# CompVis/ipoke

Hardware: AMD Instinct MI355X
Metric: video-frames/sec (second-stage train step) (higher is better)
Workload: dtype bf16; 1 GPU; plants_128 second_stage train, 16x3x128x128 clips, z=64, flow 2048 hidden (1.237 B params), per-GPU batch 20; global_batch=20, clip_frames=16, parallelism=dp1, weights=random init of the named architecture (no checkpoints offline)

## Files before the change

include/ipoke_hip.h:

```cpp
#ifndef IPOKE_HIP_H
#define IPOKE_HIP_H

#include <stdint.h>

#ifdef __cplusplus
extern "C" {
#endif

typedef enum {
  IPOKE_OK = 0,
  IPOKE_ERR_INVALID = -1,
  IPOKE_ERR_HIP = -2,
  IPOKE_ERR_STATE = -3
} ipoke_status;

enum { IPOKE_F32 = 0, IPOKE_BF16 = 1 };
enum { IPOKE_ACT_NONE = 0, IPOKE_ACT_ELU = 1, IPOKE_ACT_RELU = 2, IPOKE_ACT_LRELU02 = 3, IPOKE_ACT_TANH = 4,
       IPOKE_ACT_SIGMOID = 5 };

const char* ipoke_last_error(void);
int ipoke_version(void);
int ipoke_dtype_size(int dtype);

typedef struct {
// ... 26 lines not shown
  int32_t w_kmajor;
  int64_t c_sd;
  void* acc_scratch;
  int64_t acc_scratch_bytes;
} ipoke_conv_desc;

int ipoke_conv_forward(const ipoke_conv_desc* d, int dtype, void* stream);
int64_t ipoke_conv_acc_scratch_bytes(int M, int Nout, int splitk);
int ipoke_conv_acc_scratch_init(void* scratch, void* stream);

int ipoke_conv3x3_skinny_splitk(int M, int Kc, int dtype);

typedef struct {
  float* params; float* m; float* v; float* vmax; void* operand;
  float lr, beta1, beta2, eps, weight_decay, grad_scale;
  int32_t step;
  int32_t keep_grad;
} ipoke_wgrad_adam;

typedef struct {
  int32_t NB, Di, Hi, Wi, Do, Ho, Wo, kd, kh, kw, sd, sh, sw, pd, ph, pw, transposed;
  const void* A; int32_t a_f32; int64_t a_sn, a_sd, a_sh, a_sw, a_sc; int32_t a_coff, Kc_real, Kc;
  const void* dY; int32_t ldy; int32_t y_coff; int32_t Nout;
  float* dW; int64_t w_sn, w_sc, w_st;
  int32_t accumulate;
  int32_t splitm;
  int32_t Kc_store;
  int64_t split_stride;
  int32_t max_workgroups;
  const ipoke_wgrad_adam* adam;
} ipoke_wgrad_desc;

int ipoke_conv_wgrad(const ipoke_wgrad_desc* d, int dtype, void* stream);
int ipoke_conv_wgrad_splitm(const ipoke_wgrad_desc* d, int dtype, int target_workgroups);
int ipoke_wgrad_batch_entry_size(void);
int ipoke_conv_wgrad_batched(const ipoke_wgrad_desc* d, const void* entries_dev, int nbatch, const void* a_base,
                             const void* y_base, float* w_base, int dtype, void* stream);


int ipoke_nchw_to_state(const float* x_nchw, float* state, int B, int C, int P, int ld, void* stream);
int ipoke_state_to_nchw(const float* state, float* x_nchw, int B, int C, int P, int ld, void* stream);
int ipoke_extract_cols(const float* state, int ld, int off, int stride, int C, void* out, int ldo, int64_t M, int dtype,
                       void* stream);
int ipoke_cond_prepare(const float* cond_nchw, void* out, int B, int Cc, int P, int act, int dtype, void* stream);
int ipoke_copy_cols(const void* src, int lds, void* dst, int ldd, int C, int64_t M, int dtype, void* stream);

int ipoke_actnorm_fwd(const float* in, float* out, int M, int ld, int c0, int C, const float* log_scale,
                      const float* bias, const int32_t* idx, void* stream);
int ipoke_actnorm_inv(const float* in, float* out, int M, int ld, int c0, int C, const float* log_scale,
                      const float* bias, const int32_t* inv_idx, void* stream);
int ipoke_actnorm_inv_ext(const float* in, float* out, int M, int ld, int c0, int C, const float* log_scale,
                          const float* bias, const int32_t* inv_idx, void* ext, int ext_ld, int e_off, int e_stride, int e_C,
                          int dtype, void* stream);
int ipoke_actnorm_bwd(const float* dy, const float* x, float* dx, int M, int ld, int c0, int C,
                      const float* log_scale, const int32_t* idx, const float* dld, int B, int P,
                      float* part, void* stream);
int ipoke_actnorm_init(const float* x, int M, int ld, int c0, int C, float* log_scale, float* bias, void* stream);

typedef struct {
  const float* raw; int32_t nsplit; int64_t split_stride; int32_t ldraw;
  const float* bias;
  int32_t Cp, t_off, t_stride;
  int32_t P, ld;
} ipoke_affine_desc;
int ipoke_affine_fwd(const ipoke_affine_desc* d, const float* in, float* out, float* scale_out ,
                     float* logdet_slot , int slot_stride, int B, void* stream);
int ipoke_affine_inv(const ipoke_affine_desc* d, const float* in, float* out, int B, void* stream);
int ipoke_affine_fwd_ext(const ipoke_affine_desc* d, const float* in, float* out, float* scale_out, float* logdet_slot, int slot_stride,
                         int B, void* ext, int ext_ld, int dtype, void* stream);
int ipoke_affine_inv_ext(const ipoke_affine_desc* d, const float* in, float* out, int B, void* ext, int ext_ld, int dtype, void* stream);
int ipoke_affine_bwd(int Cp, int t_off, int t_stride, int P, int ld, const float* dy, const float* x,
                     const float* scale, const float* dld, float* dx, void* dparams , int ldp,
                     float* dbias_part , int B, int dtype, void* stream);
int ipoke_affine_actnorm_fwd(const ipoke_affine_desc* d, const float* in, float* out, float* out2, float* scale_out, float* logdet_slot,
                             int slot_stride, int B, int c0, int C, const float* log_scale, const float* bias, const int32_t* idx, void* stream);
int ipoke_actnorm_affine_bwd(int c0, int C, const float* log_scale, const int32_t* idx, const float* dy2, const float* x1, float* part,
                             int Cp, int t_off, int t_stride, int P, int ld, const float* x0, const float* scale, const float* dld, float* dx,
                             void* dparams, int ldp, float* dbias_part, int B, int dtype, void* stream);
typedef struct {
  int32_t mode;
  const float* in; float* out; float* out2; float* scale_out; float* logdet_slot; int32_t slot_stride;
  int32_t an_c0, an_C; const float* an_log_scale; const float* an_bias; const int32_t* an_idx;
  void* ext; int32_t ext_ld;
  void* xchg;
} ipoke_coupling_epi;
int ipoke_conv3x3_coupling_splitk(int M, int Kc, int dtype);
int64_t ipoke_conv3x3_coupling_xchg_bytes(void);
int ipoke_conv3x3_coupling_xchg_init(void* xchg, void* stream);
int ipoke_conv3x3_coupling(const ipoke_conv_desc* conv, const ipoke_affine_desc* aff, const ipoke_coupling_epi* epi, int B, int dtype,
                           void* stream);
int ipoke_reduce_rows(const float* src, float* dst, int R, int ncols, void* stream);
int ipoke_reduce_entry_size(void);
int ipoke_reduce_rows_multi(const float* src, float* dst, const void* entries_dev, int nentries, int R, void* stream);

int ipoke_logdet_finalize(const float* slots, int nslots, int B, int slot_w, float const_term, const float* const_dev,
                          float* logdet, void* stream);
int ipoke_actnorm_logdet(const float* params, const void* refs_dev, int n, int P, float* out_scalar, void* stream);
int ipoke_flow_nll(const float* z_state, const float* logdet, int B, int P, int C, int ld, float logdet_weight,
                   float* scalars3, float* d_out_state, float* dld, void* stream);
int ipoke_adam_amsgrad_step(float* p, const float* g, float* m, float* v, float* vmax, int64_t n, float lr, float beta1,
                            float beta2, float eps, float weight_decay, int step, float grad_scale, void* stream);
int ipoke_adam_amsgrad_step_grid(float* p, const float* g, float* m, float* v, float* vmax, int64_t n, float lr, float beta1,
                                 float beta2, float eps, float weight_decay, int step, float grad_scale, int max_blocks,
                                 void* stream);

typedef struct {
  const float* x; float* y;
  int32_t ld, C, B;
  const void* cond; int32_t Cc;
  const void* W1; const void* W2; const float* bias2;
  int32_t order;
  int32_t rows_per_block;
  void* a2_save; float* scale_save; float* logdet_slot;
  const void* W2T; const void* W1T;
  const float* dy; const float* dld; float* dx;
  void* dparams_save; void* dc_save; float* dbias_part;
  const float* post_log_scale; const float* post_bias;
  const float* y_post; float* post_part;
  void* x_op_save;
  void* zc_out; int32_t zc_off, zc_stride, zc_cin, zc_ld;
  int32_t split; void* xchg;
  const struct ipoke_unit_pair_desc* pair;
} ipoke_mcf_desc;
typedef struct ipoke_unit_pair_desc {
  const float* an_log_scale; const int32_t* an_idx; const float* an_x; float* an_part;
  int32_t Cp, t_off, t_stride; const float* x0; const float* scale; void* dparams; int32_t ldp; float* dbias_part;
  float* dx;
} ipoke_unit_pair_desc;
int ipoke_mcf_shadow_dims(int C, int Cc, int dtype, int32_t* dims8);
int ipoke_mcf_fwd(const ipoke_mcf_desc* d, int dtype, void* stream);
int ipoke_mcf_inv(const ipoke_mcf_desc* d, int dtype, void* stream);
int ipoke_mcf_bwd(const ipoke_mcf_desc* d, int dtype, void* stream);

int ipoke_macow_unit_supported(int C, int Cc, int dtype);
int64_t ipoke_macow_unit_xchg_bytes(int B, int split);
int ipoke_macow_unit_fwd(const ipoke_mcf_desc* d4, int dtype, void* stream);
int ipoke_macow_unit_bwd(const ipoke_mcf_desc* d4, int dtype, void* stream);
int ipoke_macow_unit_inv(const ipoke_mcf_desc* d4, int dtype, void* stream);

int ipoke_relayout_job_size(void);
int ipoke_wn_job_size(void);
int ipoke_relayout_multi(const float* params, void* shadow, const float* wn_scale, const void* jobs_dev, int njobs,
                         int total_blocks, const int32_t* block_job_dev, int dtype, void* stream);
int ipoke_relayout_multi_range(const float* params, void* shadow, const float* wn_scale, const void* jobs_dev, int njobs,
                               int block_begin, int nblocks, const int32_t* block_job_dev, int dtype, void* stream);
int ipoke_wn_scale_multi_range(const float* params, float* scale, float* inv_norm, const void* jobs_dev, int job_begin, int njobs,
                               int row_begin, int nrows, void* stream);
int ipoke_wn_scale_multi(const float* params, float* scale, float* inv_norm, const void* jobs_dev, int njobs,
                         int total_rows, void* stream);
int ipoke_wn_bwd_multi(const float* params, float* grads, const float* inv_norm, const void* jobs_dev, int njobs,
                       int total_rows, void* stream);
int ipoke_wn_bwd_multi_range(const float* params, float* grads, const float* inv_norm, const void* jobs_dev, int job_begin, int njobs,
                             int row_begin, int nrows, void* stream);



int ipoke_lu_job_size(void);
int ipoke_lu_prepare(const float* params, const float* fbuf, float* workspace, const void* jobs_dev, int njobs, void* stream);
int ipoke_lu_apply(const float* in, float* out, int64_t M, int ld, int C, const float* mat, int transposed, void* stream);
int ipoke_lu_wgrad(const float* dy, const float* x, int B, int P8, int ld, const float* params, const float* fbuf,
                   const float* workspace, const void* job_dev, const float* dld, float* grads, void* stream);

typedef struct ipoke_flow ipoke_flow;
typedef struct {
  int32_t z_channels;
  int32_t hidden;
  int32_t cond_channels;
  int32_t factor;
  int32_t n_levels;
  int32_t num_steps[32];
  int32_t kernel_h, kernel_w;
  int32_t dtype;
  int32_t max_batch;
  int32_t use1x1;
  int32_t condition_nice;
} ipoke_flow_config;

int ipoke_flow_create(const ipoke_flow_config* cfg, ipoke_flow** out);
void ipoke_flow_destroy(ipoke_flow* f);
int64_t ipoke_flow_param_count(const ipoke_flow* f);
int64_t ipoke_flow_index_count(const ipoke_flow* f);
int32_t ipoke_flow_tensor_count(const ipoke_flow* f);
int32_t ipoke_flow_op_count(const ipoke_flow* f);
int ipoke_flow_tensor_info(const ipoke_flow* f, int i, char* name, int name_cap, int64_t* offset, int32_t* ndim,
                           int64_t* shape4, int32_t* kind);
int ipoke_flow_set_graph(ipoke_flow* f, int enable);
int64_t ipoke_flow_float_buffer_count(const ipoke_flow* f);
int ipoke_flow_set_float_buffers(ipoke_flow* f, const float* fbuf_dev);
int64_t ipoke_flow_shadow_bytes(const ipoke_flow* f);
int ipoke_flow_op_info(const ipoke_flow* f, int i, int64_t* out32);
int64_t ipoke_flow_shadow_base(const ipoke_flow* f);
int64_t ipoke_flow_workspace_bytes(ipoke_flow* f, int B, int training);
int ipoke_flow_prepare_weights(ipoke_flow* f, const float* params, void* shadow, void* stream);
int ipoke_flow_forward(ipoke_flow* f, const float* params, const int32_t* perm, const void* shadow, const float* x_nchw,
                       const float* cond_nchw, int B, float* out_nchw, float* logdet, void* workspace,
                       int save_for_backward, void* stream);
int ipoke_flow_init_forward(ipoke_flow* f, float* params, const int32_t* perm, const float* x_nchw, int B,
                            float* out_nchw, float* logdet, void* workspace, void* stream);
int ipoke_flow_reverse(ipoke_flow* f, const float* params, const int32_t* perm, const void* shadow, const float* z_nchw,
                       const float* cond_nchw, int B, float* x_nchw, void* workspace, void* stream);
int ipoke_flow_prepare_weights_range(ipoke_flow* f, const float* params, void* shadow, int64_t begin, int64_t end, void* stream);
int ipoke_flow_adam_range(ipoke_flow* f, float* params, const float* grads, float* m, float* v, float* vmax, void* shadow, int64_t begin,
                          int64_t end, float lr, float beta1, float beta2, float eps, float weight_decay, int step, float grad_scale,
                          int max_blocks, void* stream);
int ipoke_adam_tile_job_size(void);
int ipoke_adam_seg_size(void);
int ipoke_adam_amsgrad_shadow_tiles(float* p, const float* g, float* m, float* v, float* vmax, void* shadow, const void* jobs_dev, int njobs,
                                    int tile_begin, int ntiles, float lr, float beta1, float beta2, float eps, float weight_decay, int step,
                                    float grad_scale, int max_blocks, int dtype, void* stream);
int ipoke_adam_amsgrad_cast_tiles(float* p, const float* g, float* m, float* v, float* vmax, void* shadow, const void* jobs_dev, int njobs,
                                  int tile_begin, int ntiles, float lr, float beta1, float beta2, float eps, float weight_decay, int step,
                                  float grad_scale, int max_blocks, int dtype, void* stream);
int ipoke_adam_amsgrad_segments(float* p, const float* g, float* m, float* v, float* vmax, const void* segs_dev, int seg_begin, int nsegs,
                                int64_t begin, int64_t end, float lr, float beta1, float beta2, float eps, float weight_decay, int step,
                                float grad_scale, int blocks_per_segment, void* stream);
int ipoke_flow_backward(ipoke_flow* f, const float* params, const int32_t* perm, const void* shadow,
                        const float* d_out_nchw, const float* d_logdet, int B, float* grads, float* dx_nchw,
                        void* workspace, void* stream);
typedef void (*ipoke_grad_ready_fn)(void* user, int piece, int64_t begin, int64_t end);
int ipoke_flow_piece_ranges(const ipoke_flow* f, int npieces, int64_t* ranges, int max_ranges);
int ipoke_flow_set_native_adam(ipoke_flow* f, float* m, float* v, float* vmax, float lr, float beta1, float beta2, float eps,
                               float weight_decay, int step, float grad_scale, int max_blocks);
int ipoke_flow_backward_pieces(ipoke_flow* f, const float* params, const int32_t* perm, const void* shadow,
                               const float* d_out_nchw, const float* d_logdet, int B, float* grads, float* dx_nchw,
                               void* workspace, int npieces, void* ready_stream, ipoke_grad_ready_fn ready, void* user,
                               void* stream);
int ipoke_flow_handoff_timeouts(ipoke_flow* f, uint32_t* out);
void* ipoke_flow_side_stream(ipoke_flow* f);


typedef struct {
  const void* x; int32_t ldx; void* y; int32_t ldy; int32_t y_f32;
  int32_t N, S, C, G; float eps;
  const float* gamma; const float* beta;
  const void* mod_gamma; const void* mod_beta; int32_t ld_mod;
  const void* res; int32_t ld_res;
  int32_t act;
  float* workspace;
  int32_t mod_samples;
  int32_t res_post;
  float* next_part; int32_t next_G;
  int32_t part_chunks;
} ipoke_norm_desc;
int64_t ipoke_groupnorm_workspace_floats(int N, int S, int G);
int ipoke_groupnorm(const ipoke_norm_desc* d, int dtype, void* stream);
int ipoke_add_act(const void* a, int lda, const void* b, int ldb, void* y, int ldy, int64_t M, int C, int act, int dtype,
                  void* stream);
int ipoke_gru_gates(const void* ur_pre, const void* h, int ldh, void* hr_out, int ld_hr, void* u_out, int64_t M, int Ch,
                    int dtype, void* stream);
int ipoke_gru_update(const void* o_pre, const void* u, const void* h, int ldh, void* h_new, int ld_new, int64_t M, int Ch,
                     int dtype, void* stream);
int ipoke_reparameterize(const void* mulv, int ld, const float* eps, float* z, float* mu, float* logvar, int64_t M, int Z,
                         int dtype, void* stream);
int ipoke_bilinear_cl(const float* x_nchw, float* y_cl, int N, int C, int Hi, int Wi, int Ho, int Wo, void* stream);
int ipoke_cl_to_nchw(const void* x_cl, int ld, float* y, int N, int C, int S, int dtype, void* stream);
int ipoke_nchw_to_cl(const float* x, void* y_cl, int ld, int N, int C, int S, int dtype, void* stream);

int ipoke_groupnorm_stats(const void* x, int ldx, int N, int S, int C, int G, float eps, float* workspace, int dtype, void* stream);
typedef struct {
  const void* x; int32_t ldx;
  const void* y; int32_t ldy;
  const void* dy; int32_t lddy;
  void* dx; int32_t lddx;
  void* dres; int32_t lddres;
  void* dmod_gamma; void* dmod_beta; int32_t ld_dmod;
  int32_t N, S, C, G; float eps;
  const float* gamma; const float* beta;
  const void* mod_gamma; int32_t ld_mod;
  float* dgamma; float* dbeta;
  int32_t act;
  float* workspace;
  const float* stats;
  int32_t mod_samples;
  const float* rs_scale; int32_t rs_scale_stride;
  int64_t rs_rows_per_group;
  const float* rs_bias;
  float* rs_dots;
  float* rs_dbias;
  float* rs_workspace;
  int32_t dmod_summed;
  int32_t act_from_pre;
} ipoke_norm_bwd_desc;
int64_t ipoke_groupnorm_stats_offset(int N, int S, int G);
int64_t ipoke_groupnorm_bwd_workspace_floats(int N, int S, int C, int G);
int64_t ipoke_groupnorm_bwd_rs_workspace_floats(int N, int S, int C);
int ipoke_groupnorm_bwd(const ipoke_norm_bwd_desc* d, int dtype, void* stream);
int ipoke_act_bwd(const void* dy, int lddy, const void* y, int ldy, void* out, int ldo, int64_t M, int C, int Cpad, int act,
                  int dtype, void* stream);
int64_t ipoke_colsum_workspace_floats(int64_t M, int C);
int ipoke_colsum(const void* src, int ld, int64_t M, int C, int src_f32, float* out, int accumulate, float* workspace, int dtype,
                 void* stream);
int ipoke_gru_update_bwd(const void* o_pre, const void* u, const void* h, int ldh, const void* d_hnew, int ld_dhnew, void* d_o_pre,
                         void* d_u, void* d_h, int ld_dh, int64_t M, int Ch, int dtype, void* stream);
int ipoke_gru_gates_bwd(const void* ur_pre, const void* h, int ldh, const void* d_hr, int ld_dhr, const void* d_u, void* d_ur_pre,
                        void* d_h, int ld_dh, int64_t M, int Ch, int dtype, void* stream);
int ipoke_conv_weight_operand(const float* w, int cout, int cin, int taps, int transposed, const float* inv_scale, void* out, int kc,
                              int dtype, void* stream);
int ipoke_conv_weight_operand_multi(const float* const* w, void* const* out, const int32_t* dims5, int count, int dtype, void* stream);
typedef struct { int32_t B, T, L, Cx, Ch, H, W; } ipoke_gru_desc;
int64_t ipoke_gru_workspace_bytes(const ipoke_gru_desc* d, int dtype);
int ipoke_gru_unroll_forward(const ipoke_gru_desc* d, const void* x0, int ldx, const void* h0, int ldh, const float* const* weights,
                             void* workspace, void* out, int ldo, int dtype, void* stream);
int ipoke_gru_unroll_backward(const ipoke_gru_desc* d, const void* d_out, int ldo, void* workspace, float* const* dweights, float* d_x0,
                              float* d_h0, int dtype, void* stream);
typedef struct {
  const void* dy; int32_t lddy;
// ... 80 lines not shown
```

include/ipoke_hip_dev.h:

```cpp
#ifndef IPOKE_HIP_DEV_H
#define IPOKE_HIP_DEV_H

#include "ipoke_hip.h"

#ifdef __cplusplus
extern "C" {
#endif

int ipoke_conv_forward_repeat(const ipoke_conv_desc* d, int dtype, int n, void* stream);
int ipoke_set_dispatch_override(const char* name, int value);
enum { IPOKE_KERNEL_NONE = 0, IPOKE_KERNEL_IGEMM = 1, IPOKE_KERNEL_S8 = 2, IPOKE_KERNEL_HALO = 3, IPOKE_KERNEL_HALO16 = 4, IPOKE_KERNEL_C64 = 5, IPOKE_KERNEL_K8 = 6 };
int ipoke_last_conv_kernel(void);
enum { IPOKE_WGRAD_KERNEL_NONE = 0, IPOKE_WGRAD_KERNEL_TN = 1, IPOKE_WGRAD_KERNEL_TN_GLDS = 2, IPOKE_WGRAD_KERNEL_TN_NARROW = 3,
       IPOKE_WGRAD_KERNEL_LAT8 = 4, IPOKE_WGRAD_KERNEL_HALO = 5 };
int ipoke_last_wgrad_kernel(void);

int ipoke_spin_delay(int us, void* stream);

#define IPOKE_TAG_NT_SQUARE 1
#define IPOKE_TAG_TN_SQUARE 2
#define IPOKE_TAG_UNIT_FWD 3
#define IPOKE_TAG_UNIT_BWD 4
#define IPOKE_TAG_UNIT_INV 5
#define IPOKE_TAG_NN_SQUARE 6
#define IPOKE_TAG_CONV_BASE 16
#define IPOKE_TAG_WGRAD 32
int ipoke_timing_start(void);
int ipoke_timing_start_all(void);
int ipoke_timing_stop(const int* tags, int ntags, int* counts, double* mean_us);
int ipoke_timing_stop_ex(const int* tags, int ntags, int* counts, double* total_us, double* flops, double* bytes);

int ipoke_desc_sizes(int32_t* out, int n);

int ipoke_flow_test_inject_timeout(ipoke_flow* f, int which, void* stream);

int ipoke_gru_set_fused(int mode);

#ifdef __cplusplus
}
#endif
#endif
```

ipoke_amd/_lib.py:

```python
import ctypes
import os
from ctypes import CFUNCTYPE, POINTER, Structure, c_char_p, c_float, c_int, c_int32, c_int64, c_uint32, c_void_p

_HERE = os.path.dirname(os.path.abspath(__file__))
LIB_PATH = os.environ.get("IPOKE_LIB_PATH") or os.path.join(_HERE, "libipoke_hip.so")

F32, BF16 = 0, 1
ACT_NONE, ACT_ELU, ACT_RELU, ACT_LRELU02, ACT_TANH, ACT_SIGMOID = range(6)

DTYPES = {"f32": F32, "fp32": F32, "float32": F32, "bf16": BF16, "bfloat16": BF16}


class ConvDesc(Structure):
    _fields_ = [(n, c_int32) for n in ("NB", "Di", "Hi", "Wi", "Do", "Ho", "Wo", "kd", "kh", "kw", "sd", "sh", "sw",
                                       "pd", "ph", "pw", "transposed")] + [
        ("A", c_void_p), ("a_f32", c_int32),
        ("a_sn", c_int64), ("a_sd", c_int64), ("a_sh", c_int64), ("a_sw", c_int64), ("a_sc", c_int64),
        ("a_coff", c_int32), ("Kc_real", c_int32), ("Kc", c_int32),
        ("W", c_void_p), ("ldw", c_int32), ("Nout", c_int32),
        ("bias", c_void_p), ("act", c_int32), ("dact", c_void_p), ("ld_dact", c_int32), ("dact_act", c_int32),
        ("C", c_void_p), ("c_f32", c_int32), ("c_accumulate", c_int32), ("ldc", c_int64),
        ("c_coff", c_int32), ("c_cstride", c_int32), ("splitk", c_int32),
        ("c_scatter", c_int32), ("c_sn", c_int64), ("c_sh", c_int64), ("c_sw", c_int64), ("c_row0", c_int64),
        ("row_scale", c_void_p), ("rs_images", c_int32), ("rs_stride", c_int32), ("w_kmajor", c_int32), ("c_sd", c_int64),
# ... 79 lines not shown
                ("N", c_int32), ("S", c_int32), ("C", c_int32), ("G", c_int32), ("eps", c_float),
                ("gamma", c_void_p), ("beta", c_void_p),
                ("mod_gamma", c_void_p), ("mod_beta", c_void_p), ("ld_mod", c_int32),
                ("res", c_void_p), ("ld_res", c_int32), ("act", c_int32), ("workspace", c_void_p), ("mod_samples", c_int32),
                ("res_post", c_int32), ("next_part", c_void_p), ("next_G", c_int32), ("part_chunks", c_int32)]


class SnJob(Structure):
    _fields_ = [("w", c_void_p), ("cout", c_int32), ("cin", c_int32), ("taps", c_int32), ("transposed", c_int32),
                ("u", c_void_p), ("v", c_void_p), ("out", c_void_p), ("out_stride", c_int64), ("snap", c_void_p), ("snap_stride", c_int64),
                ("workspace", c_void_p)]


class FlowConfig(Structure):
    _fields_ = [("z_channels", c_int32), ("hidden", c_int32), ("cond_channels", c_int32), ("factor", c_int32),
                ("n_levels", c_int32), ("num_steps", c_int32 * 32), ("kernel_h", c_int32), ("kernel_w", c_int32),
                ("dtype", c_int32), ("max_batch", c_int32), ("use1x1", c_int32), ("condition_nice", c_int32)]


_P = c_void_p
GRAD_READY_FN = CFUNCTYPE(None, c_void_p, c_int, c_int64, c_int64)
SIGNATURES = {
    "ipoke_last_error": (c_char_p, []),
    "ipoke_version": (c_int, []),
    "ipoke_dtype_size": (c_int, [c_int]),
    "ipoke_conv_forward": (c_int, [POINTER(ConvDesc), c_int, _P]),
    "ipoke_conv_forward_repeat": (c_int, [POINTER(ConvDesc), c_int, c_int, _P]),
    "ipoke_set_dispatch_override": (c_int, [c_char_p, c_int]),
    "ipoke_last_conv_kernel": (c_int, []),
    "ipoke_last_wgrad_kernel": (c_int, []),
    "ipoke_gru_set_fused": (c_int, [c_int]),
    "ipoke_gru_workspace_bytes": (c_int64, [POINTER(GruDesc), c_int]),
    "ipoke_gru_unroll_forward": (c_int, [POINTER(GruDesc), _P, c_int, _P, c_int, POINTER(c_void_p), _P, _P, c_int, c_int, _P]),
    "ipoke_gru_unroll_backward": (c_int, [POINTER(GruDesc), _P, c_int, _P, POINTER(c_void_p), _P, _P, c_int, _P]),
    "ipoke_rowscale_bwd_workspace_floats": (c_int64, [c_int64, c_int, c_int64]),
    "ipoke_rowscale_bwd": (c_int, [POINTER(RowScaleBwdDesc), c_int, _P]),
    "ipoke_spectral_bwd_frames": (c_int, [_P, c_int, c_int, c_int, c_int, _P, _P, c_int64, _P, c_int64, _P, c_int, _P]),
    "ipoke_sum_frames": (c_int, [_P, _P, c_int, c_int64, c_int, _P]),
    "ipoke_desc_sizes": (c_int, [POINTER(c_int32), c_int]),
    "ipoke_conv3x3_skinny_splitk": (c_int, [c_int, c_int, c_int]),
    "ipoke_conv3x3_coupling_splitk": (c_int, [c_int, c_int, c_int]),
    "ipoke_conv3x3_coupling_xchg_bytes": (c_int64, []),
    "ipoke_conv3x3_coupling_xchg_init": (c_int, [_P, _P]),
    "ipoke_conv3x3_coupling": (c_int, [POINTER(ConvDesc), POINTER(AffineDesc), POINTER(CouplingEpi), c_int, c_int, _P]),
    "ipoke_conv_wgrad": (c_int, [POINTER(WgradDesc), c_int, _P]),
    "ipoke_wgrad_batch_entry_size": (c_int, []),
    "ipoke_conv_wgrad_batched": (c_int, [POINTER(WgradDesc), _P, c_int, _P, _P, _P, c_int, _P]),
    "ipoke_reduce_entry_size": (c_int, []),
    "ipoke_reduce_rows_multi": (c_int, [_P, _P, _P, c_int, c_int, _P]),
    "ipoke_nchw_to_state": (c_int, [_P, _P, c_int, c_int, c_int, c_int, _P]),
    "ipoke_state_to_nchw": (c_int, [_P, _P, c_int, c_int, c_int, c_int, _P]),
    "ipoke_extract_cols": (c_int, [_P, c_int, c_int, c_int, c_int, _P, c_int, c_int64, c_int, _P]),
    "ipoke_copy_cols": (c_int, [_P, c_int, _P, c_int, c_int, c_int64, c_int, _P]),
    "ipoke_cond_prepare": (c_int, [_P, _P, c_int, c_int, c_int, c_int, c_int, _P]),
    "ipoke_actnorm_fwd": (c_int, [_P, _P, c_int, c_int, c_int, c_int, _P, _P, _P, _P]),
    "ipoke_actnorm_inv": (c_int, [_P, _P, c_int, c_int, c_int, c_int, _P, _P, _P, _P]),
    "ipoke_actnorm_inv_ext": (c_int, [_P, _P, c_int, c_int, c_int, c_int, _P, _P, _P, _P, c_int, c_int, c_int, c_int, c_int, _P]),
    "ipoke_actnorm_bwd": (c_int, [_P, _P, _P, c_int, c_int, c_int, c_int, _P, _P, _P, c_int, c_int, _P, _P]),
    "ipoke_actnorm_init": (c_int, [_P, c_int, c_int, c_int, c_int, _P, _P, _P]),
    "ipoke_affine_fwd": (c_int, [POINTER(AffineDesc), _P, _P, _P, _P, c_int, c_int, _P]),
    "ipoke_affine_inv": (c_int, [POINTER(AffineDesc), _P, _P, c_int, _P]),
    "ipoke_affine_fwd_ext": (c_int, [POINTER(AffineDesc), _P, _P, _P, _P, c_int, c_int, _P, c_int, c_int, _P]),
    "ipoke_affine_inv_ext": (c_int, [POINTER(AffineDesc), _P, _P, c_int, _P, c_int, c_int, _P]),
    "ipoke_affine_bwd": (c_int, [c_int, c_int, c_int, c_int, c_int, _P, _P, _P, _P, _P, _P, c_int, _P, c_int, c_int, _P]),
    "ipoke_affine_actnorm_fwd": (c_int, [POINTER(AffineDesc), _P, _P, _P, _P, _P, c_int, c_int, c_int, c_int, _P, _P, _P, _P]),
    "ipoke_actnorm_affine_bwd": (c_int, [c_int, c_int, _P, _P, _P, _P, _P, c_int, c_int, c_int, c_int, c_int, _P, _P, _P, _P, _P, c_int, _P,
                                         c_int, c_int, _P]),
    "ipoke_reduce_rows": (c_int, [_P, _P, c_int, c_int, _P]),
    "ipoke_spin_delay": (c_int, [c_int, _P]),
    "ipoke_logdet_finalize": (c_int, [_P, c_int, c_int, c_int, c_float, _P, _P, _P]),
    "ipoke_actnorm_logdet": (c_int, [_P, _P, c_int, c_int, _P, _P]),
    "ipoke_flow_nll": (c_int, [_P, _P, c_int, c_int, c_int, c_int, c_float, _P, _P, _P, _P]),
    "ipoke_adam_amsgrad_step": (c_int, [_P, _P, _P, _P, _P, c_int64, c_float, c_float, c_float, c_float, c_float, c_int,
                                        c_float, _P]),
    "ipoke_adam_amsgrad_step_grid": (c_int, [_P, _P, _P, _P, _P, c_int64, c_float, c_float, c_float, c_float, c_float, c_int,
                                             c_float, c_int, _P]),
    "ipoke_mcf_shadow_dims": (c_int, [c_int, c_int, c_int, POINTER(c_int32)]),
    "ipoke_mcf_fwd": (c_int, [POINTER(McfDesc), c_int, _P]),
    "ipoke_mcf_inv": (c_int, [POINTER(McfDesc), c_int, _P]),
    "ipoke_mcf_bwd": (c_int, [POINTER(McfDesc), c_int, _P]),
    "ipoke_macow_unit_supported": (c_int, [c_int, c_int, c_int]),
    "ipoke_macow_unit_xchg_bytes": (c_int64, [c_int, c_int]),
    "ipoke_macow_unit_fwd": (c_int, [POINTER(McfDesc), c_int, _P]),
    "ipoke_macow_unit_bwd": (c_int, [POINTER(McfDesc), c_int, _P]),
    "ipoke_macow_unit_inv": (c_int, [POINTER(McfDesc), c_int, _P]),
    "ipoke_relayout_job_size": (c_int, []),
    "ipoke_wn_job_size": (c_int, []),
    "ipoke_relayout_multi": (c_int, [_P, _P, _P, _P, c_int, c_int, _P, c_int, _P]),
    "ipoke_wn_scale_multi": (c_int, [_P, _P, _P, _P, c_int, c_int, _P]),
    "ipoke_wn_bwd_multi": (c_int, [_P, _P, _P, _P, c_int, c_int, _P]),
    "ipoke_groupnorm_workspace_floats": (c_int64, [c_int, c_int, c_int]),
    "ipoke_groupnorm": (c_int, [POINTER(NormDesc), c_int, _P]),
    "ipoke_add_act": (c_int, [_P, c_int, _P, c_int, _P, c_int, c_int64, c_int, c_int, c_int, _P]),
    "ipoke_gru_gates": (c_int, [_P, _P, c_int, _P, c_int, _P, c_int64, c_int, c_int, _P]),
    "ipoke_gru_update": (c_int, [_P, _P, _P, c_int, _P, c_int, c_int64, c_int, c_int, _P]),
    "ipoke_reparameterize": (c_int, [_P, c_int, _P, _P, _P, _P, c_int64, c_int, c_int, _P]),
    "ipoke_bilinear_cl": (c_int, [_P, _P, c_int, c_int, c_int, c_int, c_int, c_int, _P]),
    "ipoke_cl_to_nchw": (c_int, [_P, c_int, _P, c_int, c_int, c_int, c_int, _P]),
    "ipoke_nchw_to_cl": (c_int, [_P, _P, c_int, c_int, c_int, c_int, c_int, _P]),
    "ipoke_image_metrics_workspace_bytes": (c_int64, [c_int64, c_int, c_int]),
    "ipoke_psnr_ssim": (c_int, [_P, _P, c_int64, c_int, c_int, _P, _P, _P]),
    "ipoke_clip_to_cl4": (c_int, [_P, c_int64, c_int64, c_int64, c_int64, c_int64, c_int, c_int, c_int, c_int, c_int, c_int, _P, c_int, _P]),
    "ipoke_groupnorm_stats": (c_int, [_P, c_int, c_int, c_int, c_int, c_int, c_float, _P, c_int, _P]),
    "ipoke_groupnorm_stats_offset": (c_int64, [c_int, c_int, c_int]),
    "ipoke_groupnorm_bwd_workspace_floats": (c_int64, [c_int, c_int, c_int, c_int]),
    "ipoke_groupnorm_bwd": (c_int, [POINTER(NormBwdDesc), c_int, _P]),
    "ipoke_groupnorm_bwd_rs_workspace_floats": (c_int64, [c_int, c_int, c_int]),
    "ipoke_act_bwd": (c_int, [_P, c_int, _P, c_int, _P, c_int, c_int64, c_int, c_int, c_int, c_int, _P]),
    "ipoke_colsum_workspace_floats": (c_int64, [c_int64, c_int]),
    "ipoke_colsum": (c_int, [_P, c_int, c_int64, c_int, c_int, _P, c_int, _P, c_int, _P]),
    "ipoke_gru_update_bwd": (c_int, [_P, _P, _P, c_int, _P, c_int, _P, _P, _P, c_int, c_int64, c_int, c_int, _P]),
    "ipoke_gru_gates_bwd": (c_int, [_P, _P, c_int, _P, c_int, _P, _P, _P, c_int, c_int64, c_int, c_int, _P]),
    "ipoke_conv_weight_operand": (c_int, [_P, c_int, c_int, c_int, c_int, _P, _P, c_int, c_int, _P]),
    "ipoke_conv_weight_operand_multi": (c_int, [POINTER(c_void_p), POINTER(c_void_p), POINTER(c_int32), c_int, c_int, _P]),
    "ipoke_spectral_workspace_floats": (ctypes.c_long, [c_int, c_int, c_int]),
    "ipoke_spectral_sigma": (c_int, [_P, c_int, c_int, c_int, c_int, _P, _P, c_int, ctypes.c_float, _P, _P, _P, _P]),
    "ipoke_spectral_bwd": (c_int, [_P, c_int, c_int, c_int, c_int, _P, _P, _P, _P, _P]),
    "ipoke_spectral_bwd_workspace_floats": (ctypes.c_long, []),
    "ipoke_sn_job_size": (c_int, []),
    "ipoke_sn_jobs_upload": (c_int, [_P, c_int, _P, _P]),
    "ipoke_spectral_sigma_multi": (c_int, [_P, c_int, c_int, c_int, c_int, c_float, _P]),
    "ipoke_adam_multi": (c_int, [_P, _P, _P, _P, _P, c_int, ctypes.c_float, ctypes.c_float, ctypes.c_float, ctypes.c_float,
                                 ctypes.c_float, c_int, ctypes.c_float, _P]),
    "ipoke_maxpool3d_fwd": (c_int, [_P, _P, c_int, _P, c_int, _P, c_int, _P]),
    "ipoke_maxpool3d_bwd": (c_int, [_P, _P, c_int, _P, _P, c_int, c_int, _P]),
    "ipoke_avgpool_rows": (c_int, [_P, c_int, _P, c_int, c_int64, c_int, c_int, c_int, _P]),
    "ipoke_avgpool_rows_bwd": (c_int, [_P, c_int, _P, c_int, c_int64, c_int, c_int, c_int, _P]),
    "ipoke_groupnorm_jvp": (c_int, [_P, c_int, _P, c_int, _P, c_int, _P, c_int, _P, c_int, _P, c_int, c_int, c_int, c_int, c_int, c_float,
                                    _P, c_int, _P]),
    "ipoke_groupnorm_jvp_bwd": (c_int, [_P, c_int, _P, c_int, _P, c_int, _P, c_int, _P, c_int, _P, c_int, _P, c_int, _P, _P,
                                        c_int, c_int, c_int, c_int, c_int, c_float, _P, c_int, _P]),
    "ipoke_groupnorm_jvp_workspace_floats": (ctypes.c_long, [c_int, c_int]),
    "ipoke_gather_rows": (c_int, [_P, c_int, _P, _P, c_int, c_int64, c_int, c_int, _P]),
    "ipoke_l1_pair": (c_int, [_P, c_int, _P, c_int, c_int64, c_int, c_float, _P, _P, c_int, c_int, _P]),
    "ipoke_kl_loss": (c_int, [_P, _P, c_int64, c_int, _P, _P, _P, _P]),
    "ipoke_reparam_bwd": (c_int, [_P, c_int, _P, _P, _P, _P, _P, c_int, c_int64, c_int, c_int, _P]),
    "ipoke_l1_loss": (c_int, [_P, c_int, _P, c_int, c_int, c_int, c_int64, c_float, _P, _P, c_int, _P, _P]),
    "ipoke_l1_loss_partials": (ctypes.c_long, []),
    "ipoke_relayout_multi_range": (c_int, [_P, _P, _P, _P, c_int, c_int, c_int, _P, c_int, _P]),
    "ipoke_wn_scale_multi_range": (c_int, [_P, _P, _P, _P, c_int, c_int, c_int, c_int, _P]),
    "ipoke_flow_prepare_weights_range": (c_int, [_P, _P, _P, c_int64, c_int64, _P]),
    "ipoke_flow_set_native_adam": (c_int, [_P, _P, _P, _P, c_float, c_float, c_float, c_float, c_float, c_int, c_float, c_int]),
    "ipoke_flow_adam_range": (c_int, [_P, _P, _P, _P, _P, _P, _P, c_int64, c_int64, c_float, c_float, c_float, c_float, c_float, c_int,
                                      c_float, c_int, _P]),
    "ipoke_adam_tile_job_size": (c_int, []),
    "ipoke_adam_seg_size": (c_int, []),
    "ipoke_adam_amsgrad_shadow_tiles": (c_int, [_P, _P, _P, _P, _P, _P, _P, c_int, c_int, c_int, c_float, c_float, c_float, c_float, c_float,
                                                c_int, c_float, c_int, c_int, _P]),
    "ipoke_adam_amsgrad_cast_tiles": (c_int, [_P, _P, _P, _P, _P, _P, _P, c_int, c_int, c_int, c_float, c_float, c_float, c_float, c_float,
                                              c_int, c_float, c_int, c_int, _P]),
    "ipoke_adam_amsgrad_segments": (c_int, [_P, _P, _P, _P, _P, _P, c_int, c_int, c_int64, c_int64, c_float, c_float, c_float, c_float,
                                            c_float, c_int, c_float, c_int, _P]),
    "ipoke_wn_bwd_multi_range": (c_int, [_P, _P, _P, _P, c_int, c_int, c_int, c_int, _P]),
    "ipoke_flow_backward_pieces": (c_int, [_P, _P, _P, _P, _P, _P, c_int, _P, _P, _P, c_int, _P, GRAD_READY_FN, _P, _P]),
    "ipoke_video_to_cl": (c_int, [_P, c_int64, c_int64, c_int64, c_int64, c_int64, c_int, c_int, c_int, c_int, c_int, _P, c_int, c_int, c_int,
                                  c_int, _P, _P]),
    "ipoke_min_reset": (c_int, [_P, _P]),
    "ipoke_denorm_if_negative": (c_int, [_P, c_int64, c_int, c_int, c_int, c_int, _P, _P]),
    "ipoke_pool3d_same": (c_int, [_P, _P, c_int, _P, c_int, c_int, _P]),
    "ipoke_pool_rows_weighted": (c_int, [_P, c_int, _P, c_int, c_int64, c_int, c_int, _P, c_int, _P]),
    "ipoke_activation_moments": (c_int, [_P, c_int, c_int, _P, _P, _P, _P]),
    "ipoke_flow_resize": (c_int, [_P, _P, c_int, c_int, c_int, c_int, c_int, c_int, c_float, _P]),
    "ipoke_poke_workspace_bytes": (c_int64, [c_int, c_int, c_int, c_int, c_int]),
    "ipoke_poke_simulate": (c_int, [_P, c_int, c_int, c_int, c_int, c_int, c_int, c_int, _P, _P, _P, _P, _P, _P, _P, _P]),
    "ipoke_timing_start": (c_int, []),
    "ipoke_timing_start_all": (c_int, []),
    "ipoke_timing_stop": (c_int, [POINTER(c_int), c_int, POINTER(c_int), POINTER(ctypes.c_double)]),
    "ipoke_timing_stop_ex": (c_int, [POINTER(c_int), c_int, POINTER(c_int), POINTER(ctypes.c_double), POINTER(ctypes.c_double),
                                     POINTER(ctypes.c_double)]),
    "ipoke_flow_create": (c_int, [POINTER(FlowConfig), POINTER(c_void_p)]),
    "ipoke_flow_destroy": (None, [_P]),
    "ipoke_flow_piece_ranges": (c_int, [_P, c_int, POINTER(c_int64), c_int]),
    "ipoke_flow_handoff_timeouts": (c_int, [_P, POINTER(c_uint32)]),
    "ipoke_flow_side_stream": (c_void_p, [_P]),
    "ipoke_flow_test_inject_timeout": (c_int, [_P, c_int, _P]),
    "ipoke_conv_wgrad_splitm": (c_int, [_P, c_int, c_int]),
    "ipoke_conv_acc_scratch_bytes": (c_int64, [c_int, c_int, c_int]),
    "ipoke_conv_acc_scratch_init": (c_int, [_P, _P]),
    "ipoke_flow_param_count": (c_int64, [_P]),
    "ipoke_flow_index_count": (c_int64, [_P]),
    "ipoke_flow_tensor_count": (c_int32, [_P]),
    "ipoke_flow_op_count": (c_int32, [_P]),
    "ipoke_flow_tensor_info": (c_int, [_P, c_int, c_char_p, c_int, POINTER(c_int64), POINTER(c_int32), POINTER(c_int64),
                                       POINTER(c_int32)]),
    "ipoke_flow_shadow_bytes": (c_int64, [_P]),
    "ipoke_flow_set_graph": (c_int, [_P, c_int]),
    "ipoke_flow_float_buffer_count": (c_int64, [_P]),
    "ipoke_flow_set_float_buffers": (c_int, [_P, _P]),
    "ipoke_lu_job_size": (c_int, []),
    "ipoke_lu_prepare": (c_int, [_P, _P, _P, _P, c_int, _P]),
    "ipoke_lu_apply": (c_int, [_P, _P, c_int64, c_int, c_int, _P, c_int, _P]),
    "ipoke_lu_wgrad": (c_int, [_P, _P, c_int, c_int, c_int, _P, _P, _P, _P, _P, _P, _P]),
    "ipoke_flow_op_info": (c_int, [_P, c_int, POINTER(c_int64)]),
    "ipoke_flow_shadow_base": (c_int64, [_P]),
    "ipoke_flow_workspace_bytes": (c_int64, [_P, c_int, c_int]),
    "ipoke_flow_prepare_weights": (c_int, [_P, _P, _P, _P]),
    "ipoke_flow_forward": (c_int, [_P, _P, _P, _P, _P, _P, c_int, _P, _P, _P, c_int, _P]),
    "ipoke_flow_init_forward": (c_int, [_P, _P, _P, _P, c_int, _P, _P, _P, _P]),
    "ipoke_flow_reverse": (c_int, [_P, _P, _P, _P, _P, _P, c_int, _P, _P, _P]),
    "ipoke_flow_backward": (c_int, [_P, _P, _P, _P, _P, _P, c_int, _P, _P, _P, _P]),
}

_lib = None


def lib():
    global _lib
    if _lib is None:
        if not os.path.exists(LIB_PATH):
            raise RuntimeError(
                f"{LIB_PATH} not found: the HIP extension is not built. ipoke_amd has no CPU fallback; "
                "run `make -C ipoke_amd/csrc` (or __graft_entry__.build()) first.")
        import torch
        handle = ctypes.CDLL(LIB_PATH)
        for name, (res, args) in SIGNATURES.items():
            fn = getattr(handle, name)
            fn.restype = res
            fn.argtypes = args
        _lib = handle
    return _lib


def check(rc):
    if rc != 0:
        msg = lib().ipoke_last_error()
        raise RuntimeError(f"libipoke_hip call failed ({rc}): {msg.decode() if msg else '?'}")


def ptr(t):
    if t is None:
        return None
    return c_void_p(t.data_ptr())


def current_stream():
    import torch
    return c_void_p(torch.cuda.current_stream().cuda_stream)


def require_gpu():
    import torch
    if not torch.cuda.is_available():
        raise RuntimeError("ipoke_amd needs an MI355X (gfx950) GPU: no HIP device is visible and there is no CPU path")


import contextlib


KERNEL_NONE, KERNEL_IGEMM, KERNEL_S8, KERNEL_HALO, KERNEL_HALO16, KERNEL_C64, KERNEL_K8 = range(7)
WGRAD_NONE, WGRAD_TN, WGRAD_TN_GLDS, WGRAD_TN_NARROW, WGRAD_LAT8, WGRAD_HALO = range(6)


@contextlib.contextmanager
def dispatch_override(name, value):
    check(lib().ipoke_set_dispatch_override(name.encode(), int(value)))
    try:
        yield
    finally:
        check(lib().ipoke_set_dispatch_override(name.encode(), -1))
```

ipoke_amd/csrc/flow_engine.hip:

```cpp
#include <functional>
#include <memory>
#include <vector>
#include <string>
#include <cstring>

#include "common.h"

namespace ipoke {

enum OpType { OP_ACTNORM = 0, OP_MCF = 1, OP_NICE = 2, OP_LU = 3 };
enum TensorKind { TK_PARAM = 0, TK_IDX_FWD = 1, TK_IDX_BWD = 2, TK_FLAG = 3, TK_FBUF = 4 };

struct TensorInfo {
  std::string name;
  int64_t offset;
  std::vector<int64_t> shape;
  int kind;
};

struct Op {
  int type = 0;
  int C = 0;
  int c0 = 0, Cn = 0;
  int64_t p_ls = -1, p_bias = -1, idx_fwd = -1, idx_bwd = -1;
  int order = 0;
  int64_t p_w1 = -1, p_b = -1, p_g = -1, p_v = -1;
  int Cp = 0, K1p = 0, K2p = 0, K3p = 0, Hq = 0, H = 0;
  int64_t sh_w1 = -1, sh_w1t = -1, sh_w2 = -1, sh_w2t = -1;
  int64_t wn_off = -1;
  int cin = 0, cout = 0, z_off = 0, z_stride = 1, t_off = 0, t_stride = 1;
  int64_t p_c1 = -1, p_c2 = -1;
  int Kc1 = 0, Kc3 = 0;
  int64_t sh_c1 = -1, sh_c1t = -1, sh_c2 = -1, sh_c2t = -1, sh_c3 = -1, sh_c3t = -1;
  int64_t ws_a = -1, ws_b = -1, ws_c = -1, ws_d = -1, ws_e = -1, ws_f = -1, ws_g = -1;
  int slot = -1;
  int mcf_idx = -1;
  int nice_idx = -1;
  int hidK = 0;
  int level = 0;
  int fuse_act = -1;
  bool fused = false;
  bool unit_head = false;
  int unit_of = -1;
  int lu_idx = -1;
  int an_next = -1;
  int an_prev = -1;
  int pair_unit = -1;
};

struct RelayoutJobH {
  long src_off, s_n, s_k, dstA, dstB, scale_off;
  int taps, n_real, k_real, A_rows_pad, A_inner_pad, B_rows_pad, B_inner_pad, B_rows_real, tile, tiles_k, block_start, frag_tiled;
};
struct WnJobH { long v_off, g_off, out_off; int rows, K, row_start; };
struct AdamTileJobH { long src_off, dstA, dstB; int N, K, tile_start, pad; };
struct AdamSegH { long off, len; };
struct LsRefH { long off; int C; };
struct LuJobH { long p_l, p_u, p_logs, b_perm, b_sign, b_lmask, b_umask, b_eye, w_off; int C, pad; };

}

using namespace ipoke;

struct ipoke_flow {
  ipoke_flow_config cfg;
  int esz = 2, e16 = 8, ks = 32;
  std::vector<TensorInfo> tensors;
  std::vector<Op> ops;
  int64_t n_params = 0, n_perm = 0, n_fbuf = 0;
  std::vector<LuJobH> lujobs; void* d_lujobs = nullptr; const float* fbuf = nullptr;
  int64_t shadow_elems = 0;
  int64_t wn_rows = 0;
  int nslots = 0;
  int n_mcf = 0;
  int tab_B = 0; void* d_w1tab = nullptr; void* d_w2tab = nullptr; void* d_redtab = nullptr; int n_red = 0;
  void* d_ntab[3] = {nullptr, nullptr, nullptr};
  int n_nice = 0;
  std::vector<RelayoutJobH> rjobs; int rblocks = 0;
  std::vector<AdamTileJobH> ajobs; int atiles = 0;
  std::vector<RelayoutJobH> rjobs2; int rblocks2 = 0;
  std::vector<AdamSegH> asegs;
  void* d_ajobs = nullptr; void* d_rjobs2 = nullptr; void* d_rblockjob2 = nullptr; void* d_asegs = nullptr;
  std::vector<WnJobH> wjobs;
  std::vector<LsRefH> lsrefs;
  void* d_rjobs = nullptr; void* d_wjobs = nullptr; void* d_lsrefs = nullptr; void* d_rblockjob = nullptr;
  hipStream_t side = nullptr;
  std::vector<hipStream_t> lanes;
  int n_lanes = 1;
  std::vector<hipEvent_t> events; size_t ev_next = 0;
  bool use_side = true;
  struct GraphEntry { std::vector<uintptr_t> key; hipGraph_t graph = nullptr; hipGraphExec_t exec = nullptr; int state = 0; uint64_t used = 0; };
  std::vector<GraphEntry> graphs; hipStream_t cap = nullptr; bool use_graph = false; uint64_t tick = 0;
  struct Unit { int64_t p_lo, p_hi; int wj_lo, wj_hi, row_lo, row_hi; int kind; int op_lo, op_hi; int64_t p2_lo = -1, p2_hi = -1; };
  std::vector<Unit> units;
  std::vector<int> red_first;
  int last_fwd_B = 0; bool have_saved = false;
  int P = 64;
  int unit_split = 1; void* d_xchg = nullptr;
  bool coupling_fuse = false; void* d_cxchg = nullptr;
  void* d_acc = nullptr; int64_t acc_bytes = 0;
  unsigned* h_tmo = nullptr; hipEvent_t pass_ev = nullptr; hipStream_t pass_stream = nullptr; bool pass_recorded = false, pass_unchecked = false;
  int64_t xchg_bytes = 0;
  bool mcf_xop = false;
  bool c2_straight = false;
  struct NativeAdam { bool on = false; float* m = nullptr; float* v = nullptr; float* vmax = nullptr; float lr = 0, beta1 = 0, beta2 = 0, eps = 0, wd = 0,
                      grad_scale = 1; int step = 0, max_blocks = 0; } nadam;
};

namespace {

int64_t align_up(int64_t v, int64_t a) { return (v + a - 1) / a * a; }

struct Builder {
  ipoke_flow& f;
  explicit Builder(ipoke_flow& fl) : f(fl) {}
  int64_t add_param(const std::string& name, std::vector<int64_t> shape) {
    int64_t n = 1; for (auto s : shape) n *= s;
    const int64_t off = f.n_params;
    f.tensors.push_back({name, off, shape, TK_PARAM});
    f.n_params = align_up(off + n, 4);
    return off;
  }
  int64_t add_idx(const std::string& name, int C, int kind) {
    const int64_t off = f.n_perm;
    f.tensors.push_back({name, off, {C}, kind});
    f.n_perm += C;
    return off;
  }
  void add_flag(const std::string& name) { f.tensors.push_back({name, -1, {}, TK_FLAG}); }
  int64_t add_fbuf(const std::string& name, std::vector<int64_t> shape) {
    int64_t n = 1; for (auto s : shape) n *= s;
    const int64_t off = f.n_fbuf;
    f.tensors.push_back({name, off, shape, TK_FBUF});
    f.n_fbuf = align_up(off + n, 4);
    return off;
  }
  void lu(const std::string& pfx, int C) {
    Op op; op.type = OP_LU; op.C = C; op.lu_idx = (int)f.lujobs.size();
    LuJobH j{};
    j.C = C;
    j.p_l = add_param(pfx + ".l", {C, C}); j.p_u = add_param(pfx + ".u", {C, C}); j.p_logs = add_param(pfx + ".log_s", {C});
    j.b_perm = add_fbuf(pfx + ".permutated", {C, C}); j.b_sign = add_fbuf(pfx + ".sign_s", {C});
    j.b_lmask = add_fbuf(pfx + ".lmask", {C, C}); j.b_umask = add_fbuf(pfx + ".umask", {C, C}); j.b_eye = add_fbuf(pfx + ".eye", {C, C});
    j.w_off = (long)op.lu_idx * 4 * 64 * 64;
    f.lujobs.push_back(j);
    f.lsrefs.push_back({j.p_logs, C});
    f.ops.push_back(op);
  }
  int64_t add_shadow(int64_t elems) {
    const int64_t off = f.shadow_elems;
    f.shadow_elems = align_up(off + elems, 64);
    return off;
  }
  void relayout_pair(long src, long s_n, long s_k, int taps, int n_real, int k_real, long scale, long dstA, int A_rows_pad,
                     int A_inner_pad, long dstB, int B_rows_pad, int B_inner_pad, int B_rows_real, int frag_tiled = 0) {
    const int tile = taps == 1 ? 64 : 32;
    const int n_ext = std::max(A_rows_pad, B_inner_pad), k_ext = std::max(A_inner_pad, B_rows_pad);
    const int tiles_n = (n_ext + tile - 1) / tile, tiles_k = (k_ext + tile - 1) / tile;
    RelayoutJobH j{src, s_n, s_k, dstA, dstB, scale, taps, n_real, k_real, A_rows_pad, A_inner_pad, B_rows_pad, B_inner_pad,
                   B_rows_real, tile, tiles_k, f.rblocks, frag_tiled};
    f.rjobs.push_back(j);
    f.rblocks += tiles_n * tiles_k;
    const bool fusable = taps == 1 && scale < 0 && !frag_tiled && s_k == 1 && s_n == k_real && n_real % 64 == 0 && k_real % 64 == 0 &&
                         A_rows_pad == n_real && A_inner_pad == k_real && B_rows_pad == k_real && B_inner_pad == n_real &&
                         B_rows_real == k_real;
    if (fusable) {
      f.ajobs.push_back({src, dstA, dstB, n_real, k_real, f.atiles, 0});
      f.atiles += (n_real / 64) * (k_real / 64);
    } else {
      j.block_start = f.rblocks2;
      f.rjobs2.push_back(j);
      f.rblocks2 += tiles_n * tiles_k;
    }
  }

  void actnorm(const std::string& pfx, int C_active, int c0, int Cn, const std::string* shuffle_pfx) {
    Op op; op.type = OP_ACTNORM; op.C = C_active; op.c0 = c0; op.Cn = Cn;
    if (!pfx.empty()) {
      op.p_ls = add_param(pfx + ".log_scale", {Cn, 1, 1});
      op.p_bias = add_param(pfx + ".bias", {Cn, 1, 1});
      add_flag(pfx + ".initialized");
      f.lsrefs.push_back({(long)op.p_ls, Cn});
    }
    if (shuffle_pfx) {
      op.idx_fwd = add_idx(*shuffle_pfx + ".forward_shuffle_idx", Cn, TK_IDX_FWD);
      op.idx_bwd = add_idx(*shuffle_pfx + ".backward_shuffle_idx", Cn, TK_IDX_BWD);
    }
    f.ops.push_back(op);
  }

  void mcf(const std::string& pfx, int C, int order) {
    const int Cc = f.cfg.cond_channels;
    Op op; op.type = OP_MCF; op.C = C; op.order = order;
    const int kh = order < 2 ? f.cfg.kernel_h : f.cfg.kernel_w, kw = order < 2 ? f.cfg.kernel_w : f.cfg.kernel_h;
    op.H = 4 * C;
    op.Cp = round_up(C, f.ks);
    op.K1p = 6 * op.Cp;
    op.K2p = round_up(op.H + Cc, f.ks);
    op.K3p = round_up(2 * C, f.ks);
    op.Hq = round_up(op.H, f.ks);
    const int K2 = op.H + Cc;
    op.p_w1 = add_param(pfx + ".net.shift_conv.weight", {op.H, C, kh, kw});
    add_flag(pfx + ".net.conv1x1.initialized");
    op.p_b = add_param(pfx + ".net.conv1x1.conv.bias", {2 * C});
    op.p_g = add_param(pfx + ".net.conv1x1.conv.weight_g", {2 * C, 1, 1, 1});
    op.p_v = add_param(pfx + ".net.conv1x1.conv.weight_v", {2 * C, K2, 1, 1});
    op.wn_off = f.wn_rows;
    f.wjobs.push_back({(long)op.p_v, (long)op.p_g, (long)op.wn_off, 2 * C, K2, (int)f.wn_rows});
    f.wn_rows += 2 * C;
    const int Hr = round_up(op.H, 16), N2r = round_up(2 * C, 16), Cr = round_up(C, 16);
    op.sh_w1 = add_shadow((int64_t)Hr * op.K1p);
    op.sh_w1t = add_shadow((int64_t)Cr * 6 * op.Hq);
    op.sh_w2 = add_shadow((int64_t)N2r * op.K2p);
    op.sh_w2t = add_shadow((int64_t)Hr * op.K3p);
    relayout_pair(op.p_w1, (long)C * 6, 6, 6, op.H, C, -1, op.sh_w1, Hr, op.Cp, op.sh_w1t, Cr, op.Hq, C, 1);
    relayout_pair(op.p_v, K2, 1, 1, 2 * C, K2, op.wn_off, op.sh_w2, N2r, op.K2p, op.sh_w2t, Hr, op.K3p, op.H, 1);
    op.slot = f.nslots++;
    op.mcf_idx = f.n_mcf++;
    f.ops.push_back(op);
  }

  void nice(const std::string& pfx, int C, bool skip, bool up, int factor) {
    const int hid = f.cfg.hidden;
    Op op; op.type = OP_NICE; op.C = C;
    op.cout = C / factor; op.cin = C - op.cout;
    if (skip && (C % 2 == 1)) skip = false;
    if (!skip) {
      const int z1 = up ? op.cin : op.cout;
      if (up) { op.z_off = 0; op.t_off = z1; } else { op.z_off = z1; op.t_off = 0; }
      op.z_stride = op.t_stride = 1;
    } else {
      op.z_stride = op.t_stride = 2;
      if (up) { op.z_off = 0; op.t_off = 1; } else { op.z_off = 1; op.t_off = 0; }
    }
    op.Kc1 = round_up(op.cin, f.e16);
    op.Kc3 = round_up(2 * op.cout, f.e16);
// ... 304 lines not shown
  d.W1 = c.sh(op.sh_w1); d.W2 = c.sh(op.sh_w2); d.bias2 = c.params + op.p_b; d.order = op.order;
  d.W1T = c.sh(op.sh_w1t); d.W2T = c.sh(op.sh_w2t);
}

int lu_prepare_all(const Ctx& c) {
  ipoke_flow* f = c.f;
  if (f->lujobs.empty()) return IPOKE_OK;
  IPK_REQUIRE(f->fbuf != nullptr, "use1x1: ipoke_flow_set_float_buffers has not been called");
  IPK_REQUIRE(f->n_lanes == 1, "use1x1 does not support sub-batch lanes");
  return ipoke_lu_prepare(c.params, f->fbuf, c.at<float>(c.plan.lu), f->d_lujobs, (int)f->lujobs.size(), c.stream());
}
const float* lu_mat(const Ctx& c, const Op& op, int which) {
  return c.at<float>(c.plan.lu) + (int64_t)op.lu_idx * 4 * 64 * 64 + (int64_t)which * op.C * op.C;
}

int common_checks(ipoke_flow* f, int B) {
  IPK_REQUIRE(f != nullptr, "null flow handle");
  IPK_REQUIRE(B >= 1 && B <= f->cfg.max_batch, "batch exceeds max_batch of the flow handle");
  return IPOKE_OK;
}

struct WgEntryH { long a_off, y_off, w_off; int kh, kw, ph, pw; long sh_off = 0; };
struct RedEntryH { long src, dst; int ld, ncols, rmul, pad; };

void drop_graphs(ipoke_flow* f) {
  for (auto& g : f->graphs) {
    if (g.exec) (void)hipGraphExecDestroy(g.exec);
    if (g.graph) (void)hipGraphDestroy(g.graph);
  }
  f->graphs.clear();
}

int ensure_tables(ipoke_flow* f, int B, const Plan& plan) {
  if (f->tab_B == B && f->d_w1tab) return IPOKE_OK;
  IPK_REQUIRE((int)sizeof(WgEntryH) == ipoke_wgrad_batch_entry_size() && (int)sizeof(RedEntryH) == ipoke_reduce_entry_size(),
              "batch table layout mismatch");
  std::vector<WgEntryH> w1(f->n_mcf), w2(f->n_mcf);
  std::vector<WgEntryH> nt[3] = {std::vector<WgEntryH>(f->n_nice), std::vector<WgEntryH>(f->n_nice), std::vector<WgEntryH>(f->n_nice)};
  std::vector<RedEntryH> red;
  f->red_first.assign(f->ops.size() + 1, 0);
  for (size_t i = 0; i < f->ops.size(); ++i) {
    const Op& op = f->ops[i];
    f->red_first[i] = (int)red.size();
    const long dbp = (long)(plan.dbias_part / 4) + (long)i * (kMaxUnitSplit * B + 1) * 128;
    const int rmul = op.unit_of >= 0 || op.pair_unit >= 0 ? f->unit_split : 1;
    if (op.type == OP_MCF) {
      const McfGeom g = mcf_geom(op.order);
      w1[op.mcf_idx] = {f->mcf_xop ? (long)op.ws_e : (long)(plan.state0 + (int64_t)i * plan.state_stride), (long)op.ws_d, (long)op.p_w1, g.kh,
                        g.kw, -g.oy, -g.ox};
      w2[op.mcf_idx] = {(long)op.ws_a, (long)op.ws_c, (long)op.p_v, 1, 1, 0, 0};
      red.push_back({dbp, (long)op.p_b, 2 * op.C, 2 * op.C, rmul, 0});
    } else if (op.type == OP_NICE) {
      nt[0][op.nice_idx] = {(long)op.ws_g, (long)op.ws_f, (long)op.p_c1, 3, 3, 1, 1};
      nt[1][op.nice_idx] = {(long)op.ws_a, (long)op.ws_e, (long)op.p_c2, 1, 1, 0, 0, (long)op.sh_c2};
      nt[2][op.nice_idx] = {(long)op.ws_b, (long)op.ws_d, (long)op.p_v, 3, 3, 1, 1};
      red.push_back({dbp, (long)op.p_b, 2 * op.cout, 2 * op.cout, rmul, 0});
    } else if (op.p_ls >= 0) {
      red.push_back({dbp, (long)op.p_ls, 2 * op.Cn, op.Cn, rmul, 0});
      red.push_back({dbp + op.Cn, (long)op.p_bias, 2 * op.Cn, op.Cn, rmul, 0});
    }
  }
  drop_graphs(f);
  f->red_first[f->ops.size()] = (int)red.size();
  if (f->d_w1tab) { (void)hipFree(f->d_w1tab); (void)hipFree(f->d_w2tab); (void)hipFree(f->d_redtab); }
  for (int k = 0; k < 3; ++k) {
    if (f->d_ntab[k]) (void)hipFree(f->d_ntab[k]);
    IPK_HIP(hipMalloc(&f->d_ntab[k], nt[k].size() * sizeof(WgEntryH)));
    IPK_HIP(hipMemcpy(f->d_ntab[k], nt[k].data(), nt[k].size() * sizeof(WgEntryH), hipMemcpyHostToDevice));
  }
  IPK_HIP(hipMalloc(&f->d_w1tab, w1.size() * sizeof(WgEntryH)));
  IPK_HIP(hipMalloc(&f->d_w2tab, w2.size() * sizeof(WgEntryH)));
  IPK_HIP(hipMalloc(&f->d_redtab, red.size() * sizeof(RedEntryH)));
  IPK_HIP(hipMemcpy(f->d_w1tab, w1.data(), w1.size() * sizeof(WgEntryH), hipMemcpyHostToDevice));
  IPK_HIP(hipMemcpy(f->d_w2tab, w2.data(), w2.size() * sizeof(WgEntryH), hipMemcpyHostToDevice));
  IPK_HIP(hipMemcpy(f->d_redtab, red.data(), red.size() * sizeof(RedEntryH), hipMemcpyHostToDevice));
  f->n_red = (int)red.size();
  f->tab_B = B;
  return IPOKE_OK;
}

std::vector<std::pair<int, int>> backward_pieces(const ipoke_flow* f, int npieces) {
  std::vector<std::pair<int, int>> pieces;
  const int U = (int)f->units.size();
  int64_t total = 0;
  for (const auto& u : f->units) total += u.p_hi - u.p_lo;
  const int np = npieces < 1 ? 1 : (npieces > U ? U : npieces);
  static double ta = -1, tb = -1;
  if (ta < 0) {
    ta = 0.5; tb = 0.25;
    if (const char* e = getenv("IPOKE_PIECE_TAPER")) { double a = 0, b = 0; if (sscanf(e, "%lf,%lf", &a, &b) == 2 && a > 0 && b > 0) { ta = a; tb = b; } }
  }
  std::vector<double> w((size_t)np, 1.0);
  if (np >= 4) { w[(size_t)np - 2] = ta; w[(size_t)np - 1] = tb; }
  double wsum = 0; for (double x : w) wsum += x;
  int hi = U - 1;
  int64_t acc = 0; double target_acc = 0;
  int64_t done = 0;
  for (int u = U - 1; u >= 0; --u) {
    acc += f->units[u].p_hi - f->units[u].p_lo;
    const int idx = (int)pieces.size();
    const int left = np - idx;
    const double want = (double)total * (target_acc + w[(size_t)(idx < np ? idx : np - 1)]) / wsum;
    if (u == 0 || (left > 1 && ((double)(done + acc) >= want || u == left - 1))) {
      pieces.push_back({u, hi}); hi = u - 1; done += acc; acc = 0; target_acc += w[(size_t)(idx < np ? idx : np - 1)];
    }
  }
  return pieces;
}
void piece_param_ranges(const ipoke_flow* f, int lvl_lo, int lvl_hi, int64_t p0[3], int64_t p1[3]) {
  for (int k = 0; k < 3; ++k) { p0[k] = -1; p1[k] = -1; }
  for (int u = lvl_lo; u <= lvl_hi; ++u) {
    const auto& un = f->units[u];
    const int k = un.kind;
    if (p0[k] < 0) p0[k] = un.p_lo;
    p1[k] = un.p_hi;
    if (un.p2_lo >= 0) { if (p0[2] < 0) p0[2] = un.p2_lo; p1[2] = un.p2_hi; }
  }
}

hipEvent_t next_event(ipoke_flow* f) {
  hipEvent_t e = f->events[f->ev_next];
  f->ev_next = (f->ev_next + 1) % f->events.size();
  return e;
}

}

extern "C" int ipoke_flow_create(const ipoke_flow_config* cfg, ipoke_flow** out) {
  IPK_REQUIRE(cfg && out, "null argument");
  IPK_REQUIRE(cfg->dtype == IPOKE_F32 || cfg->dtype == IPOKE_BF16, "bad dtype");
  IPK_REQUIRE(cfg->n_levels >= 1 && cfg->n_levels <= 32 && cfg->n_levels < cfg->factor, "num_steps must be shorter than factor");
  IPK_REQUIRE(cfg->z_channels % cfg->factor == 0 && cfg->z_channels <= 64, "flow_in_channels must be a multiple of factor, <= 64");
  IPK_REQUIRE((cfg->z_channels / cfg->factor) % 2 == 0, "channel step must be even (skip split)");
  IPK_REQUIRE(cfg->kernel_h == 2 && cfg->kernel_w == 3, "kernel_size must be [2,3] (shipped configs)");
  IPK_REQUIRE(cfg->hidden % 32 == 0 && cfg->cond_channels % 32 == 0, "hidden / cond widths must be multiples of 32");
  std::unique_ptr<ipoke_flow> f(new ipoke_flow());
  f->cfg = *cfg;
  f->esz = cfg->dtype == IPOKE_BF16 ? 2 : 4; f->e16 = 16 / f->esz; f->ks = 64 / f->esz;
  {
    const char* cs = getenv("IPOKE_C2_STRAIGHT");
    f->c2_straight = cfg->dtype == IPOKE_BF16 && cfg->hidden % 64 == 0 && !(cs && cs[0] == '0');
  }
  int rc = build(*f); if (rc) return rc;
  {
    int64_t pos = 0;
    for (size_t k = 0; k < f->ajobs.size(); ++k) {
      IPK_REQUIRE(f->ajobs[k].src_off >= pos, "fused tensors must be in parameter order");
      if (f->ajobs[k].src_off > pos) f->asegs.push_back({(long)pos, (long)(f->ajobs[k].src_off - pos)});
      pos = f->ajobs[k].src_off + (int64_t)f->ajobs[k].N * f->ajobs[k].K;
    }
    if (pos < f->n_params) f->asegs.push_back({(long)pos, (long)(f->n_params - pos)});
    for (size_t k = 1; k < f->rjobs.size(); ++k) IPK_REQUIRE(f->rjobs[k].src_off > f->rjobs[k - 1].src_off, "relayout jobs must be in parameter order");
  }
  const char* env = getenv("IPOKE_NO_SIDE_STREAM");
  f->use_side = !(env && env[0] == '1');
  const char* gr = getenv("IPOKE_GRAPH");
  f->use_graph = gr && gr[0] == '1';
  const char* ln = getenv("IPOKE_LANES");
  f->n_lanes = ln ? atoi(ln) : 1;
  if (f->n_lanes < 1) f->n_lanes = 1;
  if (f->n_lanes > kMaxLanes) f->n_lanes = kMaxLanes;
  {
    const char* us = getenv("IPOKE_UNIT_SPLIT");
    f->unit_split = us ? atoi(us) : kDefaultUnitSplit;
    if (f->unit_split != 2 && f->unit_split != 4) f->unit_split = 1;
    if (f->n_lanes > 1 || cfg->dtype != IPOKE_BF16) f->unit_split = 1;
  }
  f->coupling_fuse = f->n_lanes == 1 && cfg->dtype == IPOKE_BF16 && ipoke_conv3x3_coupling_splitk(64, cfg->hidden, cfg->dtype) > 0;
  {
    const char* up = getenv("IPOKE_UNIT_PAIR");
    const bool on = f->unit_split > 1 && f->n_lanes == 1 && (up ? atoi(up) != 0 : true);
    for (size_t h = 2; on && h < f->ops.size(); ++h) {
      const Op& u = f->ops[h]; Op& an = f->ops[h - 1]; Op& cp = f->ops[h - 2];
      if (u.unit_head && an.type == OP_ACTNORM && an.an_prev == (int)h - 2 && cp.type == OP_NICE && an.c0 == 0 && an.Cn == u.C &&
          cp.cout <= 32 && cp.t_off + (cp.cout - 1) * cp.t_stride < u.C) {
        an.pair_unit = (int)h; cp.pair_unit = (int)h;
      }
    }
  }
  *out = f.release();
  return IPOKE_OK;
}

static int ensure_device(ipoke_flow* f) {
  if (f->d_rjobs) return IPOKE_OK;
  if (f->unit_split > 1 && !f->d_xchg) {
    const int64_t nb = ipoke_macow_unit_xchg_bytes(f->cfg.max_batch, f->unit_split);
    IPK_HIP(hipMalloc(&f->d_xchg, nb));
    IPK_HIP(hipMemset(f->d_xchg, 0, nb));
    f->xchg_bytes = nb;
  }
  if (!f->d_acc) {
    static const bool atomics = getenv("IPOKE_DGRAD_ATOMICS") != nullptr;
    if (!atomics) {
      f->acc_bytes = ipoke_conv_acc_scratch_bytes(f->cfg.max_batch * f->P, 64, 32);
      IPK_HIP(hipMalloc(&f->d_acc, (size_t)f->acc_bytes));
      int rc = ipoke_conv_acc_scratch_init(f->d_acc, nullptr); if (rc) return rc;
      IPK_HIP(hipDeviceSynchronize());
    }
  }
  if (!f->h_tmo) {
    IPK_HIP(hipHostMalloc(reinterpret_cast<void**>(&f->h_tmo), 64, hipHostMallocMapped));
    std::memset(f->h_tmo, 0, 64);
    IPK_HIP(hipEventCreateWithFlags(&f->pass_ev, hipEventDisableTiming));
  }
  if (f->coupling_fuse && !f->d_cxchg) {
    IPK_HIP(hipMalloc(&f->d_cxchg, (size_t)ipoke_conv3x3_coupling_xchg_bytes()));
    int rc = ipoke_conv3x3_coupling_xchg_init(f->d_cxchg, nullptr); if (rc) return rc;
    IPK_HIP(hipDeviceSynchronize());
  }
  IPK_REQUIRE((int)sizeof(RelayoutJobH) == ipoke_relayout_job_size() && (int)sizeof(WnJobH) == ipoke_wn_job_size(),
              "job table layout mismatch");
  IPK_HIP(hipMalloc(&f->d_rjobs, f->rjobs.size() * sizeof(RelayoutJobH)));
  IPK_HIP(hipMemcpy(f->d_rjobs, f->rjobs.data(), f->rjobs.size() * sizeof(RelayoutJobH), hipMemcpyHostToDevice));
  {
    std::vector<int32_t> bj((size_t)f->rblocks);
    for (size_t k = 0; k < f->rjobs.size(); ++k) {
      const int b0 = f->rjobs[k].block_start, b1 = k + 1 < f->rjobs.size() ? f->rjobs[k + 1].block_start : f->rblocks;
      for (int b = b0; b < b1; ++b) bj[b] = (int32_t)k;
    }
    IPK_HIP(hipMalloc(&f->d_rblockjob, bj.size() * sizeof(int32_t)));
    IPK_HIP(hipMemcpy(f->d_rblockjob, bj.data(), bj.size() * sizeof(int32_t), hipMemcpyHostToDevice));
  }
  IPK_REQUIRE((int)sizeof(AdamTileJobH) == ipoke_adam_tile_job_size() && (int)sizeof(AdamSegH) == ipoke_adam_seg_size(), "Adam table layout mismatch");
  if (!f->ajobs.empty()) {
    IPK_HIP(hipMalloc(&f->d_ajobs, f->ajobs.size() * sizeof(AdamTileJobH)));
    IPK_HIP(hipMemcpy(f->d_ajobs, f->ajobs.data(), f->ajobs.size() * sizeof(AdamTileJobH), hipMemcpyHostToDevice));
  }
  if (!f->asegs.empty()) {
    IPK_HIP(hipMalloc(&f->d_asegs, f->asegs.size() * sizeof(AdamSegH)));
    IPK_HIP(hipMemcpy(f->d_asegs, f->asegs.data(), f->asegs.size() * sizeof(AdamSegH), hipMemcpyHostToDevice));
  }
  if (!f->rjobs2.empty()) {
    IPK_HIP(hipMalloc(&f->d_rjobs2, f->rjobs2.size() * sizeof(RelayoutJobH)));
    IPK_HIP(hipMemcpy(f->d_rjobs2, f->rjobs2.data(), f->rjobs2.size() * sizeof(RelayoutJobH), hipMemcpyHostToDevice));
    std::vector<int32_t> bj((size_t)f->rblocks2);
    for (size_t k = 0; k < f->rjobs2.size(); ++k) {
      const int b0 = f->rjobs2[k].block_start, b1 = k + 1 < f->rjobs2.size() ? f->rjobs2[k + 1].block_start : f->rblocks2;
      for (int b = b0; b < b1; ++b) bj[b] = (int32_t)k;
    }
    IPK_HIP(hipMalloc(&f->d_rblockjob2, bj.size() * sizeof(int32_t)));
    IPK_HIP(hipMemcpy(f->d_rblockjob2, bj.data(), bj.size() * sizeof(int32_t), hipMemcpyHostToDevice));
  }
  IPK_HIP(hipMalloc(&f->d_wjobs, f->wjobs.size() * sizeof(WnJobH)));
  IPK_HIP(hipMemcpy(f->d_wjobs, f->wjobs.data(), f->wjobs.size() * sizeof(WnJobH), hipMemcpyHostToDevice));
  if (!f->lujobs.empty()) {
    IPK_REQUIRE((int)sizeof(LuJobH) == ipoke_lu_job_size(), "LU job table layout mismatch");
    IPK_HIP(hipMalloc(&f->d_lujobs, f->lujobs.size() * sizeof(LuJobH)));
    IPK_HIP(hipMemcpy(f->d_lujobs, f->lujobs.data(), f->lujobs.size() * sizeof(LuJobH), hipMemcpyHostToDevice));
  }
  IPK_HIP(hipMalloc(&f->d_lsrefs, f->lsrefs.size() * sizeof(LsRefH)));
  IPK_HIP(hipMemcpy(f->d_lsrefs, f->lsrefs.data(), f->lsrefs.size() * sizeof(LsRefH), hipMemcpyHostToDevice));
  {
    int least = 0, greatest = 0;
    IPK_HIP(hipDeviceGetStreamPriorityRange(&least, &greatest));
    static const bool flat = getenv("IPOKE_SIDE_FLAT_PRIORITY") != nullptr;
    IPK_HIP(hipStreamCreateWithPriority(&f->side, hipStreamNonBlocking, flat ? 0 : least));
  }
  IPK_HIP(hipStreamCreateWithFlags(&f->cap, hipStreamNonBlocking));
  f->lanes.resize(kMaxLanes - 1);
  for (auto& l : f->lanes) IPK_HIP(hipStreamCreateWithFlags(&l, hipStreamNonBlocking));
  f->events.resize(256);
  for (auto& e : f->events) IPK_HIP(hipEventCreateWithFlags(&e, hipEventDisableTiming));
  return IPOKE_OK;
}

extern "C" void ipoke_flow_destroy(ipoke_flow* f) {
  if (!f) return;
  if (f->d_rjobs) (void)hipFree(f->d_rjobs);
  if (f->d_wjobs) (void)hipFree(f->d_wjobs);
  if (f->d_lsrefs) (void)hipFree(f->d_lsrefs);
  if (f->d_lujobs) (void)hipFree(f->d_lujobs);
  if (f->d_rblockjob) (void)hipFree(f->d_rblockjob);
  if (f->d_ajobs) (void)hipFree(f->d_ajobs);
  if (f->d_asegs) (void)hipFree(f->d_asegs);
  if (f->d_rjobs2) (void)hipFree(f->d_rjobs2);
  if (f->d_rblockjob2) (void)hipFree(f->d_rblockjob2);
  if (f->d_w1tab) (void)hipFree(f->d_w1tab);
  for (int k = 0; k < 3; ++k) if (f->d_ntab[k]) (void)hipFree(f->d_ntab[k]);
  if (f->d_w2tab) (void)hipFree(f->d_w2tab);
  if (f->d_redtab) (void)hipFree(f->d_redtab);
  if (f->d_xchg) (void)hipFree(f->d_xchg);
  if (f->d_cxchg) (void)hipFree(f->d_cxchg);
  if (f->d_acc) (void)hipFree(f->d_acc);
  if (f->pass_ev) (void)hipEventDestroy(f->pass_ev);
  if (f->h_tmo) (void)hipHostFree(f->h_tmo);
  for (auto e : f->events) (void)hipEventDestroy(e);
  drop_graphs(f);
  if (f->side) (void)hipStreamDestroy(f->side);
  if (f->cap) (void)hipStreamDestroy(f->cap);
  for (auto l : f->lanes) if (l) (void)hipStreamDestroy(l);
  delete f;
}

extern "C" int ipoke_flow_piece_ranges(const ipoke_flow* f, int npieces, int64_t* ranges, int max_ranges) {
  IPK_REQUIRE(f != nullptr && (ranges != nullptr || max_ranges == 0), "bad arguments");
  const std::vector<std::pair<int, int>> pieces = backward_pieces(f, npieces);
  int n = 0;
  for (size_t i = 0; i < pieces.size(); ++i) {
    int64_t p0[3], p1[3];
    piece_param_ranges(f, pieces[i].first, pieces[i].second, p0, p1);
    for (int kind = 0; kind < 3; ++kind) {
      if (p0[kind] < 0 || p1[kind] <= p0[kind]) continue;
      if (n < max_ranges) { ranges[3 * n] = (int64_t)i; ranges[3 * n + 1] = p0[kind]; ranges[3 * n + 2] = p1[kind]; }
      ++n;
    }
  }
  return n;
}

extern "C" void* ipoke_flow_side_stream(ipoke_flow* f) {
  if (!f || ensure_device(f) != IPOKE_OK) return nullptr;
  return reinterpret_cast<void*>(f->side);
}
extern "C" int64_t ipoke_flow_param_count(const ipoke_flow* f) { return f ? f->n_params : -1; }
extern "C" int64_t ipoke_flow_index_count(const ipoke_flow* f) { return f ? f->n_perm : -1; }
extern "C" int ipoke_flow_set_graph(ipoke_flow* f, int enable) {
  IPK_REQUIRE(f != nullptr, "null flow handle");
  f->use_graph = enable != 0;
  return IPOKE_OK;
}
extern "C" int64_t ipoke_flow_float_buffer_count(const ipoke_flow* f) { return f ? f->n_fbuf : -1; }
extern "C" int ipoke_flow_set_float_buffers(ipoke_flow* f, const float* fbuf_dev) {
  IPK_REQUIRE(f != nullptr, "null flow handle");
  f->fbuf = fbuf_dev;
  return IPOKE_OK;
}
extern "C" int32_t ipoke_flow_tensor_count(const ipoke_flow* f) { return f ? (int32_t)f->tensors.size() : -1; }
extern "C" int32_t ipoke_flow_op_count(const ipoke_flow* f) { return f ? (int32_t)f->ops.size() : -1; }
extern "C" int ipoke_flow_tensor_info(const ipoke_flow* f, int i, char* name, int name_cap, int64_t* offset, int32_t* ndim,
                                      int64_t* shape4, int32_t* kind) {
  IPK_REQUIRE(f && i >= 0 && i < (int)f->tensors.size() && name && offset && ndim && shape4 && kind, "bad arguments");
  const TensorInfo& t = f->tensors[i];
  IPK_REQUIRE((int)t.name.size() + 1 <= name_cap, "name buffer too small");
  std::memcpy(name, t.name.c_str(), t.name.size() + 1);
  *offset = t.offset; *ndim = (int32_t)t.shape.size(); *kind = t.kind;
  for (int k = 0; k < 4; ++k) shape4[k] = k < (int)t.shape.size() ? t.shape[k] : 1;
  return IPOKE_OK;
}
extern "C" int ipoke_flow_op_info(const ipoke_flow* f, int i, int64_t* out32) {
  IPK_REQUIRE(f && out32 && i >= 0 && i < (int)f->ops.size(), "bad arguments");
  const Op& o = f->ops[i];
  const int64_t v[32] = {o.type, o.C, o.c0, o.Cn, o.p_ls, o.p_bias, o.idx_fwd, o.idx_bwd, o.order, o.p_w1, o.p_b, o.p_g, o.p_v,
                         o.sh_w1, o.sh_w1t, o.sh_w2, o.sh_w2t, o.wn_off, o.cin, o.cout, o.z_off, o.z_stride, o.t_off, o.t_stride,
                         o.p_c1, o.p_c2, o.sh_c1, o.sh_c1t, o.sh_c2, o.sh_c2t, o.sh_c3, o.sh_c3t};
  for (int k = 0; k < 32; ++k) out32[k] = v[k];
  return IPOKE_OK;
}
extern "C" int64_t ipoke_flow_shadow_base(const ipoke_flow* f) { return f ? 2 * align_up(f->wn_rows, 64) * 4 : -1; }

extern "C" int64_t ipoke_flow_shadow_bytes(const ipoke_flow* f) {
  if (!f) return -1;
  return 2 * align_up(f->wn_rows, 64) * 4 + f->shadow_elems * f->esz;
}
extern "C" int64_t ipoke_flow_workspace_bytes(ipoke_flow* f, int B, int training) {
  if (!f || B < 1) return -1;
  return make_plan(*f, B, training ? 1 : 0).bytes;
}

extern "C" int ipoke_flow_prepare_weights(ipoke_flow* f, const float* params, void* shadow, void* stream) {
  IPK_REQUIRE(f && params && shadow, "null argument");
  { int rc0 = ensure_device(f); if (rc0) return rc0; }
  float* wn_scale = reinterpret_cast<float*>(shadow);
  float* wn_inv = wn_scale + align_up(f->wn_rows, 64);
  int rc = ipoke_wn_scale_multi(params, wn_scale, wn_inv, f->d_wjobs, (int)f->wjobs.size(), (int)f->wn_rows, stream);
  if (rc) return rc;
  void* sh = reinterpret_cast<unsigned char*>(shadow) + 2 * align_up(f->wn_rows, 64) * 4;
  return ipoke_relayout_multi(params, sh, wn_scale, f->d_rjobs, (int)f->rjobs.size(), f->rblocks,
                              reinterpret_cast<const int32_t*>(f->d_rblockjob), f->cfg.dtype, stream);
}

static int prepare_range(ipoke_flow* f, const float* params, void* shadow, int64_t begin, int64_t end, bool skip_fused, void* stream) {
  float* wn_scale = reinterpret_cast<float*>(shadow);
  float* wn_inv = wn_scale + align_up(f->wn_rows, 64);
  int w0 = 0, w1 = 0;
  while (w0 < (int)f->wjobs.size() && f->wjobs[w0].v_off < begin) ++w0;
  w1 = w0;
  while (w1 < (int)f->wjobs.size() && f->wjobs[w1].v_off < end) ++w1;
  if (w1 > w0) {
    const int row0 = f->wjobs[w0].row_start;
    const int row1 = w1 < (int)f->wjobs.size() ? f->wjobs[w1].row_start : (int)f->wn_rows;
    int rc = ipoke_wn_scale_multi_range(params, wn_scale, wn_inv, f->d_wjobs, w0, w1 - w0, row0, row1 - row0, stream);
    if (rc) return rc;
  }
  const std::vector<RelayoutJobH>& jobs = skip_fused ? f->rjobs2 : f->rjobs;
  const int nblocks = skip_fused ? f->rblocks2 : f->rblocks;
  int j0 = 0, j1 = 0;
  while (j0 < (int)jobs.size() && jobs[j0].src_off < begin) ++j0;
  j1 = j0;
  while (j1 < (int)jobs.size() && jobs[j1].src_off < end) ++j1;
  if (j1 > j0) {
    const int b0 = jobs[j0].block_start;
    const int b1 = j1 < (int)jobs.size() ? jobs[j1].block_start : nblocks;
    void* sh = reinterpret_cast<unsigned char*>(shadow) + 2 * align_up(f->wn_rows, 64) * 4;
    return ipoke_relayout_multi_range(params, sh, wn_scale, skip_fused ? f->d_rjobs2 : f->d_rjobs, (int)jobs.size(), b0, b1 - b0,
                                      reinterpret_cast<const int32_t*>(skip_fused ? f->d_rblockjob2 : f->d_rblockjob), f->cfg.dtype, stream);
  }
  return IPOKE_OK;
}

extern "C" int ipoke_flow_set_native_adam(ipoke_flow* f, float* m, float* v, float* vmax, float lr, float beta1, float beta2, float eps,
                                          float weight_decay, int step, float grad_scale, int max_blocks) {
  IPK_REQUIRE(f != nullptr, "null flow handle");
  ipoke_flow::NativeAdam& A = f->nadam;
  A.on = m != nullptr;
  if (!A.on) return IPOKE_OK;
  IPK_REQUIRE(v && vmax && step >= 1, "bad optimizer state");
  A.m = m; A.v = v; A.vmax = vmax; A.lr = lr; A.beta1 = beta1; A.beta2 = beta2; A.eps = eps; A.wd = weight_decay; A.step = step;
  A.grad_scale = grad_scale; A.max_blocks = max_blocks;
  return IPOKE_OK;
}

extern "C" int ipoke_flow_prepare_weights_range(ipoke_flow* f, const float* params, void* shadow, int64_t begin, int64_t end,
                                                void* stream) {
  IPK_REQUIRE(f && params && shadow && begin >= 0 && end >= begin, "bad arguments");
  { int rc0 = ensure_device(f); if (rc0) return rc0; }
  return prepare_range(f, params, shadow, begin, end, false, stream);
}

static int adam_range(ipoke_flow* f, float* params, const float* grads, float* m, float* v, float* vmax, void* shadow, int64_t begin, int64_t end,
                      float lr, float beta1, float beta2, float eps, float weight_decay, int step, float grad_scale, int max_blocks, void* stream,
                      bool skip_tiles = false);

extern "C" int ipoke_flow_adam_range(ipoke_flow* f, float* params, const float* grads, float* m, float* v, float* vmax, void* shadow,
                                     int64_t begin, int64_t end, float lr, float beta1, float beta2, float eps, float weight_decay,
                                     int step, float grad_scale, int max_blocks, void* stream) {
  IPK_REQUIRE(f && params && grads && m && v && vmax && shadow && begin >= 0 && end >= begin && end <= f->n_params, "bad arguments");
  { int rc0 = ensure_device(f); if (rc0) return rc0; }
  return adam_range(f, params, grads, m, v, vmax, shadow, begin, end, lr, beta1, beta2, eps, weight_decay, step, grad_scale, max_blocks, stream);
}

static int adam_range(ipoke_flow* f, float* params, const float* grads, float* m, float* v, float* vmax, void* shadow, int64_t begin, int64_t end,
                      float lr, float beta1, float beta2, float eps, float weight_decay, int step, float grad_scale, int max_blocks, void* stream,
                      bool skip_tiles) {
  if (end == begin) return IPOKE_OK;
  int a0 = 0, a1 = 0;
  while (a0 < (int)f->ajobs.size() && f->ajobs[a0].src_off < begin) ++a0;
  a1 = a0;
  while (a1 < (int)f->ajobs.size() && f->ajobs[a1].src_off < end) ++a1;
  if (a1 > a0 && !skip_tiles) {
    IPK_REQUIRE(f->ajobs[a1 - 1].src_off + (int64_t)f->ajobs[a1 - 1].N * f->ajobs[a1 - 1].K <= end, "range must cover whole tensors");
    const int t0 = f->ajobs[a0].tile_start, t1 = a1 < (int)f->ajobs.size() ? f->ajobs[a1].tile_start : f->atiles;
    void* sh = reinterpret_cast<unsigned char*>(shadow) + 2 * align_up(f->wn_rows, 64) * 4;
    int rc = f->c2_straight
        ? ipoke_adam_amsgrad_cast_tiles(params, grads, m, v, vmax, sh, f->d_ajobs, (int)f->ajobs.size(), t0, t1 - t0, lr, beta1, beta2,
                                        eps, weight_decay, step, grad_scale, max_blocks, f->cfg.dtype, stream)
        : ipoke_adam_amsgrad_shadow_tiles(params, grads, m, v, vmax, sh, f->d_ajobs, (int)f->ajobs.size(), t0, t1 - t0, lr, beta1, beta2,
                                          eps, weight_decay, step, grad_scale, max_blocks, f->cfg.dtype, stream);
    if (rc) return rc;
  }
  int s0 = 0, s1 = 0;
  while (s0 < (int)f->asegs.size() && f->asegs[s0].off + f->asegs[s0].len <= begin) ++s0;
  s1 = s0;
  while (s1 < (int)f->asegs.size() && f->asegs[s1].off < end) ++s1;
  if (s1 > s0) {
    int per = max_blocks > 0 ? max_blocks / (s1 - s0) : 16;
    if (per < 2) per = 2; if (per > 32) per = 32;
    int rc = ipoke_adam_amsgrad_segments(params, grads, m, v, vmax, f->d_asegs, s0, s1 - s0, begin, end, lr, beta1, beta2, eps, weight_decay,
                                         step, grad_scale, per, stream);
    if (rc) return rc;
  }
  return prepare_range(f, params, shadow, begin, end, true, stream);
}

static int make_lanes(const Ctx& full, int want, std::vector<Ctx>& lanes) {
  ipoke_flow* f = full.f;
  int n = want < 1 ? 1 : want;
  if (n > kMaxLanes) n = kMaxLanes;
  if (n > full.B) n = full.B;
  lanes.clear();
  int b0 = 0;
  for (int k = 0; k < n; ++k) {
    const int nb = (full.B - b0 + (n - k) - 1) / (n - k);
    Ctx c = full;
    c.b0 = b0; c.B = nb; c.M = (int64_t)nb * f->P; c.Bfull = full.B; c.lane = k;
    c.s = k == 0 ? full.s : f->lanes[k - 1];
    lanes.push_back(c);
    b0 += nb;
  }
  return IPOKE_OK;
}
static int fork_lanes(ipoke_flow* f, hipStream_t from, const std::vector<Ctx>& lanes) {
  if (lanes.size() < 2) return IPOKE_OK;
  hipEvent_t e = next_event(f);
  IPK_HIP(hipEventRecord(e, from));
  for (size_t k = 1; k < lanes.size(); ++k) IPK_HIP(hipStreamWaitEvent(lanes[k].s, e, 0));
  return IPOKE_OK;
}
static int join_lanes(ipoke_flow* f, const std::vector<Ctx>& lanes, hipStream_t to) {
  for (size_t k = 0; k < lanes.size(); ++k) {
    if (lanes[k].s == to) continue;
    hipEvent_t e = next_event(f);
    IPK_HIP(hipEventRecord(e, lanes[k].s));
    IPK_HIP(hipStreamWaitEvent(to, e, 0));
  }
  return IPOKE_OK;
}

template <typename Fn>
static int with_graph(ipoke_flow* f, std::vector<uintptr_t> key, hipStream_t caller, Fn enqueue) {
  if (!f->use_graph) return enqueue(caller);
  int rc0 = ensure_device(f); if (rc0) return rc0;
  ipoke_flow::GraphEntry* e = nullptr;
  for (auto& g : f->graphs) if (g.key == key) { e = &g; break; }
  if (!e) {
    if (f->graphs.size() >= 12) {
      size_t old = 0;
      for (size_t i = 1; i < f->graphs.size(); ++i) if (f->graphs[i].used < f->graphs[old].used) old = i;
      if (f->graphs[old].exec) (void)hipGraphExecDestroy(f->graphs[old].exec);
      if (f->graphs[old].graph) (void)hipGraphDestroy(f->graphs[old].graph);
      f->graphs.erase(f->graphs.begin() + old);
    }
    ipoke_flow::GraphEntry ne; ne.key = std::move(key); ne.used = ++f->tick;
    f->graphs.push_back(std::move(ne));
    return enqueue(caller);
  }
  e->used = ++f->tick;
  if (e->state < 0) return enqueue(caller);
  if (!e->exec) {
    const std::vector<uintptr_t> k = e->key;
    IPK_HIP(hipStreamBeginCapture(f->cap, hipStreamCaptureModeThreadLocal));
    const int rc = enqueue(f->cap);
    hipGraph_t g = nullptr;
    const hipError_t er = hipStreamEndCapture(f->cap, &g);
    e = nullptr;
    for (auto& ge : f->graphs) if (ge.key == k) { e = &ge; break; }
    if (rc != IPOKE_OK) { if (g) (void)hipGraphDestroy(g); if (e) e->state = -1; return rc; }
    if (er != hipSuccess || !g || !e) { (void)hipGetLastError(); if (g) (void)hipGraphDestroy(g); if (e) e->state = -1; return enqueue(caller); }
    hipGraphExec_t ex = nullptr;
    if (hipGraphInstantiate(&ex, g, nullptr, nullptr, 0) != hipSuccess) {
      (void)hipGetLastError(); (void)hipGraphDestroy(g); e->state = -1; return enqueue(caller);
    }
    e->graph = g; e->exec = ex; e->state = 1;
  }
  hipEvent_t a = next_event(f);
  IPK_HIP(hipEventRecord(a, caller)); IPK_HIP(hipStreamWaitEvent(f->cap, a, 0));
  IPK_HIP(hipGraphLaunch(e->exec, f->cap));
  hipEvent_t b = next_event(f);
  IPK_HIP(hipEventRecord(b, f->cap)); IPK_HIP(hipStreamWaitEvent(caller, b, 0));
  return IPOKE_OK;
}

__global__ void handoff_poll_kernel(const unsigned* unit_xchg, const unsigned* coupling_xchg, unsigned* host_words) {
  if (threadIdx.x == 0) {
    host_words[0] = unit_xchg ? unit_xchg[0] : 0u;
    host_words[1] = coupling_xchg ? coupling_xchg[0] : 0u;
  }
}
static int reinit_scratch(ipoke_flow* f, hipStream_t s) {
  if (f->d_xchg) IPK_HIP(hipMemsetAsync(f->d_xchg, 0, (size_t)f->xchg_bytes, s));
  if (f->d_cxchg) { int rc = ipoke_conv3x3_coupling_xchg_init(f->d_cxchg, reinterpret_cast<void*>(s)); if (rc) return rc; }
  return IPOKE_OK;
}
static bool stream_is_capturing(hipStream_t s) {
  hipStreamCaptureStatus st = hipStreamCaptureStatusNone;
  if (hipStreamIsCapturing(s, &st) != hipSuccess) { (void)hipGetLastError(); return false; }
  return st != hipStreamCaptureStatusNone;
}
static int pass_begin(ipoke_flow* f, hipStream_t s) {
  int rc = ensure_device(f); if (rc) return rc;
  if (!f->pass_recorded || stream_is_capturing(s)) return IPOKE_OK;
  if (s != f->pass_stream) IPK_HIP(hipStreamWaitEvent(s, f->pass_ev, 0));
  if (f->pass_unchecked) {
    const hipError_t q = hipEventQuery(f->pass_ev);
    if (q == hipSuccess) {
      f->pass_unchecked = false;
      const unsigned tu = f->h_tmo[0], tc = f->h_tmo[1];
      if (tu | tc) {
        rc = reinit_scratch(f, s); if (rc) return rc;
        f->h_tmo[0] = f->h_tmo[1] = 0;
        return fail(IPOKE_ERR_STATE, "hand-off time-out in an earlier pass of this flow (row-split unit launches: " + std::to_string(tu) +
                                     ", fused conv3 + coupling launches: " + std::to_string(tc) +
                                     "): the states / gradients of that pass are invalid; the exchange scratches have been re-initialised");
      }
    } else {
      (void)hipGetLastError();
    }
  }
  return IPOKE_OK;
}
static int pass_end(ipoke_flow* f, hipStream_t s) {
  if (!f->h_tmo || (!f->d_xchg && !f->d_cxchg) || stream_is_capturing(s)) return IPOKE_OK;
  hipLaunchKernelGGL(handoff_poll_kernel, dim3(1), dim3(64), 0, s, reinterpret_cast<const unsigned*>(f->d_xchg),
                     reinterpret_cast<const unsigned*>(f->d_cxchg), f->h_tmo);
  IPK_LAUNCH_CHECK();
  IPK_HIP(hipEventRecord(f->pass_ev, s));
  f->pass_stream = s; f->pass_recorded = true; f->pass_unchecked = true;
  return IPOKE_OK;
}
__global__ void handoff_inject_kernel(unsigned* word) { if (threadIdx.x == 0) atomicAdd(word, 1u); }
extern "C" int ipoke_flow_test_inject_timeout(ipoke_flow* f, int which, void* stream) {
  IPK_REQUIRE(f && (which == 0 || which == 1), "bad arguments");
  int rc = ensure_device(f); if (rc) return rc;
  unsigned* w = reinterpret_cast<unsigned*>(which == 0 ? f->d_xchg : f->d_cxchg);
  IPK_REQUIRE(w != nullptr, "this flow has no such scratch (unit_split = 1 / coupling fusion off)");
  hipLaunchKernelGGL(handoff_inject_kernel, dim3(1), dim3(64), 0, reinterpret_cast<hipStream_t>(stream), w);
  IPK_LAUNCH_CHECK();
  return IPOKE_OK;
}
extern "C" int ipoke_flow_handoff_timeouts(ipoke_flow* f, uint32_t* out) {
  IPK_REQUIRE(f && out, "null argument");
  out[0] = out[1] = 0;
  IPK_HIP(hipDeviceSynchronize());
  if (f->d_xchg) IPK_HIP(hipMemcpy(&out[0], f->d_xchg, sizeof(uint32_t), hipMemcpyDeviceToHost));
  if (f->d_cxchg) IPK_HIP(hipMemcpy(&out[1], f->d_cxchg, sizeof(uint32_t), hipMemcpyDeviceToHost));
  return IPOKE_OK;
}

static int run_forward(ipoke_flow* f, const float* params, const int32_t* perm, const void* shadow, const float* x_nchw,
                       const float* cond_nchw, int B, float* out_nchw, float* logdet, void* workspace, int save, int init,
                       float* params_mut, hipStream_t stream_h) {
  void* stream = reinterpret_cast<void*>(stream_h);
  int rc = common_checks(f, B); if (rc) return rc;
  rc = ensure_device(f); if (rc) return rc;
  IPK_REQUIRE(params && perm && x_nchw && out_nchw && workspace, "null argument");
// ... 172 lines not shown
  std::vector<Ctx> lanes;
  rc = make_lanes(c, f->n_lanes, lanes); if (rc) return rc;
  rc = fork_lanes(f, c.s, lanes); if (rc) return rc;
  const int64_t hb = (int64_t)f->cfg.hidden * f->esz;
  static const bool no_an_ext = getenv("IPOKE_NO_AN_EXT") != nullptr;
  auto actnorm_feeds = [&](int k) {
    if (no_an_ext || k < 1 || k >= (int)f->ops.size()) return false;
    const Op& an = f->ops[k]; const Op& nx = f->ops[k - 1];
    return an.type == OP_ACTNORM && an.unit_of < 0 && nx.type == OP_NICE && nx.Kc1 - nx.cin <= c.ld && nx.Kc1 <= 64;
  };
  int cur = 0;
  for (int i = (int)f->ops.size() - 1; i >= 0; --i) {
    const Op& op = f->ops[i];
    if (op.unit_of >= 0 && i == op.unit_of + 5) {
      const int h = op.unit_of;
      static const int lidx[4] = {0, 1, 3, 4};
      for (const Ctx& l : lanes) {
        ipoke_mcf_desc d4[4];
        for (int k = 0; k < 4; ++k) {
          const Op& mk = f->ops[h + lidx[k]];
          mcf_desc(l, mk, d4[k]);
          if (mk.fuse_act >= 0) { d4[k].post_log_scale = params + f->ops[mk.fuse_act].p_ls; d4[k].post_bias = params + f->ops[mk.fuse_act].p_bias; }
        }
        d4[3].x = l.state(cur); d4[0].y = l.state(cur ^ 1);
        d4[0].x = d4[3].x; d4[3].y = d4[0].y;
        rc = ipoke_macow_unit_inv(d4, l.dtype, l.stream()); if (rc) return rc;
      }
      cur ^= 1;
      i = h;
      continue;
    }
    for (const Ctx& l : lanes) {
      const float* in = l.state(cur); float* out = l.state(cur ^ 1);
      if (op.type == OP_LU) {
        rc = ipoke_lu_apply(in, out, (int64_t)l.B * l.f->P, l.ld, op.C, lu_mat(l, op, 1), 0, l.stream());
      } else if (op.type == OP_ACTNORM) {
        const Op* nx = actnorm_feeds(i) ? &f->ops[i - 1] : nullptr;
        rc = ipoke_actnorm_inv_ext(in, out, (int)l.M, l.ld, op.c0, op.Cn, op.p_ls >= 0 ? params + op.p_ls : nullptr,
                                   op.p_bias >= 0 ? params + op.p_bias : nullptr, op.idx_bwd >= 0 ? perm + op.idx_bwd : nullptr,
                                   nx ? l.rows(l.plan.tmp_zc, 64L * f->esz) : nullptr, nx ? nx->Kc1 : 0, nx ? nx->z_off : 0,
                                   nx ? nx->z_stride : 1, nx ? nx->cin : 0, l.dtype, l.stream());
      } else if (op.type == OP_MCF) {
        ipoke_mcf_desc d; mcf_desc(l, op, d);
        d.x = in; d.y = out;
        rc = ipoke_mcf_inv(&d, l.dtype, l.stream());
      } else {
        const bool have_zc = i + 1 < (int)f->ops.size() && (nice_feeds(f->ops[i + 1], op) || actnorm_feeds(i + 1));
        const bool one_launch = nice_fused(l, op);
        void* h2 = l.rows(l.plan.tmp_h2, (int64_t)op.hidK * f->esz);
        rc = nice_net(l, op, in, l.rows(l.plan.tmp_h1, hb), h2, l.rows(l.plan.tmp_zc, 64L * f->esz), have_zc, !one_launch);
        if (rc) return rc;
        ipoke_affine_desc a; nice_affine_desc(l, op, a);
        const bool feed = i > 0 && nice_feeds(op, f->ops[i - 1]);
        void* ext = feed ? l.rows(l.plan.tmp_zc, 64L * f->esz) : nullptr;
        const int ext_ld = feed ? f->ops[i - 1].Kc1 : 0;
        if (one_launch) {
          ipoke_conv_desc d3; nice_conv3_desc(l, op, h2, d3);
          ipoke_coupling_epi e; std::memset(&e, 0, sizeof(e));
          e.mode = 2; e.in = in; e.out = out; e.ext = ext; e.ext_ld = ext_ld; e.xchg = f->d_cxchg;
          rc = ipoke_conv3x3_coupling(&d3, &a, &e, l.B, l.dtype, l.stream());
        } else {
          rc = ipoke_affine_inv_ext(&a, in, out, l.B, ext, ext_ld, l.dtype, l.stream());
        }
      }
      if (rc) return rc;
    }
    cur ^= 1;
  }
  rc = join_lanes(f, lanes, c.s); if (rc) return rc;
  return ipoke_state_to_nchw(c.state(cur), x_nchw, B, z, f->P, c.ld, stream);
}

extern "C" int ipoke_flow_reverse(ipoke_flow* f, const float* params, const int32_t* perm, const void* shadow,
                                  const float* z_nchw, const float* cond_nchw, int B, float* x_nchw, void* workspace,
                                  void* stream) {
  IPK_REQUIRE(f != nullptr, "null flow handle");
  std::vector<uintptr_t> key = {2, (uintptr_t)params, (uintptr_t)perm, (uintptr_t)shadow, (uintptr_t)z_nchw, (uintptr_t)cond_nchw,
                                (uintptr_t)B, (uintptr_t)x_nchw, (uintptr_t)workspace};
  int rc = pass_begin(f, reinterpret_cast<hipStream_t>(stream)); if (rc) return rc;
  rc = with_graph(f, std::move(key), reinterpret_cast<hipStream_t>(stream), [&](hipStream_t s) {
    return run_reverse(f, params, perm, shadow, z_nchw, cond_nchw, B, x_nchw, workspace, s);
  });
  return rc ? rc : pass_end(f, reinterpret_cast<hipStream_t>(stream));
}

static int run_backward(ipoke_flow* f, const float* params, const int32_t* perm, const void* shadow,
                        const float* d_out_nchw, const float* d_logdet, int B, float* grads, float* dx_nchw,
                        void* workspace, hipStream_t stream_h, int npieces = 1, hipStream_t ready_stream = nullptr,
                        ipoke_grad_ready_fn ready = nullptr, void* user = nullptr) {
  void* stream = reinterpret_cast<void*>(stream_h);
  int rc = common_checks(f, B); if (rc) return rc;
  rc = ensure_device(f); if (rc) return rc;
  IPK_REQUIRE(params && perm && shadow && d_out_nchw && d_logdet && grads && workspace, "null argument");
  hipStream_t s = reinterpret_cast<hipStream_t>(stream);
  Ctx c{f, B, (int64_t)B * f->P, f->cfg.z_channels, f->cfg.dtype, s, params, perm,
        reinterpret_cast<const unsigned char*>(shadow), reinterpret_cast<unsigned char*>(workspace), make_plan(*f, B, 1)};
  c.Bfull = B;
  const int z = f->cfg.z_channels, hid = f->cfg.hidden;
  const int64_t hb = (int64_t)hid * f->esz;
  rc = ipoke_nchw_to_state(d_out_nchw, c.at<float>(c.plan.g0), B, z, f->P, c.ld, stream); if (rc) return rc;
  IPK_HIP(hipMemcpyAsync(c.dld(), d_logdet, B * sizeof(float), hipMemcpyDeviceToDevice, s));
  std::vector<Ctx> lanes;
  rc = make_lanes(c, f->n_lanes, lanes); if (rc) return rc;
  rc = fork_lanes(f, s, lanes); if (rc) return rc;
  hipStream_t ws_stream = f->use_side ? f->side : s;
  void* wstream = reinterpret_cast<void*>(ws_stream);
  static const int side_delay = getenv("IPOKE_SIDE_DELAY_US") ? atoi(getenv("IPOKE_SIDE_DELAY_US")) : 0;
  auto wgrads_wait_lanes = [&]() -> int {
    int r0 = join_lanes(f, lanes, ws_stream); if (r0) return r0;
    if (side_delay > 0 && f->use_side) return ipoke_spin_delay(side_delay, wstream);
    return IPOKE_OK;
  };
  rc = ensure_tables(f, B, c.plan); if (rc) return rc;
  int pend_lo = -1, pend_hi = -1, pend_op = -1;
  auto flush_mcf = [&]() -> int {
    if (pend_lo < 0) return IPOKE_OK;
    const Op& op = f->ops[pend_op];
    const int nb = pend_hi - pend_lo + 1;
    int r = wgrads_wait_lanes(); if (r) return r;
    static const int mcf_cap = getenv("IPOKE_TN_MAX_WGS") ? atoi(getenv("IPOKE_TN_MAX_WGS")) : 0;
    ipoke_wgrad_desc w; std::memset(&w, 0, sizeof(w));
    w.NB = B; w.Di = 1; w.Hi = 8; w.Wi = 8; w.Do = 1; w.Ho = 8; w.Wo = 8; w.kd = w.kh = w.kw = 1; w.sd = w.sh = w.sw = 1;
    w.max_workgroups = f->use_side ? mcf_cap : 0;
    const int K2 = op.H + f->cfg.cond_channels;
    w.a_f32 = 0; w.a_sn = 64L * op.K2p; w.a_sh = 8L * op.K2p; w.a_sw = op.K2p; w.a_sc = 1; w.Kc_real = K2; w.Kc = op.K2p;
    w.ldy = op.K3p; w.Nout = 2 * op.C; w.w_sn = K2; w.w_sc = 1; w.w_st = 0;
    r = ipoke_conv_wgrad_batched(&w, reinterpret_cast<const unsigned char*>(f->d_w2tab) + (size_t)pend_lo * ipoke_wgrad_batch_entry_size(),
                                 nb, c.ws, c.ws, grads, c.dtype, wstream);
    if (r) return r;
    std::memset(&w, 0, sizeof(w));
    w.NB = B; w.Di = 1; w.Hi = 8; w.Wi = 8; w.Do = 1; w.Ho = 8; w.Wo = 8; w.kd = 1; w.kh = 2; w.kw = 3; w.sd = w.sh = w.sw = 1;
    w.max_workgroups = f->use_side ? mcf_cap : 0;
    if (f->mcf_xop) {
      w.a_f32 = 0; w.a_sn = 64L * op.Cp; w.a_sh = 8L * op.Cp; w.a_sw = op.Cp; w.a_sc = 1; w.Kc_real = op.Cp; w.Kc = op.Cp; w.Kc_store = op.C;
    } else {
      w.a_f32 = 1; w.a_sn = 64L * c.ld; w.a_sh = 8L * c.ld; w.a_sw = c.ld; w.a_sc = 1; w.Kc_real = op.C; w.Kc = op.Cp;
    }
    w.ldy = op.Hq; w.Nout = op.H; w.w_sn = (int64_t)op.C * 6; w.w_sc = 6; w.w_st = 1;
    r = ipoke_conv_wgrad_batched(&w, reinterpret_cast<const unsigned char*>(f->d_w1tab) + (size_t)pend_lo * ipoke_wgrad_batch_entry_size(),
                                 nb, c.ws, c.ws, grads, c.dtype, wstream);
    pend_lo = pend_hi = pend_op = -1;
    return r;
  };
  if (f->use_side) {
    hipEvent_t e = next_event(f);
    IPK_HIP(hipEventRecord(e, s)); IPK_HIP(hipStreamWaitEvent(f->side, e, 0));
  }
  hipStream_t rs = ready_stream ? ready_stream : s;
  const std::vector<std::pair<int, int>> pieces = backward_pieces(f, npieces);
  const int wgrad_adam_mode = getenv("IPOKE_WGRAD_ADAM") ? atoi(getenv("IPOKE_WGRAD_ADAM")) : 0;
  const bool wgrad_adam = wgrad_adam_mode != 0 && f->nadam.on && !getenv("IPOKE_PROBE_SKIP_ADAM") && f->c2_straight &&
                          c.dtype == IPOKE_BF16 && f->use_side && lanes.size() == 1 && hid % 128 == 0 && (int)f->ajobs.size() == f->n_nice && !f->cfg.condition_nice;
  std::function<int()> flush_nice_fn = []() { return (int)IPOKE_OK; };
  auto native_adam_range = [&](int64_t b0, int64_t b1, int max_blocks) -> int {
    const ipoke_flow::NativeAdam& A = f->nadam;
    float* pm = const_cast<float*>(params);
    void* rstream = reinterpret_cast<void*>(rs);
    if (f->c2_straight)
      return adam_range(f, pm, grads, A.m, A.v, A.vmax, const_cast<void*>(shadow), b0, b1, A.lr, A.beta1, A.beta2, A.eps, A.wd, A.step,
                        A.grad_scale, max_blocks, rstream, wgrad_adam);
    int r = ipoke_adam_amsgrad_step_grid(pm + b0, grads + b0, A.m + b0, A.v + b0, A.vmax + b0, b1 - b0, A.lr, A.beta1, A.beta2, A.eps, A.wd, A.step,
                                         A.grad_scale, max_blocks, rstream);
    if (r) return r;
    return prepare_range(f, params, const_cast<void*>(shadow), b0, b1, false, rstream);
  };
  auto finish_piece = [&](int lvl_lo, int lvl_hi, int piece) -> int {
    int r = flush_nice_fn(); if (r) return r;
    r = flush_mcf(); if (r) return r;
    r = join_lanes(f, lanes, rs); if (r) return r;
    if (f->use_side && f->side != rs) {
      hipEvent_t e = next_event(f);
      IPK_HIP(hipEventRecord(e, f->side)); IPK_HIP(hipStreamWaitEvent(rs, e, 0));
    }
    void* rstream = reinterpret_cast<void*>(rs);
    const int r0 = f->red_first[f->units[lvl_lo].op_lo], r1 = f->red_first[f->units[lvl_hi].op_hi];
    if (r1 > r0) {
      r = ipoke_reduce_rows_multi(reinterpret_cast<const float*>(c.ws), grads,
                                  reinterpret_cast<const unsigned char*>(f->d_redtab) + (size_t)r0 * ipoke_reduce_entry_size(), r1 - r0, B,
                                  rstream);
      if (r) return r;
    }
    int64_t p0[3] = {-1, -1, -1}, p1[3] = {-1, -1, -1};
    int wj0[3] = {0, 0, 0}, wj1[3] = {0, 0, 0}, rw0[3] = {0, 0, 0}, rw1[3] = {0, 0, 0};
    for (int u = lvl_lo; u <= lvl_hi; ++u) {
      const auto& un = f->units[u];
      const int k = un.kind;
      if (p0[k] < 0) { p0[k] = un.p_lo; wj0[k] = un.wj_lo; rw0[k] = un.row_lo; }
      p1[k] = un.p_hi; wj1[k] = un.wj_hi; rw1[k] = un.row_hi;
      if (un.p2_lo >= 0) { if (p0[2] < 0) p0[2] = un.p2_lo; p1[2] = un.p2_hi; }
    }
    for (int kind = 0; kind < 2; ++kind) {
      if (p0[kind] < 0) continue;
      r = ipoke_wn_bwd_multi_range(params, grads, c.wn_inv(), f->d_wjobs, wj0[kind], wj1[kind] - wj0[kind], rw0[kind],
                                   rw1[kind] - rw0[kind], rstream);
      if (r) return r;
    }
    static const bool probe_skip_adam = getenv("IPOKE_PROBE_SKIP_ADAM") != nullptr;
    if (f->nadam.on && !probe_skip_adam) {
      ipoke_flow::NativeAdam A = f->nadam;
      {
        static const int early = getenv("IPOKE_ADAM_EARLY_BLOCKS") ? atoi(getenv("IPOKE_ADAM_EARLY_BLOCKS")) : 0;
        static const int late = getenv("IPOKE_ADAM_LATE_PIECES") ? atoi(getenv("IPOKE_ADAM_LATE_PIECES")) : 3;
        if (early > 0 && piece < (int)pieces.size() - late) A.max_blocks = early;
      }
      for (int kind = 0; kind < 3; ++kind) {
        if (p0[kind] < 0 || p1[kind] <= p0[kind]) continue;
        r = native_adam_range(p0[kind], p1[kind], A.max_blocks); if (r) return r;
      }
    }
    if (ready)
      for (int kind = 0; kind < 3; ++kind)
        if (p0[kind] >= 0 && p1[kind] > p0[kind]) ready(user, piece, p0[kind], p1[kind]);
    return IPOKE_OK;
  };
  std::vector<int> pend_nice;
  auto flush_nice = [&]() -> int {
    if (pend_nice.empty()) return IPOKE_OK;
    int rc = wgrads_wait_lanes(); if (rc) return rc;
    static const int tn_cap = getenv("IPOKE_TN_MAX_WGS") ? atoi(getenv("IPOKE_TN_MAX_WGS")) : 0;
    size_t i0 = 0;
    while (i0 < pend_nice.size()) {
      const Op& op = f->ops[pend_nice[i0]];
      size_t i1 = i0 + 1;
      while (i1 < pend_nice.size()) {
        const Op& o2 = f->ops[pend_nice[i1]];
        if (o2.nice_idx != f->ops[pend_nice[i1 - 1]].nice_idx - 1 || o2.Kc1 != op.Kc1 || o2.cin != op.cin || o2.cout != op.cout ||
            o2.Kc3 != op.Kc3) break;
        ++i1;
      }
      const int nb = (int)(i1 - i0), lo = f->ops[pend_nice[i1 - 1]].nice_idx;
      ipoke_wgrad_desc w;
      auto base8 = [&](int k, int pad) {
        std::memset(&w, 0, sizeof(w));
        w.NB = B; w.Di = 1; w.Hi = 8; w.Wi = 8; w.Do = 1; w.Ho = 8; w.Wo = 8; w.kd = 1; w.kh = w.kw = k;
        w.sd = w.sh = w.sw = 1; w.ph = w.pw = pad;
        w.max_workgroups = f->use_side ? tn_cap : 0;
      };
      auto entries = [&](int k) {
        return reinterpret_cast<const unsigned char*>(f->d_ntab[k]) + (size_t)lo * ipoke_wgrad_batch_entry_size();
      };
      base8(3, 1);
      w.a_sn = 64L * op.hidK; w.a_sh = 8L * op.hidK; w.a_sw = op.hidK; w.a_sc = 1; w.Kc_real = op.hidK; w.Kc = op.hidK;
      w.ldy = op.Kc3; w.Nout = 2 * op.cout;
      w.w_sn = (int64_t)op.hidK * 9; w.w_sc = 9; w.w_st = 1;
      rc = ipoke_conv_wgrad_batched(&w, entries(2), nb, c.ws, c.ws, grads, c.dtype, wstream); if (rc) return rc;
      base8(1, 0);
      w.a_sn = 64L * hid; w.a_sh = 8L * hid; w.a_sw = hid; w.a_sc = 1; w.Kc_real = hid; w.Kc = hid;
      w.ldy = hid; w.Nout = hid;
      w.w_sn = hid; w.w_sc = 1; w.w_st = 0;
      ipoke_wgrad_adam wa;
      if (wgrad_adam) {
        const ipoke_flow::NativeAdam& A = f->nadam;
        wa.params = const_cast<float*>(params); wa.m = A.m; wa.v = A.v; wa.vmax = A.vmax;
        wa.operand = const_cast<unsigned char*>(c.shadow + c.shadow_base());
        wa.lr = A.lr; wa.beta1 = A.beta1; wa.beta2 = A.beta2; wa.eps = A.eps; wa.weight_decay = A.wd; wa.grad_scale = A.grad_scale; wa.step = A.step;
        wa.keep_grad = wgrad_adam_mode == 2;
        w.adam = &wa;
      }
      rc = ipoke_conv_wgrad_batched(&w, entries(1), nb, c.ws, c.ws, grads, c.dtype, wstream); if (rc) return rc;
      base8(3, 1);
      w.a_f32 = 0; w.a_sn = 64L * op.Kc1; w.a_sh = 8L * op.Kc1; w.a_sw = op.Kc1; w.a_sc = 1;
      w.Kc_real = op.Kc1; w.Kc = op.Kc1;
      w.ldy = hid; w.Nout = hid;
      w.w_sn = (int64_t)op.cin * 9; w.w_sc = 9; w.w_st = 1; w.Kc_store = op.cin;
      rc = ipoke_conv_wgrad_batched(&w, entries(0), nb, c.ws, c.ws, grads, c.dtype, wstream); if (rc) return rc;
      i0 = i1;
    }
    pend_nice.clear();
    return IPOKE_OK;
  };
  flush_nice_fn = flush_nice;
  static const int flush_min = getenv("IPOKE_NICE_FLUSH_MIN") ? atoi(getenv("IPOKE_NICE_FLUSH_MIN")) : 4;
  auto maybe_flush_nice = [&]() -> int { return (int)pend_nice.size() >= flush_min ? flush_nice() : (int)IPOKE_OK; };
  size_t pk = 0;
  int cur = 0;
  int pending_an = -1;
  const int64_t goff[2] = {c.plan.g0, c.plan.g1};
  for (int i = (int)f->ops.size() - 1; i >= 0; --i) {
    const Op& op = f->ops[i];
    if (op.unit_of >= 0 && i == op.unit_of + 5) {
      const int h = op.unit_of;
      rc = maybe_flush_nice(); if (rc) return rc;
      static const int lidx[4] = {0, 1, 3, 4};
      for (const Ctx& l : lanes) {
        ipoke_mcf_desc d4[4];
        for (int k = 0; k < 4; ++k) {
          const int j = h + lidx[k];
          const Op& mk = f->ops[j];
          mcf_desc(l, mk, d4[k]);
          d4[k].x = l.state(j);
          d4[k].a2_save = l.rows(mk.ws_a, (int64_t)mk.K2p * f->esz); d4[k].scale_save = l.rowsf(mk.ws_b, mk.C);
          d4[k].dparams_save = l.rows(mk.ws_c, (int64_t)mk.K3p * f->esz); d4[k].dc_save = l.rows(mk.ws_d, (int64_t)mk.Hq * f->esz);
          if (f->mcf_xop) d4[k].x_op_save = l.rows(mk.ws_e, (int64_t)mk.Cp * f->esz);
          d4[k].dbias_part = l.dbp(j, 2 * mk.C, f->unit_split);
          if (mk.fuse_act >= 0) {
            const Op& an = f->ops[mk.fuse_act];
            d4[k].post_log_scale = params + an.p_ls; d4[k].post_bias = params + an.p_bias;
            d4[k].y_post = l.state(j + 2);
            d4[k].post_part = l.dbp(mk.fuse_act, 2 * an.Cn, f->unit_split);
          }
        }
        d4[3].dy = l.rowsf(goff[cur], l.ld); d4[0].dx = l.rowsf(goff[cur ^ 1], l.ld); d4[0].dld = l.dld();
        IPK_REQUIRE(f->unit_split == 1 || f->d_xchg, "row-split unit launches without exchange scratch (ensure_tables)");
        if (f->unit_split > 1) { d4[0].split = f->unit_split; d4[0].xchg = f->d_xchg; }
        ipoke_unit_pair_desc pq;
        if (h >= 2 && f->ops[h - 1].pair_unit == h) {
          const Op& an = f->ops[h - 1]; const Op& cp = f->ops[h - 2];
          std::memset(&pq, 0, sizeof(pq));
          pq.an_log_scale = an.p_ls >= 0 ? params + an.p_ls : nullptr; pq.an_idx = an.idx_fwd >= 0 ? perm + an.idx_fwd : nullptr;
          pq.an_x = l.state(h - 1); pq.an_part = an.p_ls >= 0 ? l.dbp(h - 1, 2 * an.Cn, f->unit_split) : nullptr;
          pq.Cp = cp.cout; pq.t_off = cp.t_off; pq.t_stride = cp.t_stride; pq.x0 = l.state(h - 2); pq.scale = l.rowsf(cp.ws_c, cp.cout);
          pq.dparams = l.rows(cp.ws_d, (int64_t)cp.Kc3 * f->esz); pq.ldp = cp.Kc3; pq.dbias_part = l.dbp(h - 2, 2 * cp.cout, f->unit_split);
          pq.dx = d4[0].dx;
          d4[0].pair = &pq;
        }
        rc = ipoke_macow_unit_bwd(d4, l.dtype, l.stream()); if (rc) return rc;
      }
      for (int k = 3; k >= 0; --k) {
        const int j = h + lidx[k];
        const Op& mk = f->ops[j];
        if (pend_lo >= 0 && (f->ops[pend_op].C != mk.C || pend_hi - pend_lo + 1 >= 256)) { rc = flush_mcf(); if (rc) return rc; }
        if (pend_lo < 0) { pend_hi = mk.mcf_idx; pend_op = j; }
        pend_lo = mk.mcf_idx;
      }
      cur ^= 1;
      i = h;
      continue;
    }
    if (op.fused) {
      if (i == f->units[pieces[pk].first].op_lo) { rc = finish_piece(pieces[pk].first, pieces[pk].second, pk); if (rc) return rc; ++pk; }
      continue;
    }
    if (op.type == OP_ACTNORM && op.pair_unit >= 0) {
      if (i == f->units[pieces[pk].first].op_lo) { rc = finish_piece(pieces[pk].first, pieces[pk].second, pk); if (rc) return rc; ++pk; }
      continue;
    }
    if (op.type == OP_ACTNORM && op.an_prev >= 0 && i != f->units[pieces[pk].first].op_lo) { pending_an = i; continue; }
    if (op.type != OP_NICE) { rc = maybe_flush_nice(); if (rc) return rc; }
    for (const Ctx& l : lanes) {
      const bool by_unit = op.type == OP_NICE && op.pair_unit >= 0;
      const float* gin = l.rowsf(goff[cur], l.ld); float* gout = l.rowsf(goff[by_unit ? cur : cur ^ 1], l.ld);
      const float* xin = l.state(i);
      if (op.type == OP_LU) {
        rc = ipoke_lu_apply(gin, gout, (int64_t)l.B * l.f->P, l.ld, op.C, lu_mat(l, op, 0), 1, l.stream()); if (rc) return rc;
        rc = ipoke_lu_wgrad(gin, xin, l.B, f->P, l.ld, params, f->fbuf, l.at<float>(l.plan.lu),
                            reinterpret_cast<const unsigned char*>(f->d_lujobs) + (size_t)op.lu_idx * sizeof(LuJobH), l.dld(), grads,
                            l.stream());
        if (rc) return rc;
      } else if (op.type == OP_ACTNORM) {
        rc = ipoke_actnorm_bwd(gin, xin, gout, (int)l.M, l.ld, op.c0, op.Cn, op.p_ls >= 0 ? params + op.p_ls : nullptr,
// ... 104 lines not shown
```

ipoke_amd/csrc/prep.hip:

```cpp
#include "common.h"

namespace ipoke {

struct RelayoutJob {
  long src_off;
  long s_n, s_k;
  long dstA, dstB;
  long scale_off;
  int taps, n_real, k_real;
  int A_rows_pad, A_inner_pad, B_rows_pad, B_inner_pad, B_rows_real;
  int tile, tiles_k;
  int block_start;
  int frag_tiled;
};

template <typename T>
__device__ __forceinline__ long tiled_offset(int row, int col, int ld) {
  constexpr int KS = 64 / (int)sizeof(T), E16 = 16 / (int)sizeof(T);
  const int rb = row >> 4, r = row & 15, ks = col / KS, cq = col - ks * KS;
  return ((long)rb * (ld / KS) + ks) * (16 * KS) + (cq / E16) * (16 * E16) + r * E16 + (cq % E16);
}

template <typename T> struct RPack4;
template <> struct RPack4<bf16_t> { typedef __attribute__((ext_vector_type(4))) __bf16 type; };
template <> struct RPack4<float> { typedef f32x4 type; };

template <typename T, int TAPS, int TE>
__device__ __forceinline__ void relayout_tile(const RelayoutJob& j, const float* __restrict__ params, T* __restrict__ shadow,
                                              const float* __restrict__ wn_scale, int n0, int k0, float* tile) {
  constexpr int TP = TE + 1;
  constexpr int total = TE * TE * TAPS;
  typedef typename RPack4<T>::type pack_t;
  const bool k_mid = j.s_k < j.s_n;
  if (TAPS == 1 && j.s_k == 1 && ((j.s_n | j.src_off) & 3) == 0) {
    for (int e = threadIdx.x; e < total / 4; e += 256) {
      const int kl = (e % (TE / 4)) * 4, nl = e / (TE / 4);
      const int n = n0 + nl, k = k0 + kl;
      f32x4 v = {0.f, 0.f, 0.f, 0.f};
      if (n < j.n_real && k < j.k_real) {
        const float sc = j.scale_off >= 0 ? wn_scale[j.scale_off + n] : 1.f;
        const float* src = params + j.src_off + (long)n * j.s_n + k;
        if (k + 3 < j.k_real) {
          v = *reinterpret_cast<const f32x4*>(src);
          v[0] *= sc; v[1] *= sc; v[2] *= sc; v[3] *= sc;
        } else {
          for (int q = 0; q < 4; ++q) if (k + q < j.k_real) v[q] = src[q] * sc;
        }
      }
#pragma unroll
      for (int q = 0; q < 4; ++q) tile[nl * TP + kl + q] = v[q];
    }
  } else {
    for (int e = threadIdx.x; e < total; e += 256) {
      const int t = e % TAPS, rest = e / TAPS;
      const int m = rest % TE, sl = rest / TE;
      const int nl = k_mid ? sl : m, kl = k_mid ? m : sl;
      const int n = n0 + nl, k = k0 + kl;
      float v = 0.f;
      if (n < j.n_real && k < j.k_real) {
        v = params[j.src_off + (long)n * j.s_n + (long)k * j.s_k + t];
        if (j.scale_off >= 0) v *= wn_scale[j.scale_off + n];
      }
      tile[(nl * TAPS + t) * TP + kl] = v;
    }
  }
  __syncthreads();
  const int ldA = TAPS * j.A_inner_pad, ldB = TAPS * j.B_inner_pad;
  for (int e = threadIdx.x; e < total / 4; e += 256) {
    const int kl = (e % (TE / 4)) * 4, rest = e / (TE / 4);
    const int t = rest % TAPS, nl = rest / TAPS;
    const int n = n0 + nl, k = k0 + kl;
    if (n < j.A_rows_pad && k < j.A_inner_pad) {
      pack_t o;
#pragma unroll
      for (int q = 0; q < 4; ++q) o[q] = ET<T>::from_f32(tile[(nl * TAPS + t) * TP + kl + q]);
      const long off = j.frag_tiled ? tiled_offset<T>(n, t * j.A_inner_pad + k, ldA) : (long)n * ldA + t * j.A_inner_pad + k;
      *reinterpret_cast<pack_t*>(shadow + j.dstA + off) = o;
    }
  }
  for (int e = threadIdx.x; j.dstB >= 0 && e < total / 4; e += 256) {
    const int nl = (e % (TE / 4)) * 4, rest = e / (TE / 4);
    const int t = rest % TAPS, kl = rest / TAPS;
    const int n = n0 + nl, k = k0 + kl;
    if (k < j.B_rows_pad && n < j.B_inner_pad) {
      pack_t o;
      const bool live = k < j.B_rows_real;
#pragma unroll
      for (int q = 0; q < 4; ++q) o[q] = ET<T>::from_f32(live ? tile[((nl + q) * TAPS + t) * TP + kl] : 0.f);
      const long off = j.frag_tiled ? tiled_offset<T>(k, t * j.B_inner_pad + n, ldB) : (long)k * ldB + t * j.B_inner_pad + n;
      *reinterpret_cast<pack_t*>(shadow + j.dstB + off) = o;
    }
  }
}

template <typename T>
__global__ __launch_bounds__(256) void relayout_kernel(const float* __restrict__ params, T* __restrict__ shadow,
                                                       const float* __restrict__ wn_scale, const RelayoutJob* __restrict__ jobs,
                                                       int njobs, const int* __restrict__ block_job, int block_base, int nblocks) {
  __shared__ __attribute__((aligned(16))) float tile[32 * 33 * 9];
  for (int bid = (int)blockIdx.x + block_base; bid < block_base + nblocks; bid += (int)gridDim.x) {
    int lo = 0;
    if (block_job) {
      lo = block_job[bid];
    } else {
      int hi = njobs - 1;
      while (lo < hi) {
        const int mid = (lo + hi + 1) >> 1;
        if (jobs[mid].block_start <= bid) lo = mid; else hi = mid - 1;
      }
    }
    const RelayoutJob j = jobs[lo];
    const int t_id = bid - j.block_start;
    const int n0 = (t_id / j.tiles_k) * j.tile, k0 = (t_id % j.tiles_k) * j.tile;
    if (j.taps == 1) relayout_tile<T, 1, 64>(j, params, shadow, wn_scale, n0, k0, tile);
    else if (j.taps == 9) relayout_tile<T, 9, 32>(j, params, shadow, wn_scale, n0, k0, tile);
    else relayout_tile<T, 6, 32>(j, params, shadow, wn_scale, n0, k0, tile);
    __syncthreads();
  }
}

struct WnJob { long v_off, g_off, out_off; int rows, K; int row_start; };

__global__ void wn_scale_kernel(const float* __restrict__ params, float* __restrict__ scale, float* __restrict__ inv_norm,
                                const WnJob* __restrict__ jobs, int njobs, int row_base, int total_rows) {
  const int grow = row_base + blockIdx.x * (blockDim.x >> 6) + (threadIdx.x >> 6);
  if (grow >= row_base + total_rows) return;
  int lo = 0, hi = njobs - 1;
  while (lo < hi) {
    const int mid = (lo + hi + 1) >> 1;
    if (jobs[mid].row_start <= grow) lo = mid; else hi = mid - 1;
  }
  const WnJob j = jobs[lo];
  const int row = grow - j.row_start, lane = threadIdx.x & 63;
  const float* v = params + j.v_off + (long)row * j.K;
  float s = 0.f;
  if ((j.K & 3) == 0 && (((j.v_off + (long)row * j.K)) & 3) == 0) {
    const f32x4* v4 = reinterpret_cast<const f32x4*>(v);
    const int n4 = j.K >> 2;
    int k = lane;
    for (; k + 64 < n4; k += 128) {
      const f32x4 a = v4[k], b = v4[k + 64];
      s += a[0] * a[0] + a[1] * a[1] + a[2] * a[2] + a[3] * a[3] + b[0] * b[0] + b[1] * b[1] + b[2] * b[2] + b[3] * b[3];
    }
    if (k < n4) { const f32x4 a = v4[k]; s += a[0] * a[0] + a[1] * a[1] + a[2] * a[2] + a[3] * a[3]; }
  } else {
    for (int k = lane; k < j.K; k += 64) s += v[k] * v[k];
  }
  s = wave_sum(s);
  if (lane == 0) {
    const float nrm = sqrtf(s);
    scale[j.out_off + row] = params[j.g_off + row] / nrm;
    inv_norm[j.out_off + row] = 1.f / nrm;
  }
}

__global__ void wn_bwd_kernel(const float* __restrict__ params, float* __restrict__ grads, const float* __restrict__ inv_norm,
                              const WnJob* __restrict__ jobs, int njobs, int row_base, int total_rows) {
  const int grow = row_base + blockIdx.x * (blockDim.x >> 6) + (threadIdx.x >> 6);
  if (grow >= row_base + total_rows) return;
  int lo = 0, hi = njobs - 1;
  while (lo < hi) {
    const int mid = (lo + hi + 1) >> 1;
    if (jobs[mid].row_start <= grow) lo = mid; else hi = mid - 1;
  }
  const WnJob j = jobs[lo];
  const int row = grow - j.row_start, lane = threadIdx.x & 63;
  const float* v = params + j.v_off + (long)row * j.K;
  float* dw = grads + j.v_off + (long)row * j.K;
  const bool vec = (j.K & 3) == 0 && (((j.v_off + (long)row * j.K)) & 3) == 0;
  float dot = 0.f;
  if (vec && (j.K >> 2) <= 192) {
    const f32x4* v4 = reinterpret_cast<const f32x4*>(v);
    f32x4* d4 = reinterpret_cast<f32x4*>(dw);
    const int n4 = j.K >> 2;
    const f32x4 z4 = {0.f, 0.f, 0.f, 0.f};
    const bool h0 = lane < n4, h1 = lane + 64 < n4, h2 = lane + 128 < n4;
    const f32x4 a0 = h0 ? v4[lane] : z4, b0 = h0 ? d4[lane] : z4, a1 = h1 ? v4[lane + 64] : z4, b1 = h1 ? d4[lane + 64] : z4;
    const f32x4 a2 = h2 ? v4[lane + 128] : z4, b2 = h2 ? d4[lane + 128] : z4;
    if (h1) dot += a0[0] * b0[0] + a0[1] * b0[1] + a0[2] * b0[2] + a0[3] * b0[3] + a1[0] * b1[0] + a1[1] * b1[1] + a1[2] * b1[2] + a1[3] * b1[3];
    else if (h0) dot += a0[0] * b0[0] + a0[1] * b0[1] + a0[2] * b0[2] + a0[3] * b0[3];
    if (h2) dot += a2[0] * b2[0] + a2[1] * b2[1] + a2[2] * b2[2] + a2[3] * b2[3];
    dot = wave_sum(dot);
    const float inv = inv_norm[j.out_off + row], g = params[j.g_off + row];
    const float a = g * inv, bcoef = g * dot * inv * inv * inv;
    f32x4 o0, o1, o2;
#pragma unroll
    for (int q = 0; q < 4; ++q) { o0[q] = a * b0[q] - bcoef * a0[q]; o1[q] = a * b1[q] - bcoef * a1[q]; o2[q] = a * b2[q] - bcoef * a2[q]; }
    if (h0) d4[lane] = o0;
    if (h1) d4[lane + 64] = o1;
    if (h2) d4[lane + 128] = o2;
    if (lane == 0) grads[j.g_off + row] = dot * inv;
    return;
  }
  if (vec) {
    const f32x4* v4 = reinterpret_cast<const f32x4*>(v);
    const f32x4* d4 = reinterpret_cast<const f32x4*>(dw);
    const int n4 = j.K >> 2;
    int k = lane;
    for (; k + 64 < n4; k += 128) {
      const f32x4 a0 = v4[k], b0 = d4[k], a1 = v4[k + 64], b1 = d4[k + 64];
      dot += a0[0] * b0[0] + a0[1] * b0[1] + a0[2] * b0[2] + a0[3] * b0[3] + a1[0] * b1[0] + a1[1] * b1[1] + a1[2] * b1[2] + a1[3] * b1[3];
    }
    if (k < n4) { const f32x4 a0 = v4[k], b0 = d4[k]; dot += a0[0] * b0[0] + a0[1] * b0[1] + a0[2] * b0[2] + a0[3] * b0[3]; }
  } else {
    for (int k = lane; k < j.K; k += 64) dot += dw[k] * v[k];
  }
  dot = wave_sum(dot);
  const float inv = inv_norm[j.out_off + row], g = params[j.g_off + row];
  const float a = g * inv, bcoef = g * dot * inv * inv * inv;
  if (vec) {
    const f32x4* v4 = reinterpret_cast<const f32x4*>(v);
    f32x4* d4 = reinterpret_cast<f32x4*>(dw);
    const int n4 = j.K >> 2;
    int k = lane;
    for (; k + 64 < n4; k += 128) {
      const f32x4 a0 = v4[k], a1 = v4[k + 64];
      f32x4 b0 = d4[k], b1 = d4[k + 64];
#pragma unroll
      for (int q = 0; q < 4; ++q) { b0[q] = a * b0[q] - bcoef * a0[q]; b1[q] = a * b1[q] - bcoef * a1[q]; }
      d4[k] = b0; d4[k + 64] = b1;
    }
    if (k < n4) {
      const f32x4 a0 = v4[k]; f32x4 b0 = d4[k];
#pragma unroll
      for (int q = 0; q < 4; ++q) b0[q] = a * b0[q] - bcoef * a0[q];
      d4[k] = b0;
    }
  } else {
    for (int k = lane; k < j.K; k += 64) dw[k] = a * dw[k] - bcoef * v[k];
  }
  if (lane == 0) grads[j.g_off + row] = dot * inv;
}


struct AdamTileJob { long src_off, dstA, dstB; int N, K, tile_start, pad; };

template <typename T> struct Out8;
template <> struct Out8<bf16_t> {
  static __device__ __forceinline__ void store(bf16_t* dst, const float* x) {
    bf16x8 o;
#pragma unroll
    for (int q = 0; q < 8; ++q) o[q] = (bf16_t)x[q];
    *reinterpret_cast<bf16x8*>(dst) = o;
  }
};
template <> struct Out8<float> {
  static __device__ __forceinline__ void store(float* dst, const float* x) {
    *reinterpret_cast<f32x4*>(dst) = f32x4{x[0], x[1], x[2], x[3]};
    *reinterpret_cast<f32x4*>(dst + 4) = f32x4{x[4], x[5], x[6], x[7]};
  }
};

template <bool NT> __device__ __forceinline__ f32x4 ld_stream(const float* q) {
  if (NT) return __builtin_nontemporal_load(reinterpret_cast<const f32x4*>(q));
  return *reinterpret_cast<const f32x4*>(q);
}
template <bool NT> __device__ __forceinline__ void st_stream(float* q, f32x4 v) {
  if (NT) __builtin_nontemporal_store(v, reinterpret_cast<f32x4*>(q));
  else *reinterpret_cast<f32x4*>(q) = v;
}
#ifdef IPOKE_ADAM_TEMPORAL
static constexpr bool kNtCast = false, kNtSeg = false;
#else
static constexpr bool kNtCast = true, kNtSeg = true;
#endif

template <typename T>
__global__ __launch_bounds__(256) void adam_shadow_tile_kernel(float* __restrict__ p, const float* __restrict__ g, float* __restrict__ m,
                                                               float* __restrict__ v, float* __restrict__ vmax, T* __restrict__ shadow,
                                                               const AdamTileJob* __restrict__ jobs, int njobs, int tile_begin,
                                                               int ntiles, AdamHyper h) {
  constexpr int TP = 65;
  __shared__ float tile[64 * TP];
  const int tid = threadIdx.x;
  const int G = (int)gridDim.x, end = tile_begin + ntiles;
  struct Regs { f32x4 pp[4], gg[4], mm[4], vv[4], vx[4]; long off[2]; long dstA, dstB; int N, K, n0, k0; };
  auto load = [&](int t, Regs& R) {
    int lo = 0, hi = njobs - 1;
    while (lo < hi) {
      const int mid = (lo + hi + 1) >> 1;
      if (jobs[mid].tile_start <= t) lo = mid; else hi = mid - 1;
    }
    const AdamTileJob j = jobs[lo];
    const int lt = t - j.tile_start, tiles_k = j.K >> 6;
    R.n0 = (lt / tiles_k) << 6; R.k0 = (lt % tiles_k) << 6; R.N = j.N; R.K = j.K; R.dstA = j.dstA; R.dstB = j.dstB;
#pragma unroll
    for (int i = 0; i < 2; ++i) {
      const int u = tid + 256 * i, r = u >> 3, c = (u & 7) * 8;
      R.off[i] = j.src_off + (long)(R.n0 + r) * j.K + R.k0 + c;
#pragma unroll
      for (int q = 0; q < 2; ++q) {
        R.pp[2 * i + q] = ld_stream<kNtCast>(p + R.off[i] + 4 * q);
        R.gg[2 * i + q] = ld_stream<kNtCast>(g + R.off[i] + 4 * q);
        R.mm[2 * i + q] = ld_stream<kNtCast>(m + R.off[i] + 4 * q);
        R.vv[2 * i + q] = ld_stream<kNtCast>(v + R.off[i] + 4 * q);
        R.vx[2 * i + q] = ld_stream<kNtCast>(vmax + R.off[i] + 4 * q);
      }
    }
  };
  auto process = [&](Regs& R) {
#pragma unroll
    for (int e = 0; e < 4; ++e) adam_amsgrad_update4(R.pp[e], R.gg[e], R.mm[e], R.vv[e], R.vx[e], h);
#pragma unroll
    for (int i = 0; i < 2; ++i) {
      const int u = tid + 256 * i, r = u >> 3, c = (u & 7) * 8;
      float x[8];
#pragma unroll
      for (int q = 0; q < 2; ++q) {
        st_stream<kNtCast>(p + R.off[i] + 4 * q, R.pp[2 * i + q]);
        st_stream<kNtCast>(m + R.off[i] + 4 * q, R.mm[2 * i + q]);
        st_stream<kNtCast>(v + R.off[i] + 4 * q, R.vv[2 * i + q]);
        st_stream<kNtCast>(vmax + R.off[i] + 4 * q, R.vx[2 * i + q]);
#pragma unroll
        for (int k = 0; k < 4; ++k) { x[4 * q + k] = R.pp[2 * i + q][k]; tile[r * TP + c + 4 * q + k] = R.pp[2 * i + q][k]; }
      }
      Out8<T>::store(shadow + R.dstA + (long)(R.n0 + r) * R.K + R.k0 + c, x);
    }
    __syncthreads();
#pragma unroll
    for (int i = 0; i < 2; ++i) {
      const int u = tid + 256 * i, kl = u >> 3, nl = (u & 7) * 8;
      float x[8];
#pragma unroll
      for (int q = 0; q < 8; ++q) x[q] = tile[(nl + q) * TP + kl];
      Out8<T>::store(shadow + R.dstB + (long)(R.k0 + kl) * R.N + R.n0 + nl, x);
    }
    __syncthreads();
  };
  int t = tile_begin + (int)blockIdx.x;
  if (t >= end) return;
  Regs RA, RB;
  load(t, RA);
  while (true) {
    const int t1 = t + G;
    if (t1 < end) load(t1, RB);
    process(RA);
    if (t1 >= end) break;
    const int t2 = t1 + G;
    if (t2 < end) load(t2, RA);
    process(RB);
    if (t2 >= end) break;
    t = t2;
  }
}

template <typename T>
__global__ __launch_bounds__(256) void adam_cast_kernel(float* __restrict__ p, const float* __restrict__ g, float* __restrict__ m,
                                                        float* __restrict__ v, float* __restrict__ vmax, T* __restrict__ shadow,
                                                        const AdamTileJob* __restrict__ jobs, int njobs, int chunk_begin, int nchunks, AdamHyper h) {
  typedef typename RPack4<T>::type pack_t;
  for (int c = chunk_begin + (int)blockIdx.x; c < chunk_begin + nchunks; c += (int)gridDim.x) {
    int lo = 0, hi = njobs - 1;
    while (lo < hi) {
      const int mid = (lo + hi + 1) >> 1;
      if (jobs[mid].tile_start <= c) lo = mid; else hi = mid - 1;
    }
    const AdamTileJob j = jobs[lo];
    const long rel = (long)(c - j.tile_start) * 4096 + threadIdx.x * 4;
    f32x4 pp[4], gg[4], mm[4], vv[4], vx[4];
#pragma unroll
    for (int q = 0; q < 4; ++q) {
      const long i = j.src_off + rel + q * 1024;
      pp[q] = ld_stream<kNtCast>(p + i); gg[q] = ld_stream<kNtCast>(g + i);
      mm[q] = ld_stream<kNtCast>(m + i); vv[q] = ld_stream<kNtCast>(v + i);
      vx[q] = ld_stream<kNtCast>(vmax + i);
    }
#pragma unroll
    for (int q = 0; q < 4; ++q) {
      adam_amsgrad_update4(pp[q], gg[q], mm[q], vv[q], vx[q], h);
      const long i = j.src_off + rel + q * 1024;
      st_stream<kNtCast>(p + i, pp[q]); st_stream<kNtCast>(m + i, mm[q]);
      st_stream<kNtCast>(v + i, vv[q]); st_stream<kNtCast>(vmax + i, vx[q]);
      pack_t o;
#pragma unroll
      for (int k = 0; k < 4; ++k) o[k] = ET<T>::from_f32(pp[q][k]);
      *reinterpret_cast<pack_t*>(shadow + j.dstA + rel + q * 1024) = o;
    }
  }
}

struct AdamSeg { long off, len; };
__global__ void adam_amsgrad_seg_kernel(float* __restrict__ p, const float* __restrict__ g, float* __restrict__ m, float* __restrict__ v,
                                        float* __restrict__ vmax, const AdamSeg* __restrict__ segs, int s0, long begin, long end,
                                        AdamHyper h) {
  const AdamSeg sg = segs[s0 + blockIdx.y];
  const long lo = sg.off > begin ? sg.off : begin, hi = sg.off + sg.len < end ? sg.off + sg.len : end;
  const long stride = (long)gridDim.x * blockDim.x * 4;
  for (long i0 = lo + ((long)blockIdx.x * blockDim.x + threadIdx.x) * 4; i0 < hi; i0 += 4 * stride) {
    if (i0 + 3 * stride + 3 < hi) {
      f32x4 pp[4], gg[4], mm[4], vv[4], vx[4];
#pragma unroll
      for (int q = 0; q < 4; ++q) {
        const long i = i0 + q * stride;
        pp[q] = ld_stream<kNtSeg>(p + i); gg[q] = ld_stream<kNtSeg>(g + i);
        mm[q] = ld_stream<kNtSeg>(m + i); vv[q] = ld_stream<kNtSeg>(v + i); vx[q] = ld_stream<kNtSeg>(vmax + i);
      }
#pragma unroll
      for (int q = 0; q < 4; ++q) {
        const long i = i0 + q * stride;
        adam_amsgrad_update4(pp[q], gg[q], mm[q], vv[q], vx[q], h);
        st_stream<kNtSeg>(p + i, pp[q]); st_stream<kNtSeg>(m + i, mm[q]);
        st_stream<kNtSeg>(v + i, vv[q]); st_stream<kNtSeg>(vmax + i, vx[q]);
      }
      continue;
    }
    for (int q = 0; q < 4; ++q) {
      const long i = i0 + q * stride;
      if (i + 3 < hi) {
        f32x4 pp = *reinterpret_cast<f32x4*>(p + i), gg = *reinterpret_cast<const f32x4*>(g + i);
        f32x4 mm = *reinterpret_cast<f32x4*>(m + i), vv = *reinterpret_cast<f32x4*>(v + i);
        f32x4 vx = *reinterpret_cast<f32x4*>(vmax + i);
        adam_amsgrad_update4(pp, gg, mm, vv, vx, h);
        *reinterpret_cast<f32x4*>(p + i) = pp; *reinterpret_cast<f32x4*>(m + i) = mm;
        *reinterpret_cast<f32x4*>(v + i) = vv; *reinterpret_cast<f32x4*>(vmax + i) = vx;
      } else {
        for (long k = i; k < hi; ++k) adam_amsgrad_update(p[k], g[k], m[k], v[k], vmax[k], h);
      }
    }
  }
}

}

using namespace ipoke;

extern "C" int ipoke_adam_tile_job_size(void) { return (int)sizeof(AdamTileJob); }
extern "C" int ipoke_adam_seg_size(void) { return (int)sizeof(AdamSeg); }

static AdamHyper make_hyper(float lr, float beta1, float beta2, float eps, float wd, int step, float grad_scale) {
  return adam_make_hyper(lr, beta1, beta2, eps, wd, step, grad_scale);
}

extern "C" int ipoke_adam_amsgrad_shadow_tiles(float* p, const float* g, float* m, float* v, float* vmax, void* shadow, const void* jobs_dev,
                                               int njobs, int tile_begin, int ntiles, float lr, float beta1, float beta2, float eps,
                                               float weight_decay, int step, float grad_scale, int max_blocks, int dtype, void* stream) {
  IPK_REQUIRE(p && g && m && v && vmax && shadow && jobs_dev && njobs >= 1 && ntiles >= 0 && step >= 1, "bad arguments");
  IPK_REQUIRE(dtype == IPOKE_BF16 || dtype == IPOKE_F32, "bad dtype");
  if (ntiles == 0) return IPOKE_OK;
  const AdamHyper h = make_hyper(lr, beta1, beta2, eps, weight_decay, step, grad_scale);
  const int grid = max_blocks > 0 && max_blocks < ntiles ? max_blocks : ntiles;
  hipStream_t s = reinterpret_cast<hipStream_t>(stream);
  if (dtype == IPOKE_BF16)
    hipLaunchKernelGGL(adam_shadow_tile_kernel<bf16_t>, dim3(grid), dim3(256), 0, s, p, g, m, v, vmax, (bf16_t*)shadow,
                       (const AdamTileJob*)jobs_dev, njobs, tile_begin, ntiles, h);
  else
    hipLaunchKernelGGL(adam_shadow_tile_kernel<float>, dim3(grid), dim3(256), 0, s, p, g, m, v, vmax, (float*)shadow,
                       (const AdamTileJob*)jobs_dev, njobs, tile_begin, ntiles, h);
  IPK_LAUNCH_CHECK();
  return IPOKE_OK;
}

extern "C" int ipoke_adam_amsgrad_cast_tiles(float* p, const float* g, float* m, float* v, float* vmax, void* shadow, const void* jobs_dev,
                                             int njobs, int tile_begin, int ntiles, float lr, float beta1, float beta2, float eps,
                                             float weight_decay, int step, float grad_scale, int max_blocks, int dtype, void* stream) {
  IPK_REQUIRE(p && g && m && v && vmax && shadow && jobs_dev && njobs >= 1 && ntiles >= 0 && step >= 1, "bad arguments");
  IPK_REQUIRE(dtype == IPOKE_BF16 || dtype == IPOKE_F32, "bad dtype");
  if (ntiles == 0) return IPOKE_OK;
  const AdamHyper h = make_hyper(lr, beta1, beta2, eps, weight_decay, step, grad_scale);
  const int cap = max_blocks > 0 ? max_blocks : 4096;
  const int grid = cap < ntiles ? cap : ntiles;
  hipStream_t s = reinterpret_cast<hipStream_t>(stream);
  if (dtype == IPOKE_BF16)
    hipLaunchKernelGGL(adam_cast_kernel<bf16_t>, dim3(grid), dim3(256), 0, s, p, g, m, v, vmax, (bf16_t*)shadow, (const AdamTileJob*)jobs_dev, njobs,
                       tile_begin, ntiles, h);
  else
    hipLaunchKernelGGL(adam_cast_kernel<float>, dim3(grid), dim3(256), 0, s, p, g, m, v, vmax, (float*)shadow, (const AdamTileJob*)jobs_dev, njobs,
                       tile_begin, ntiles, h);
  IPK_LAUNCH_CHECK();
  return IPOKE_OK;
}

extern "C" int ipoke_adam_amsgrad_segments(float* p, const float* g, float* m, float* v, float* vmax, const void* segs_dev, int seg_begin,
                                           int nsegs, int64_t begin, int64_t end, float lr, float beta1, float beta2, float eps,
                                           float weight_decay, int step, float grad_scale, int blocks_per_segment, void* stream) {
  IPK_REQUIRE(p && g && m && v && vmax && segs_dev && nsegs >= 0 && seg_begin >= 0 && end >= begin && step >= 1, "bad arguments");
  if (nsegs == 0) return IPOKE_OK;
  const AdamHyper h = make_hyper(lr, beta1, beta2, eps, weight_decay, step, grad_scale);
  hipLaunchKernelGGL(adam_amsgrad_seg_kernel, dim3(blocks_per_segment > 0 ? blocks_per_segment : 8, nsegs), dim3(256), 0,
                     reinterpret_cast<hipStream_t>(stream), p, g, m, v, vmax, (const AdamSeg*)segs_dev, seg_begin, (long)begin, (long)end, h);
  IPK_LAUNCH_CHECK();
  return IPOKE_OK;
}

extern "C" int ipoke_relayout_job_size(void) { return (int)sizeof(RelayoutJob); }
extern "C" int ipoke_wn_job_size(void) { return (int)sizeof(WnJob); }

extern "C" int ipoke_relayout_multi(const float* params, void* shadow, const float* wn_scale, const void* jobs_dev, int njobs,
                                    int total_blocks, const int32_t* block_job_dev, int dtype, void* stream) {
  return ipoke_relayout_multi_range(params, shadow, wn_scale, jobs_dev, njobs, 0, total_blocks, block_job_dev, dtype, stream);
}
extern "C" int ipoke_relayout_multi_range(const float* params, void* shadow, const float* wn_scale, const void* jobs_dev, int njobs,
                                          int block_begin, int nblocks, const int32_t* block_job_dev, int dtype, void* stream) {
  IPK_REQUIRE(params && shadow && jobs_dev && njobs > 0 && nblocks >= 0 && block_begin >= 0, "bad arguments");
  if (nblocks == 0) return IPOKE_OK;
  hipStream_t s = reinterpret_cast<hipStream_t>(stream);
  static const int cap_env = getenv("IPOKE_RELAYOUT_BLOCKS") ? atoi(getenv("IPOKE_RELAYOUT_BLOCKS")) : 0;
  const int cap = block_begin == 0 && nblocks > 100000 ? 65536 : (cap_env > 0 ? cap_env : nblocks);
  const int grid = nblocks < cap ? nblocks : cap;
  if (dtype == IPOKE_BF16)
    hipLaunchKernelGGL(relayout_kernel<bf16_t>, dim3(grid), dim3(256), 0, s, params, (bf16_t*)shadow, wn_scale,
                       (const RelayoutJob*)jobs_dev, njobs, block_job_dev, block_begin, nblocks);
  else
    hipLaunchKernelGGL(relayout_kernel<float>, dim3(grid), dim3(256), 0, s, params, (float*)shadow, wn_scale,
                       (const RelayoutJob*)jobs_dev, njobs, block_job_dev, block_begin, nblocks);
  IPK_LAUNCH_CHECK();
  return IPOKE_OK;
}
extern "C" int ipoke_wn_scale_multi(const float* params, float* scale, float* inv_norm, const void* jobs_dev, int njobs,
                                    int total_rows, void* stream) {
  return ipoke_wn_scale_multi_range(params, scale, inv_norm, jobs_dev, 0, njobs, 0, total_rows, stream);
}
extern "C" int ipoke_wn_scale_multi_range(const float* params, float* scale, float* inv_norm, const void* jobs_dev, int job_begin,
                                          int njobs, int row_begin, int nrows, void* stream) {
  IPK_REQUIRE(params && scale && inv_norm && jobs_dev && njobs >= 0 && nrows >= 0, "bad arguments");
  if (njobs == 0 || nrows == 0) return IPOKE_OK;
  hipLaunchKernelGGL(wn_scale_kernel, dim3(ceil_div(nrows, 4)), dim3(256), 0, reinterpret_cast<hipStream_t>(stream),
                     params, scale, inv_norm, (const WnJob*)jobs_dev + job_begin, njobs, row_begin, nrows);
  IPK_LAUNCH_CHECK();
  return IPOKE_OK;
}
extern "C" int ipoke_wn_bwd_multi(const float* params, float* grads, const float* inv_norm, const void* jobs_dev, int njobs,
                                  int total_rows, void* stream) {
  IPK_REQUIRE(params && grads && inv_norm && jobs_dev && njobs > 0, "bad arguments");
  hipLaunchKernelGGL(wn_bwd_kernel, dim3(ceil_div(total_rows, 4)), dim3(256), 0, reinterpret_cast<hipStream_t>(stream),
                     params, grads, inv_norm, (const WnJob*)jobs_dev, njobs, 0, total_rows);
  IPK_LAUNCH_CHECK();
  return IPOKE_OK;
}
extern "C" int ipoke_wn_bwd_multi_range(const float* params, float* grads, const float* inv_norm, const void* jobs_dev, int job_begin,
                                        int njobs, int row_begin, int nrows, void* stream) {
  IPK_REQUIRE(params && grads && inv_norm && jobs_dev && njobs >= 0 && nrows >= 0, "bad arguments");
  if (njobs == 0 || nrows == 0) return IPOKE_OK;
  hipLaunchKernelGGL(wn_bwd_kernel, dim3(ceil_div(nrows, 4)), dim3(256), 0, reinterpret_cast<hipStream_t>(stream),
                     params, grads, inv_norm, (const WnJob*)jobs_dev + job_begin, njobs, row_begin, nrows);
  IPK_LAUNCH_CHECK();
  return IPOKE_OK;
}
```

Measured before the change: 6573 video-frames/sec.

## Fuse weight-norm backward, Adam update and norm rescale into one row pass

Adds row-wise kernels that, per weight-normalized row, compute the g/v gradients from the norm, apply the AMSGrad Adam update to g and v, and recompute the new norm and scale in a single pass. Jobs are split into a wave-per-row class for short aligned rows and a block-per-row class, using LDS, for long rows. The separate wn_bwd and wn_scale launches and the Adam segment work over those rows are skipped when the layout check passes. This cuts repeated passes over parameter, gradient and moment memory, at the cost of more complex kernels and large LDS use for long rows. Launch counters are also added.

```diff
diff --git a/include/ipoke_hip.h b/include/ipoke_hip.h
--- a/include/ipoke_hip.h
+++ b/include/ipoke_hip.h
@@ -202,6 +202,11 @@
                        int total_rows, void* stream);
 int ipoke_wn_bwd_multi_range(const float* params, float* grads, const float* inv_norm, const void* jobs_dev, int job_begin, int njobs,
                              int row_begin, int nrows, void* stream);
+#define IPOKE_WN_ROWS_MAX_K 20000
+int ipoke_wn_adam_rows_range(float* params, float* grads, float* m, float* v, float* vmax, float* scale, float* inv_norm,
+                             const void* jobs_dev, int job_begin, int njobs, int row_begin, int nrows, int classes, int max_K,
+                             float lr, float beta1, float beta2, float eps, float weight_decay, int step, float grad_scale,
+                             int max_blocks, void* stream);
 
 
 
diff --git a/include/ipoke_hip_dev.h b/include/ipoke_hip_dev.h
--- a/include/ipoke_hip_dev.h
+++ b/include/ipoke_hip_dev.h
@@ -34,6 +34,11 @@
 
 int ipoke_flow_test_inject_timeout(ipoke_flow* f, int which, void* stream);
 
+enum { IPOKE_OPTIM_WN_BWD = 0, IPOKE_OPTIM_WN_SCALE = 1, IPOKE_OPTIM_ADAM_SEG = 2, IPOKE_OPTIM_RELAYOUT = 3, IPOKE_OPTIM_ADAM_CAST = 4,
+       IPOKE_OPTIM_ADAM_SHADOW_TILES = 5, IPOKE_OPTIM_WN_ADAM_ROWS = 6, IPOKE_OPTIM_KERNELS = 7 };
+int64_t ipoke_optim_launch_count(int kernel);
+int ipoke_optim_launch_count_reset(void);
+
 int ipoke_gru_set_fused(int mode);
 
 #ifdef __cplusplus
diff --git a/ipoke_amd/_lib.py b/ipoke_amd/_lib.py
--- a/ipoke_amd/_lib.py
+++ b/ipoke_amd/_lib.py
@@ -255,6 +255,10 @@
     "ipoke_adam_amsgrad_segments": (c_int, [_P, _P, _P, _P, _P, _P, c_int, c_int, c_int64, c_int64, c_float, c_float, c_float, c_float,
                                             c_float, c_int, c_float, c_int, _P]),
     "ipoke_wn_bwd_multi_range": (c_int, [_P, _P, _P, _P, c_int, c_int, c_int, c_int, _P]),
+    "ipoke_wn_adam_rows_range": (c_int, [_P, _P, _P, _P, _P, _P, _P, _P, c_int, c_int, c_int, c_int, c_int, c_int, c_float, c_float, c_float,
+                                         c_float, c_float, c_int, c_float, c_int, _P]),
+    "ipoke_optim_launch_count": (c_int64, [c_int]),
+    "ipoke_optim_launch_count_reset": (c_int, []),
     "ipoke_flow_backward_pieces": (c_int, [_P, _P, _P, _P, _P, _P, c_int, _P, _P, _P, c_int, _P, GRAD_READY_FN, _P, _P]),
     "ipoke_video_to_cl": (c_int, [_P, c_int64, c_int64, c_int64, c_int64, c_int64, c_int, c_int, c_int, c_int, c_int, _P, c_int, c_int, c_int,
                                   c_int, _P, _P]),
diff --git a/ipoke_amd/csrc/flow_engine.hip b/ipoke_amd/csrc/flow_engine.hip
--- a/ipoke_amd/csrc/flow_engine.hip
+++ b/ipoke_amd/csrc/flow_engine.hip
@@ -1,3 +1,5 @@
+#include <algorithm>
+#include <utility>
 #include <functional>
 #include <memory>
 #include <vector>
@@ -82,6 +84,9 @@
   std::vector<AdamSegH> asegs;
   void* d_ajobs = nullptr; void* d_rjobs2 = nullptr; void* d_rblockjob2 = nullptr; void* d_asegs = nullptr;
   std::vector<WnJobH> wjobs;
+  std::vector<WnJobH> wjobs_r, wjobs_b; int wrows_r = 0, wrows_b = 0, wn_max_K = 0; bool wn_onepass = false;
+  std::vector<AdamSegH> asegs_w;
+  void* d_wjobs_r = nullptr; void* d_wjobs_b = nullptr; void* d_asegs_w = nullptr;
   std::vector<LsRefH> lsrefs;
   void* d_rjobs = nullptr; void* d_wjobs = nullptr; void* d_lsrefs = nullptr; void* d_rblockjob = nullptr;
   hipStream_t side = nullptr;
@@ -692,6 +697,31 @@
     if (pos < f->n_params) f->asegs.push_back({(long)pos, (long)(f->n_params - pos)});
     for (size_t k = 1; k < f->rjobs.size(); ++k) IPK_REQUIRE(f->rjobs[k].src_off > f->rjobs[k - 1].src_off, "relayout jobs must be in parameter order");
   }
+  {
+    f->wn_onepass = true;
+    std::vector<std::pair<int64_t, int64_t>> taken;
+    for (const auto& a : f->ajobs) taken.push_back({a.src_off, a.src_off + (int64_t)a.N * a.K});
+    for (const auto& w : f->wjobs) {
+      WnJobH j = w;
+      if (!(w.g_off < w.v_off && w.v_off - (w.g_off + w.rows) < 4)) f->wn_onepass = false;
+      taken.push_back({w.g_off, w.v_off + (int64_t)w.rows * w.K});
+      if ((w.K & 3) == 0 && (w.v_off & 3) == 0 && (w.K >> 2) <= 192) {
+        j.row_start = f->wrows_r; f->wjobs_r.push_back(j); f->wrows_r += w.rows;
+      } else {
+        j.row_start = f->wrows_b; f->wjobs_b.push_back(j); f->wrows_b += w.rows;
+        f->wn_max_K = std::max(f->wn_max_K, w.K);
+      }
+    }
+    if (f->wn_max_K > IPOKE_WN_ROWS_MAX_K) f->wn_onepass = false;
+    std::sort(taken.begin(), taken.end());
+    int64_t pos = 0;
+    for (const auto& t : taken) {
+      if (t.first < pos) { f->wn_onepass = false; break; }
+      if (t.first > pos) f->asegs_w.push_back({(long)pos, (long)(t.first - pos)});
+      pos = t.second;
+    }
+    if (pos < f->n_params) f->asegs_w.push_back({(long)pos, (long)(f->n_params - pos)});
+  }
   const char* env = getenv("IPOKE_NO_SIDE_STREAM");
   f->use_side = !(env && env[0] == '1');
   const char* gr = getenv("IPOKE_GRAPH");
@@ -784,6 +814,18 @@
   }
   IPK_HIP(hipMalloc(&f->d_wjobs, f->wjobs.size() * sizeof(WnJobH)));
   IPK_HIP(hipMemcpy(f->d_wjobs, f->wjobs.data(), f->wjobs.size() * sizeof(WnJobH), hipMemcpyHostToDevice));
+  if (!f->wjobs_r.empty()) {
+    IPK_HIP(hipMalloc(&f->d_wjobs_r, f->wjobs_r.size() * sizeof(WnJobH)));
+    IPK_HIP(hipMemcpy(f->d_wjobs_r, f->wjobs_r.data(), f->wjobs_r.size() * sizeof(WnJobH), hipMemcpyHostToDevice));
+  }
+  if (!f->wjobs_b.empty()) {
+    IPK_HIP(hipMalloc(&f->d_wjobs_b, f->wjobs_b.size() * sizeof(WnJobH)));
+    IPK_HIP(hipMemcpy(f->d_wjobs_b, f->wjobs_b.data(), f->wjobs_b.size() * sizeof(WnJobH), hipMemcpyHostToDevice));
+  }
+  if (!f->asegs_w.empty()) {
+    IPK_HIP(hipMalloc(&f->d_asegs_w, f->asegs_w.size() * sizeof(AdamSegH)));
+    IPK_HIP(hipMemcpy(f->d_asegs_w, f->asegs_w.data(), f->asegs_w.size() * sizeof(AdamSegH), hipMemcpyHostToDevice));
+  }
   if (!f->lujobs.empty()) {
     IPK_REQUIRE((int)sizeof(LuJobH) == ipoke_lu_job_size(), "LU job table layout mismatch");
     IPK_HIP(hipMalloc(&f->d_lujobs, f->lujobs.size() * sizeof(LuJobH)));
@@ -814,6 +856,9 @@
   if (f->d_rblockjob) (void)hipFree(f->d_rblockjob);
   if (f->d_ajobs) (void)hipFree(f->d_ajobs);
   if (f->d_asegs) (void)hipFree(f->d_asegs);
+  if (f->d_asegs_w) (void)hipFree(f->d_asegs_w);
+  if (f->d_wjobs_r) (void)hipFree(f->d_wjobs_r);
+  if (f->d_wjobs_b) (void)hipFree(f->d_wjobs_b);
   if (f->d_rjobs2) (void)hipFree(f->d_rjobs2);
   if (f->d_rblockjob2) (void)hipFree(f->d_rblockjob2);
   if (f->d_w1tab) (void)hipFree(f->d_w1tab);
@@ -910,14 +955,15 @@
                               reinterpret_cast<const int32_t*>(f->d_rblockjob), f->cfg.dtype, stream);
 }
 
-static int prepare_range(ipoke_flow* f, const float* params, void* shadow, int64_t begin, int64_t end, bool skip_fused, void* stream) {
+static int prepare_range(ipoke_flow* f, const float* params, void* shadow, int64_t begin, int64_t end, bool skip_fused, void* stream,
+                         bool skip_scale = false) {
   float* wn_scale = reinterpret_cast<float*>(shadow);
   float* wn_inv = wn_scale + align_up(f->wn_rows, 64);
   int w0 = 0, w1 = 0;
   while (w0 < (int)f->wjobs.size() && f->wjobs[w0].v_off < begin) ++w0;
   w1 = w0;
   while (w1 < (int)f->wjobs.size() && f->wjobs[w1].v_off < end) ++w1;
-  if (w1 > w0) {
+  if (w1 > w0 && !skip_scale) {
     const int row0 = f->wjobs[w0].row_start;
     const int row1 = w1 < (int)f->wjobs.size() ? f->wjobs[w1].row_start : (int)f->wn_rows;
     int rc = ipoke_wn_scale_multi_range(params, wn_scale, wn_inv, f->d_wjobs, w0, w1 - w0, row0, row1 - row0, stream);
@@ -960,7 +1006,7 @@
 
 static int adam_range(ipoke_flow* f, float* params, const float* grads, float* m, float* v, float* vmax, void* shadow, int64_t begin, int64_t end,
                       float lr, float beta1, float beta2, float eps, float weight_decay, int step, float grad_scale, int max_blocks, void* stream,
-                      bool skip_tiles = false);
+                      bool skip_tiles = false, bool rows_done = false);
 
 extern "C" int ipoke_flow_adam_range(ipoke_flow* f, float* params, const float* grads, float* m, float* v, float* vmax, void* shadow,
                                      int64_t begin, int64_t end, float lr, float beta1, float beta2, float eps, float weight_decay,
@@ -970,9 +1016,28 @@
   return adam_range(f, params, grads, m, v, vmax, shadow, begin, end, lr, beta1, beta2, eps, weight_decay, step, grad_scale, max_blocks, stream);
 }
 
+static int wn_rows_range(ipoke_flow* f, float* params, float* grads, float* m, float* v, float* vmax, void* shadow, int64_t begin, int64_t end,
+                         float lr, float beta1, float beta2, float eps, float weight_decay, int step, float grad_scale, int max_blocks, void* stream) {
+  float* wn_scale = reinterpret_cast<float*>(shadow);
+  float* wn_inv = wn_scale + align_up(f->wn_rows, 64);
+  for (int cls = 0; cls < 2; ++cls) {
+    const std::vector<WnJobH>& jobs = cls == 0 ? f->wjobs_r : f->wjobs_b;
+    int w0 = 0, w1 = 0;
+    while (w0 < (int)jobs.size() && jobs[w0].v_off < begin) ++w0;
+    w1 = w0;
+    while (w1 < (int)jobs.size() && jobs[w1].v_off < end) ++w1;
+    if (w1 == w0) continue;
+    const int row0 = jobs[w0].row_start, row1 = w1 < (int)jobs.size() ? jobs[w1].row_start : (cls == 0 ? f->wrows_r : f->wrows_b);
+    int rc = ipoke_wn_adam_rows_range(params, grads, m, v, vmax, wn_scale, wn_inv, cls == 0 ? f->d_wjobs_r : f->d_wjobs_b, w0, w1 - w0, row0,
+                                      row1 - row0, 1 << cls, f->wn_max_K, lr, beta1, beta2, eps, weight_decay, step, grad_scale, max_blocks, stream);
+    if (rc) return rc;
+  }
+  return IPOKE_OK;
+}
+
 static int adam_range(ipoke_flow* f, float* params, const float* grads, float* m, float* v, float* vmax, void* shadow, int64_t begin, int64_t end,
                       float lr, float beta1, float beta2, float eps, float weight_decay, int step, float grad_scale, int max_blocks, void* stream,
-                      bool skip_tiles) {
+                      bool skip_tiles, bool rows_done) {
   if (end == begin) return IPOKE_OK;
   int a0 = 0, a1 = 0;
   while (a0 < (int)f->ajobs.size() && f->ajobs[a0].src_off < begin) ++a0;
@@ -989,18 +1054,19 @@
                                           eps, weight_decay, step, grad_scale, max_blocks, f->cfg.dtype, stream);
     if (rc) return rc;
   }
+  const std::vector<AdamSegH>& segs = rows_done ? f->asegs_w : f->asegs;
   int s0 = 0, s1 = 0;
-  while (s0 < (int)f->asegs.size() && f->asegs[s0].off + f->asegs[s0].len <= begin) ++s0;
+  while (s0 < (int)segs.size() && segs[s0].off + segs[s0].len <= begin) ++s0;
   s1 = s0;
-  while (s1 < (int)f->asegs.size() && f->asegs[s1].off < end) ++s1;
+  while (s1 < (int)segs.size() && segs[s1].off < end) ++s1;
   if (s1 > s0) {
     int per = max_blocks > 0 ? max_blocks / (s1 - s0) : 16;
     if (per < 2) per = 2; if (per > 32) per = 32;
-    int rc = ipoke_adam_amsgrad_segments(params, grads, m, v, vmax, f->d_asegs, s0, s1 - s0, begin, end, lr, beta1, beta2, eps, weight_decay,
-                                         step, grad_scale, per, stream);
+    int rc = ipoke_adam_amsgrad_segments(params, grads, m, v, vmax, rows_done ? f->d_asegs_w : f->d_asegs, s0, s1 - s0, begin, end, lr, beta1,
+                                         beta2, eps, weight_decay, step, grad_scale, per, stream);
     if (rc) return rc;
   }
-  return prepare_range(f, params, shadow, begin, end, true, stream);
+  return prepare_range(f, params, shadow, begin, end, true, stream, rows_done);
 }
 
 static int make_lanes(const Ctx& full, int want, std::vector<Ctx>& lanes) {
@@ -1479,13 +1545,20 @@
   const bool wgrad_adam = wgrad_adam_mode != 0 && f->nadam.on && !getenv("IPOKE_PROBE_SKIP_ADAM") && f->c2_straight &&
                           c.dtype == IPOKE_BF16 && f->use_side && lanes.size() == 1 && hid % 128 == 0 && (int)f->ajobs.size() == f->n_nice && !f->cfg.condition_nice;
   std::function<int()> flush_nice_fn = []() { return (int)IPOKE_OK; };
+  static const bool probe_skip_adam = getenv("IPOKE_PROBE_SKIP_ADAM") != nullptr;
+  const bool wn_onepass = f->nadam.on && !probe_skip_adam && f->c2_straight && f->wn_onepass;
   auto native_adam_range = [&](int64_t b0, int64_t b1, int max_blocks) -> int {
     const ipoke_flow::NativeAdam& A = f->nadam;
     float* pm = const_cast<float*>(params);
     void* rstream = reinterpret_cast<void*>(rs);
+    if (wn_onepass) {
+      int r = wn_rows_range(f, pm, grads, A.m, A.v, A.vmax, const_cast<void*>(shadow), b0, b1, A.lr, A.beta1, A.beta2, A.eps, A.wd, A.step,
+                            A.grad_scale, max_blocks, rstream);
+      if (r) return r;
+    }
     if (f->c2_straight)
       return adam_range(f, pm, grads, A.m, A.v, A.vmax, const_cast<void*>(shadow), b0, b1, A.lr, A.beta1, A.beta2, A.eps, A.wd, A.step,
-                        A.grad_scale, max_blocks, rstream, wgrad_adam);
+                        A.grad_scale, max_blocks, rstream, wgrad_adam, wn_onepass);
     int r = ipoke_adam_amsgrad_step_grid(pm + b0, grads + b0, A.m + b0, A.v + b0, A.vmax + b0, b1 - b0, A.lr, A.beta1, A.beta2, A.eps, A.wd, A.step,
                                          A.grad_scale, max_blocks, rstream);
     if (r) return r;
@@ -1516,13 +1589,12 @@
       p1[k] = un.p_hi; wj1[k] = un.wj_hi; rw1[k] = un.row_hi;
       if (un.p2_lo >= 0) { if (p0[2] < 0) p0[2] = un.p2_lo; p1[2] = un.p2_hi; }
     }
-    for (int kind = 0; kind < 2; ++kind) {
+    for (int kind = 0; kind < 2 && !wn_onepass; ++kind) {
       if (p0[kind] < 0) continue;
       r = ipoke_wn_bwd_multi_range(params, grads, c.wn_inv(), f->d_wjobs, wj0[kind], wj1[kind] - wj0[kind], rw0[kind],
                                    rw1[kind] - rw0[kind], rstream);
       if (r) return r;
     }
-    static const bool probe_skip_adam = getenv("IPOKE_PROBE_SKIP_ADAM") != nullptr;
     if (f->nadam.on && !probe_skip_adam) {
       ipoke_flow::NativeAdam A = f->nadam;
       {
diff --git a/ipoke_amd/csrc/prep.hip b/ipoke_amd/csrc/prep.hip
--- a/ipoke_amd/csrc/prep.hip
+++ b/ipoke_amd/csrc/prep.hip
@@ -1,4 +1,6 @@
 #include "common.h"
+
+#include <atomic>
 
 namespace ipoke {
 
@@ -121,6 +123,51 @@
 
 struct WnJob { long v_off, g_off, out_off; int rows, K; int row_start; };
 
+__device__ __forceinline__ float wn_sumsq4(const f32x4* v4, int n4, int lane) {
+  float s = 0.f;
+  int k = lane;
+  for (; k + 64 < n4; k += 128) {
+    const f32x4 a = v4[k], b = v4[k + 64];
+    s += a[0] * a[0] + a[1] * a[1] + a[2] * a[2] + a[3] * a[3] + b[0] * b[0] + b[1] * b[1] + b[2] * b[2] + b[3] * b[3];
+  }
+  if (k < n4) { const f32x4 a = v4[k]; s += a[0] * a[0] + a[1] * a[1] + a[2] * a[2] + a[3] * a[3]; }
+  return s;
+}
+__device__ __forceinline__ float wn_sumsq1(const float* v, int K, int lane) {
+  float s = 0.f;
+  for (int k = lane; k < K; k += 64) s += v[k] * v[k];
+  return s;
+}
+__device__ __forceinline__ float wn_dot_regs(const f32x4& a0, const f32x4& b0, const f32x4& a1, const f32x4& b1, const f32x4& a2,
+                                             const f32x4& b2, bool h0, bool h1, bool h2) {
+  float dot = 0.f;
+  if (h1) dot += a0[0] * b0[0] + a0[1] * b0[1] + a0[2] * b0[2] + a0[3] * b0[3] + a1[0] * b1[0] + a1[1] * b1[1] + a1[2] * b1[2] + a1[3] * b1[3];
+  else if (h0) dot += a0[0] * b0[0] + a0[1] * b0[1] + a0[2] * b0[2] + a0[3] * b0[3];
+  if (h2) dot += a2[0] * b2[0] + a2[1] * b2[1] + a2[2] * b2[2] + a2[3] * b2[3];
+  return dot;
+}
+__device__ __forceinline__ float wn_dot4(const f32x4* v4, const f32x4* d4, int n4, int lane) {
+  float dot = 0.f;
+  int k = lane;
+  for (; k + 64 < n4; k += 128) {
+    const f32x4 a0 = v4[k], b0 = d4[k], a1 = v4[k + 64], b1 = d4[k + 64];
+    dot += a0[0] * b0[0] + a0[1] * b0[1] + a0[2] * b0[2] + a0[3] * b0[3] + a1[0] * b1[0] + a1[1] * b1[1] + a1[2] * b1[2] + a1[3] * b1[3];
+  }
+  if (k < n4) { const f32x4 a0 = v4[k], b0 = d4[k]; dot += a0[0] * b0[0] + a0[1] * b0[1] + a0[2] * b0[2] + a0[3] * b0[3]; }
+  return dot;
+}
+__device__ __forceinline__ float wn_dot1(const float* v, const float* dw, int K, int lane) {
+  float dot = 0.f;
+  for (int k = lane; k < K; k += 64) dot += dw[k] * v[k];
+  return dot;
+}
+__device__ __forceinline__ float wn_dv(float a, float bcoef, float dw, float v) {
+#pragma clang fp contract(off)
+  return fmaf(a, dw, -(bcoef * v));
+}
+__device__ __forceinline__ bool wn_row_vec(long row_off, int K) { return (K & 3) == 0 && (row_off & 3) == 0; }
+__device__ __forceinline__ bool wn_row_in_regs(long row_off, int K) { return wn_row_vec(row_off, K) && (K >> 2) <= 192; }
+
 __global__ void wn_scale_kernel(const float* __restrict__ params, float* __restrict__ scale, float* __restrict__ inv_norm,
                                 const WnJob* __restrict__ jobs, int njobs, int row_base, int total_rows) {
   const int grow = row_base + blockIdx.x * (blockDim.x >> 6) + (threadIdx.x >> 6);
@@ -133,19 +180,7 @@
   const WnJob j = jobs[lo];
   const int row = grow - j.row_start, lane = threadIdx.x & 63;
   const float* v = params + j.v_off + (long)row * j.K;
-  float s = 0.f;
-  if ((j.K & 3) == 0 && (((j.v_off + (long)row * j.K)) & 3) == 0) {
-    const f32x4* v4 = reinterpret_cast<const f32x4*>(v);
-    const int n4 = j.K >> 2;
-    int k = lane;
-    for (; k + 64 < n4; k += 128) {
-      const f32x4 a = v4[k], b = v4[k + 64];
-      s += a[0] * a[0] + a[1] * a[1] + a[2] * a[2] + a[3] * a[3] + b[0] * b[0] + b[1] * b[1] + b[2] * b[2] + b[3] * b[3];
-    }
-    if (k < n4) { const f32x4 a = v4[k]; s += a[0] * a[0] + a[1] * a[1] + a[2] * a[2] + a[3] * a[3]; }
-  } else {
-    for (int k = lane; k < j.K; k += 64) s += v[k] * v[k];
-  }
+  float s = wn_row_vec(j.v_off + (long)row * j.K, j.K) ? wn_sumsq4(reinterpret_cast<const f32x4*>(v), j.K >> 2, lane) : wn_sumsq1(v, j.K, lane);
   s = wave_sum(s);
   if (lane == 0) {
     const float nrm = sqrtf(s);
@@ -167,9 +202,9 @@
   const int row = grow - j.row_start, lane = threadIdx.x & 63;
   const float* v = params + j.v_off + (long)row * j.K;
   float* dw = grads + j.v_off + (long)row * j.K;
-  const bool vec = (j.K & 3) == 0 && (((j.v_off + (long)row * j.K)) & 3) == 0;
+  const bool vec = wn_row_vec(j.v_off + (long)row * j.K, j.K);
   float dot = 0.f;
-  if (vec && (j.K >> 2) <= 192) {
+  if (wn_row_in_regs(j.v_off + (long)row * j.K, j.K)) {
     const f32x4* v4 = reinterpret_cast<const f32x4*>(v);
     f32x4* d4 = reinterpret_cast<f32x4*>(dw);
     const int n4 = j.K >> 2;
@@ -177,34 +212,19 @@
     const bool h0 = lane < n4, h1 = lane + 64 < n4, h2 = lane + 128 < n4;
     const f32x4 a0 = h0 ? v4[lane] : z4, b0 = h0 ? d4[lane] : z4, a1 = h1 ? v4[lane + 64] : z4, b1 = h1 ? d4[lane + 64] : z4;
     const f32x4 a2 = h2 ? v4[lane + 128] : z4, b2 = h2 ? d4[lane + 128] : z4;
-    if (h1) dot += a0[0] * b0[0] + a0[1] * b0[1] + a0[2] * b0[2] + a0[3] * b0[3] + a1[0] * b1[0] + a1[1] * b1[1] + a1[2] * b1[2] + a1[3] * b1[3];
-    else if (h0) dot += a0[0] * b0[0] + a0[1] * b0[1] + a0[2] * b0[2] + a0[3] * b0[3];
-    if (h2) dot += a2[0] * b2[0] + a2[1] * b2[1] + a2[2] * b2[2] + a2[3] * b2[3];
-    dot = wave_sum(dot);
+    dot = wave_sum(wn_dot_regs(a0, b0, a1, b1, a2, b2, h0, h1, h2));
     const float inv = inv_norm[j.out_off + row], g = params[j.g_off + row];
     const float a = g * inv, bcoef = g * dot * inv * inv * inv;
     f32x4 o0, o1, o2;
 #pragma unroll
-    for (int q = 0; q < 4; ++q) { o0[q] = a * b0[q] - bcoef * a0[q]; o1[q] = a * b1[q] - bcoef * a1[q]; o2[q] = a * b2[q] - bcoef * a2[q]; }
+    for (int q = 0; q < 4; ++q) { o0[q] = wn_dv(a, bcoef, b0[q], a0[q]); o1[q] = wn_dv(a, bcoef, b1[q], a1[q]); o2[q] = wn_dv(a, bcoef, b2[q], a2[q]); }
     if (h0) d4[lane] = o0;
     if (h1) d4[lane + 64] = o1;
     if (h2) d4[lane + 128] = o2;
     if (lane == 0) grads[j.g_off + row] = dot * inv;
     return;
   }
-  if (vec) {
-    const f32x4* v4 = reinterpret_cast<const f32x4*>(v);
-    const f32x4* d4 = reinterpret_cast<const f32x4*>(dw);
-    const int n4 = j.K >> 2;
-    int k = lane;
-    for (; k + 64 < n4; k += 128) {
-      const f32x4 a0 = v4[k], b0 = d4[k], a1 = v4[k + 64], b1 = d4[k + 64];
-      dot += a0[0] * b0[0] + a0[1] * b0[1] + a0[2] * b0[2] + a0[3] * b0[3] + a1[0] * b1[0] + a1[1] * b1[1] + a1[2] * b1[2] + a1[3] * b1[3];
-    }
-    if (k < n4) { const f32x4 a0 = v4[k], b0 = d4[k]; dot += a0[0] * b0[0] + a0[1] * b0[1] + a0[2] * b0[2] + a0[3] * b0[3]; }
-  } else {
-    for (int k = lane; k < j.K; k += 64) dot += dw[k] * v[k];
-  }
+  dot = vec ? wn_dot4(reinterpret_cast<const f32x4*>(v), reinterpret_cast<const f32x4*>(dw), j.K >> 2, lane) : wn_dot1(v, dw, j.K, lane);
   dot = wave_sum(dot);
   const float inv = inv_norm[j.out_off + row], g = params[j.g_off + row];
   const float a = g * inv, bcoef = g * dot * inv * inv * inv;
@@ -217,17 +237,17 @@
       const f32x4 a0 = v4[k], a1 = v4[k + 64];
       f32x4 b0 = d4[k], b1 = d4[k + 64];
 #pragma unroll
-      for (int q = 0; q < 4; ++q) { b0[q] = a * b0[q] - bcoef * a0[q]; b1[q] = a * b1[q] - bcoef * a1[q]; }
+      for (int q = 0; q < 4; ++q) { b0[q] = wn_dv(a, bcoef, b0[q], a0[q]); b1[q] = wn_dv(a, bcoef, b1[q], a1[q]); }
       d4[k] = b0; d4[k + 64] = b1;
     }
     if (k < n4) {
       const f32x4 a0 = v4[k]; f32x4 b0 = d4[k];
 #pragma unroll
-      for (int q = 0; q < 4; ++q) b0[q] = a * b0[q] - bcoef * a0[q];
+      for (int q = 0; q < 4; ++q) b0[q] = wn_dv(a, bcoef, b0[q], a0[q]);
       d4[k] = b0;
     }
   } else {
-    for (int k = lane; k < j.K; k += 64) dw[k] = a * dw[k] - bcoef * v[k];
+    for (int k = lane; k < j.K; k += 64) dw[k] = wn_dv(a, bcoef, dw[k], v[k]);
   }
   if (lane == 0) grads[j.g_off + row] = dot * inv;
 }
@@ -420,9 +440,187 @@
   }
 }
 
+
+
+__global__ __launch_bounds__(256) void wn_adam_rows_wave_kernel(float* params, float* grads, float* __restrict__ m, float* __restrict__ v2,
+                                                                float* __restrict__ vmax, float* __restrict__ scale, float* inv_norm,
+                                                                const WnJob* __restrict__ jobs, int njobs, int row_base, int total_rows,
+                                                                AdamHyper h) {
+  __shared__ __attribute__((aligned(16))) float stage[4][768];
+  const int w = threadIdx.x >> 6, lane = threadIdx.x & 63;
+  for (int grow = row_base + (int)blockIdx.x * 4 + w; grow < row_base + total_rows; grow += (int)gridDim.x * 4) {
+    int lo = 0, hi = njobs - 1;
+    while (lo < hi) {
+      const int mid = (lo + hi + 1) >> 1;
+      if (jobs[mid].row_start <= grow) lo = mid; else hi = mid - 1;
+    }
+    const WnJob j = jobs[lo];
+    const int row = grow - j.row_start;
+    const long roff = j.v_off + (long)row * j.K;
+    if (!wn_row_in_regs(roff, j.K)) continue;
+    const int n4 = j.K >> 2;
+    const f32x4 z4 = {0.f, 0.f, 0.f, 0.f};
+    const bool hv[3] = {lane < n4, lane + 64 < n4, lane + 128 < n4};
+    f32x4 a[3], b[3], mm[3], vv[3], vx[3];
+#pragma unroll
+    for (int i = 0; i < 3; ++i) {
+      const long o = roff + 4 * (lane + 64 * i);
+      a[i] = hv[i] ? ld_stream<kNtSeg>(params + o) : z4; b[i] = hv[i] ? ld_stream<kNtSeg>(grads + o) : z4;
+      mm[i] = hv[i] ? ld_stream<kNtSeg>(m + o) : z4; vv[i] = hv[i] ? ld_stream<kNtSeg>(v2 + o) : z4;
+      vx[i] = hv[i] ? ld_stream<kNtSeg>(vmax + o) : z4;
+    }
+    const float dot = wave_sum(wn_dot_regs(a[0], b[0], a[1], b[1], a[2], b[2], hv[0], hv[1], hv[2]));
+    const float inv = inv_norm[j.out_off + row], g = params[j.g_off + row];
+    const float ca = g * inv, bcoef = g * dot * inv * inv * inv;
+    f32x4* st4 = reinterpret_cast<f32x4*>(stage[w]);
+#pragma unroll
+    for (int i = 0; i < 3; ++i) {
+      if (!hv[i]) continue;
+      const long o = roff + 4 * (lane + 64 * i);
+      f32x4 dv;
+#pragma unroll
+      for (int q = 0; q < 4; ++q) dv[q] = wn_dv(ca, bcoef, b[i][q], a[i][q]);
+      adam_amsgrad_update4(a[i], dv, mm[i], vv[i], vx[i], h);
+      st_stream<kNtSeg>(params + o, a[i]); st_stream<kNtSeg>(m + o, mm[i]); st_stream<kNtSeg>(v2 + o, vv[i]);
+      st_stream<kNtSeg>(vmax + o, vx[i]); st_stream<kNtSeg>(grads + o, dv);
+      st4[lane + 64 * i] = a[i];
+    }
+    float gp = g;
+    if (lane == 0) {
+      const long o = j.g_off + row;
+      const float dg = dot * inv;
+      float gm = m[o], gv = v2[o], gx = vmax[o];
+      adam_amsgrad_update(gp, dg, gm, gv, gx, h);
+      params[o] = gp; m[o] = gm; v2[o] = gv; vmax[o] = gx; grads[o] = dg;
+    }
+    __builtin_amdgcn_wave_barrier();
+    const float s = wave_sum(wn_sumsq4(st4, n4, lane));
+    if (lane == 0) {
+      const float nrm = sqrtf(s);
+      scale[j.out_off + row] = gp / nrm;
+      inv_norm[j.out_off + row] = 1.f / nrm;
+    }
+    __builtin_amdgcn_wave_barrier();
+  }
+}
+
+static constexpr int kWnRowThreads = 768;
+template <int NV>
+__global__ __launch_bounds__(kWnRowThreads) void wn_adam_rows_block_kernel(float* params, float* grads, float* __restrict__ m, float* __restrict__ v2,
+                                                                  float* __restrict__ vmax, float* __restrict__ scale, float* inv_norm,
+                                                                  const WnJob* __restrict__ jobs, int njobs, int row_base, int total_rows,
+                                                                  int lds_k, AdamHyper h) {
+  extern __shared__ __attribute__((aligned(16))) float wn_smem[];
+  float* sv = wn_smem;
+  float* sd = wn_smem + lds_k;
+  float* sx = wn_smem + 2 * lds_k;
+  const int tid = threadIdx.x, lane = tid & 63;
+  for (int grow = row_base + (int)blockIdx.x; grow < row_base + total_rows; grow += (int)gridDim.x) {
+    int lo = 0, hi = njobs - 1;
+    while (lo < hi) {
+      const int mid = (lo + hi + 1) >> 1;
+      if (jobs[mid].row_start <= grow) lo = mid; else hi = mid - 1;
+    }
+    const WnJob j = jobs[lo];
+    const int row = grow - j.row_start;
+    const long roff = j.v_off + (long)row * j.K;
+    if (wn_row_in_regs(roff, j.K) || j.K > lds_k) continue;
+    const bool vec = wn_row_vec(roff, j.K);
+    const int n4 = j.K >> 2;
+    f32x4* sv4 = reinterpret_cast<f32x4*>(sv);
+    f32x4* sd4 = reinterpret_cast<f32x4*>(sd);
+    f32x4 mm[NV], vv[NV], vx[NV];
+    if (vec) {
+      f32x4 pa[NV], pb[NV];
+#pragma unroll
+      for (int i = 0; i < NV; ++i) {
+        const int idx = tid + kWnRowThreads * i;
+        if (idx < n4) { pa[i] = ld_stream<kNtSeg>(params + roff + 4 * idx); pb[i] = ld_stream<kNtSeg>(grads + roff + 4 * idx); }
+      }
+#pragma unroll
+      for (int i = 0; i < NV; ++i) {
+        const int idx = tid + kWnRowThreads * i;
+        if (idx < n4) { sv4[idx] = pa[i]; sd4[idx] = pb[i]; }
+      }
+#pragma unroll
+      for (int i = 0; i < NV; ++i) {
+        const int idx = tid + kWnRowThreads * i;
+        if (idx < n4) {
+          mm[i] = ld_stream<kNtSeg>(m + roff + 4 * idx); vv[i] = ld_stream<kNtSeg>(v2 + roff + 4 * idx);
+          vx[i] = ld_stream<kNtSeg>(vmax + roff + 4 * idx);
+        }
+      }
+    } else {
+      for (int k = tid; k < j.K; k += kWnRowThreads) { sv[k] = params[roff + k]; sd[k] = grads[roff + k]; }
+    }
+    __syncthreads();
+    if (tid < 64) {
+      const float d = wave_sum(vec ? wn_dot4(sv4, sd4, n4, lane) : wn_dot1(sv, sd, j.K, lane));
+      if (tid == 0) { sx[0] = d; sx[1] = params[j.g_off + row]; sx[2] = inv_norm[j.out_off + row]; }
+    }
+    __syncthreads();
+    const float dot = sx[0], g = sx[1], inv = sx[2];
+    const float ca = g * inv, bcoef = g * dot * inv * inv * inv;
+    if (vec) {
+#pragma unroll
+      for (int i = 0; i < NV; ++i) {
+        const int idx = tid + kWnRowThreads * i;
+        if (idx < n4) {
+          const long o = roff + 4 * idx;
+          f32x4 a = sv4[idx], dv;
+          const f32x4 b = sd4[idx];
+#pragma unroll
+          for (int q = 0; q < 4; ++q) dv[q] = wn_dv(ca, bcoef, b[q], a[q]);
+          adam_amsgrad_update4(a, dv, mm[i], vv[i], vx[i], h);
+          st_stream<kNtSeg>(params + o, a); st_stream<kNtSeg>(m + o, mm[i]); st_stream<kNtSeg>(v2 + o, vv[i]);
+          st_stream<kNtSeg>(vmax + o, vx[i]); st_stream<kNtSeg>(grads + o, dv);
+          sv4[idx] = a;
+        }
+      }
+    } else {
+      for (int k = tid; k < j.K; k += kWnRowThreads) {
+        const long o = roff + k;
+        float a = sv[k], mk = m[o], vk = v2[o], xk = vmax[o];
+        const float dv = wn_dv(ca, bcoef, sd[k], a);
+        adam_amsgrad_update(a, dv, mk, vk, xk, h);
+        params[o] = a; m[o] = mk; v2[o] = vk; vmax[o] = xk; grads[o] = dv;
+        sv[k] = a;
+      }
+    }
+    float gp = g;
+    if (tid == 0) {
+      const long o = j.g_off + row;
+      const float dg = dot * inv;
+      float gm = m[o], gv = v2[o], gx = vmax[o];
+      adam_amsgrad_update(gp, dg, gm, gv, gx, h);
+      params[o] = gp; m[o] = gm; v2[o] = gv; vmax[o] = gx; grads[o] = dg;
+    }
+    __syncthreads();
+    if (tid < 64) {
+      const float s = wave_sum(vec ? wn_sumsq4(sv4, n4, lane) : wn_sumsq1(sv, j.K, lane));
+      if (tid == 0) {
+        const float nrm = sqrtf(s);
+        scale[j.out_off + row] = gp / nrm;
+        inv_norm[j.out_off + row] = 1.f / nrm;
+      }
+    }
+    __syncthreads();
+  }
+}
+
 }
 
 using namespace ipoke;
+
+static std::atomic<int64_t> g_optim_launches[IPOKE_OPTIM_KERNELS];
+static inline void count_launch(int kernel) { g_optim_launches[kernel].fetch_add(1, std::memory_order_relaxed); }
+extern "C" int64_t ipoke_optim_launch_count(int kernel) {
+  return kernel >= 0 && kernel < IPOKE_OPTIM_KERNELS ? g_optim_launches[kernel].load(std::memory_order_relaxed) : -1;
+}
+extern "C" int ipoke_optim_launch_count_reset(void) {
+  for (auto& c : g_optim_launches) c.store(0, std::memory_order_relaxed);
+  return IPOKE_OK;
+}
 
 extern "C" int ipoke_adam_tile_job_size(void) { return (int)sizeof(AdamTileJob); }
 extern "C" int ipoke_adam_seg_size(void) { return (int)sizeof(AdamSeg); }
@@ -440,6 +638,7 @@
   const AdamHyper h = make_hyper(lr, beta1, beta2, eps, weight_decay, step, grad_scale);
   const int grid = max_blocks > 0 && max_blocks < ntiles ? max_blocks : ntiles;
   hipStream_t s = reinterpret_cast<hipStream_t>(stream);
+  count_launch(IPOKE_OPTIM_ADAM_SHADOW_TILES);
   if (dtype == IPOKE_BF16)
     hipLaunchKernelGGL(adam_shadow_tile_kernel<bf16_t>, dim3(grid), dim3(256), 0, s, p, g, m, v, vmax, (bf16_t*)shadow,
                        (const AdamTileJob*)jobs_dev, njobs, tile_begin, ntiles, h);
@@ -460,6 +659,7 @@
   const int cap = max_blocks > 0 ? max_blocks : 4096;
   const int grid = cap < ntiles ? cap : ntiles;
   hipStream_t s = reinterpret_cast<hipStream_t>(stream);
+  count_launch(IPOKE_OPTIM_ADAM_CAST);
   if (dtype == IPOKE_BF16)
     hipLaunchKernelGGL(adam_cast_kernel<bf16_t>, dim3(grid), dim3(256), 0, s, p, g, m, v, vmax, (bf16_t*)shadow, (const AdamTileJob*)jobs_dev, njobs,
                        tile_begin, ntiles, h);
@@ -476,6 +676,7 @@
   IPK_REQUIRE(p && g && m && v && vmax && segs_dev && nsegs >= 0 && seg_begin >= 0 && end >= begin && step >= 1, "bad arguments");
   if (nsegs == 0) return IPOKE_OK;
   const AdamHyper h = make_hyper(lr, beta1, beta2, eps, weight_decay, step, grad_scale);
+  count_launch(IPOKE_OPTIM_ADAM_SEG);
   hipLaunchKernelGGL(adam_amsgrad_seg_kernel, dim3(blocks_per_segment > 0 ? blocks_per_segment : 8, nsegs), dim3(256), 0,
                      reinterpret_cast<hipStream_t>(stream), p, g, m, v, vmax, (const AdamSeg*)segs_dev, seg_begin, (long)begin, (long)end, h);
   IPK_LAUNCH_CHECK();
@@ -497,6 +698,7 @@
   static const int cap_env = getenv("IPOKE_RELAYOUT_BLOCKS") ? atoi(getenv("IPOKE_RELAYOUT_BLOCKS")) : 0;
   const int cap = block_begin == 0 && nblocks > 100000 ? 65536 : (cap_env > 0 ? cap_env : nblocks);
   const int grid = nblocks < cap ? nblocks : cap;
+  count_launch(IPOKE_OPTIM_RELAYOUT);
   if (dtype == IPOKE_BF16)
     hipLaunchKernelGGL(relayout_kernel<bf16_t>, dim3(grid), dim3(256), 0, s, params, (bf16_t*)shadow, wn_scale,
                        (const RelayoutJob*)jobs_dev, njobs, block_job_dev, block_begin, nblocks);
@@ -514,6 +716,7 @@
                                           int njobs, int row_begin, int nrows, void* stream) {
   IPK_REQUIRE(params && scale && inv_norm && jobs_dev && njobs >= 0 && nrows >= 0, "bad arguments");
   if (njobs == 0 || nrows == 0) return IPOKE_OK;
+  count_launch(IPOKE_OPTIM_WN_SCALE);
   hipLaunchKernelGGL(wn_scale_kernel, dim3(ceil_div(nrows, 4)), dim3(256), 0, reinterpret_cast<hipStream_t>(stream),
                      params, scale, inv_norm, (const WnJob*)jobs_dev + job_begin, njobs, row_begin, nrows);
   IPK_LAUNCH_CHECK();
@@ -522,6 +725,7 @@
 extern "C" int ipoke_wn_bwd_multi(const float* params, float* grads, const float* inv_norm, const void* jobs_dev, int njobs,
                                   int total_rows, void* stream) {
   IPK_REQUIRE(params && grads && inv_norm && jobs_dev && njobs > 0, "bad arguments");
+  count_launch(IPOKE_OPTIM_WN_BWD);
   hipLaunchKernelGGL(wn_bwd_kernel, dim3(ceil_div(total_rows, 4)), dim3(256), 0, reinterpret_cast<hipStream_t>(stream),
                      params, grads, inv_norm, (const WnJob*)jobs_dev, njobs, 0, total_rows);
   IPK_LAUNCH_CHECK();
@@ -531,8 +735,56 @@
                                         int njobs, int row_begin, int nrows, void* stream) {
   IPK_REQUIRE(params && grads && inv_norm && jobs_dev && njobs >= 0 && nrows >= 0, "bad arguments");
   if (njobs == 0 || nrows == 0) return IPOKE_OK;
+  count_launch(IPOKE_OPTIM_WN_BWD);
   hipLaunchKernelGGL(wn_bwd_kernel, dim3(ceil_div(nrows, 4)), dim3(256), 0, reinterpret_cast<hipStream_t>(stream),
                      params, grads, inv_norm, (const WnJob*)jobs_dev + job_begin, njobs, row_begin, nrows);
   IPK_LAUNCH_CHECK();
   return IPOKE_OK;
 }
+
+extern "C" int ipoke_wn_adam_rows_range(float* params, float* grads, float* m, float* v, float* vmax, float* scale, float* inv_norm,
+                                        const void* jobs_dev, int job_begin, int njobs, int row_begin, int nrows, int classes, int max_K,
+                                        float lr, float beta1, float beta2, float eps, float weight_decay, int step, float grad_scale,
+                                        int max_blocks, void* stream) {
+  IPK_REQUIRE(params && grads && m && v && vmax && scale && inv_norm && jobs_dev && njobs >= 0 && nrows >= 0 && job_begin >= 0 && step >= 1,
+              "bad arguments");
+  IPK_REQUIRE((classes & ~3) == 0 && (!(classes & 2) || (max_K >= 1 && max_K <= IPOKE_WN_ROWS_MAX_K)), "bad row classes / row length");
+  if (njobs == 0 || nrows == 0 || classes == 0) return IPOKE_OK;
+  const AdamHyper h = make_hyper(lr, beta1, beta2, eps, weight_decay, step, grad_scale);
+  hipStream_t s = reinterpret_cast<hipStream_t>(stream);
+  const WnJob* jobs = (const WnJob*)jobs_dev + job_begin;
+  if (classes & 1) {
+    const int want = ceil_div(nrows, 4);
+    const int grid = max_blocks > 0 && max_blocks < want ? max_blocks : want;
+    count_launch(IPOKE_OPTIM_WN_ADAM_ROWS);
+    hipLaunchKernelGGL(wn_adam_rows_wave_kernel, dim3(grid), dim3(256), 0, s, params, grads, m, v, vmax, scale, inv_norm, jobs, njobs, row_begin,
+                       nrows, h);
+    IPK_LAUNCH_CHECK();
+  }
+  if (classes & 2) {
+    const int lds_k = round_up(max_K, 4);
+    const size_t lds = (size_t)(2 * lds_k + 4) * sizeof(float);
+    const int grid = max_blocks > 0 && max_blocks < nrows ? max_blocks : nrows;
+    count_launch(IPOKE_OPTIM_WN_ADAM_ROWS);
+#define IPK_WN_ROWS_LAUNCH(NV)                                                                                                         \
+    do {                                                                                                                                \
+      static bool big_lds = false;                             \
+      if (lds > 65536 && !big_lds) {                                                                                                    \
+        IPK_HIP(hipFuncSetAttribute(reinterpret_cast<const void*>(wn_adam_rows_block_kernel<NV>), hipFuncAttributeMaxDynamicSharedMemorySize, \
+                                    (int)((2 * IPOKE_WN_ROWS_MAX_K + 4) * sizeof(float))));                                             \
+        big_lds = true;                                                                                                                 \
+      }                                                                                                                                 \
+      hipLaunchKernelGGL(wn_adam_rows_block_kernel<NV>, dim3(grid), dim3(kWnRowThreads), lds, s, params, grads, m, v, vmax, scale, inv_norm, jobs, njobs, \
+                         row_begin, nrows, lds_k, h);                                                                                   \
+    } while (0)
+    constexpr int per_group = 4 * kWnRowThreads;
+    static_assert(7 * per_group >= IPOKE_WN_ROWS_MAX_K, "the widest instantiation must hold the longest row");
+    if (lds_k <= 2 * per_group) IPK_WN_ROWS_LAUNCH(2);
+    else if (lds_k <= 4 * per_group) IPK_WN_ROWS_LAUNCH(4);
+    else if (lds_k <= 6 * per_group) IPK_WN_ROWS_LAUNCH(6);
+    else IPK_WN_ROWS_LAUNCH(7);
+#undef IPK_WN_ROWS_LAUNCH
+    IPK_LAUNCH_CHECK();
+  }
+  return IPOKE_OK;
+}
```

New measurement: 6490 video-frames/sec. -1.3%, worse.
